# VKostoulas/Medical_Image_Generation

Measured on AMD Instinct MI355X. Metric: 3D DDPM U-Net train-step voxels/sec at 128^3 bf16, higher is better.
Workload: dtype bf16; 1 GPU; C4: DiffusionModelUNet num_channels=(32,64,128,256), attention at 16^3 (heads of 64), 128^3 x batch 1/GPU, eps-prediction, AdamW, clip 1.0; global_batch=1, parallelism=dp1, hipgraph=True

## Files before the change

include/medimgen_hip.h:

```cpp
#ifndef MEDIMGEN_HIP_H
#define MEDIMGEN_HIP_H

#include <hip/hip_runtime_api.h>
#include <stdint.h>

#ifdef __cplusplus
extern "C" {
#endif

#define MI_ERR_BAD_ARG 10001
#define MI_ERR_UNSUPPORTED 10002

int mi_abi_version(void);

int mi_ncdhw_f32_to_ndhwc_bf16(const float* src, void* dst, int N, int C, int64_t V, hipStream_t stream);
int mi_ndhwc_bf16_to_ncdhw_f32(const void* src, float* dst, int N, int C, int64_t V, hipStream_t stream);
int mi_cast_f32_to_bf16(const float* src, void* dst, int64_t n, hipStream_t stream);
int mi_cast_bf16_to_f32(const void* src, float* dst, int64_t n, int accumulate, hipStream_t stream);

int mi_add_bf16(const void* a, const void* b, void* out, int64_t n, hipStream_t stream);
int mi_copy_channels(const void* src, int Cs, int c0s, void* dst, int Cd, int c0d, int nC, int64_t nvox, hipStream_t stream);

int mi_upsample_nearest_fwd(const void* x, void* y, int N, int D, int H, int W, int C, int fd, int fh, int fw, hipStream_t stream);
int mi_upsample_nearest_bwd(const void* dy, void* dx, int N, int D, int H, int W, int C, int fd, int fh, int fw, hipStream_t stream);
int mi_space_to_depth(const void* in, int in_cstride, void* out, int N, int D, int H, int W, int C, int fd, int fh, int fw, hipStream_t stream);
int mi_depth_to_space(const void* in, void* out, int N, int D, int H, int W, int C, int fd, int fh, int fw, hipStream_t stream);

int64_t mi_gn_workspace_bytes(int N, int64_t V, int C);
int mi_gn_stats(const void* x, int x_cstride, int N, int64_t V, int C, int G, float eps, const float* gamma, const float* beta,
                float* scale_shift, float* mean_rstd, void* workspace, int64_t workspace_bytes, hipStream_t stream);
int mi_gn_stats_from_partial(const float* partial_a, int chunks_a, int Ca, const float* partial_b, int chunks_b, int Cb, int N, int64_t V,
                             int G, float eps, const float* gamma, const float* beta, float* scale_shift, float* mean_rstd,
                             hipStream_t stream);
int mi_gn_small_supported(int N, int64_t V, int C, int G);
int mi_gn_small_fwd(const void* x, int x_cstride, void* y, int y_cstride, int N, int64_t V, int C, int G, float eps, const float* gamma,
                    const float* beta, float* scale_shift, float* mean_rstd, int act, hipStream_t stream);
int mi_gn_apply(const void* x, int x_cstride, const float* scale_shift, void* y, int y_cstride, int N, int64_t V, int C, int silu,
                hipStream_t stream);
int mi_gn_bwd(const void* g, int g_cstride, const void* x, int x_cstride, int N, int64_t V, int C, int G, const float* gamma,
              const float* scale_shift, const float* mean_rstd, int silu, const void* add, int add_cstride, const void* add2, int add2_cstride,
              void* dx, int dx_cstride, float* dgamma, float* dbeta, float* coef, void* workspace, int64_t workspace_bytes, hipStream_t stream);

#define MI_GN_FUSED_REPLICAS 16
int mi_gn_bwd_fused(const void* g, int g_cstride, const void* x, int x_cstride, int N, int64_t V, int C, int G, const float* gamma,
                    const float* scale_shift, const float* mean_rstd, int silu, const void* add, int add_cstride, const void* add2,
                    int add2_cstride, void* dx, int dx_cstride, float* dgamma, float* dbeta, double* sums_zeroed, hipStream_t stream);

typedef struct mi_conv_plan mi_conv_plan;
int mi_conv_plan_create(mi_conv_plan** plan, int N, int Di, int Hi, int Wi, int Cin, int Cout, const int* kernel3, const int* stride3,
                        const int* padding3);
int mi_upconv_plan_create(mi_conv_plan** out, int N, int D, int H, int W, int Cin, int Cout);
int mi_conv_plan_destroy(mi_conv_plan* plan);
int mi_conv_plan_out_dims(const mi_conv_plan* plan, int* dims3);
int mi_conv_pack_weights(mi_conv_plan* plan, const float* weight, hipStream_t stream);
typedef struct mi_pack_batch mi_pack_batch;
int mi_conv_pack_batch_create(mi_pack_batch** out, mi_conv_plan* const* plans, const float* const* weights, int n);
int mi_conv_pack_batch_run(mi_pack_batch* batch, hipStream_t stream);
int mi_conv_pack_batch_destroy(mi_pack_batch* batch);

int mi_conv_fwd(mi_conv_plan* plan, const void* x, int x_cstride, const float* scale_shift, int silu, const float* addvec,
                int addvec_stride, const void* res, int res_cstride, void* y, int y_cstride, float* out_stats, hipStream_t stream);
int mi_conv_fwd_stats_chunks(const mi_conv_plan* plan);
int mi_conv_dgrad(mi_conv_plan* plan, const void* dy, int dy_cstride, void* dx, int dx_cstride, hipStream_t stream);
int mi_conv_wgrad(mi_conv_plan* plan, const void* x, int x_cstride, const float* scale_shift, int silu, const void* dy, int dy_cstride,
                  float* dweight, float* dy_colsum, int dy_colsum_stride, hipStream_t stream);
int mi_linear_wgrad_bf16(const void* x, int ldx, int in_features, const void* dy, int ldy, int out_features, int64_t rows, float* dw,
                         float* dbias, hipStream_t stream);

int mi_colsum_bf16(const void* x, float* out, int out_stride, int N, int64_t V, int C, int accumulate, hipStream_t stream);
int mi_add_f32_2d(const float* x, int ldx, float* y, int ldy, int rows, int cols, hipStream_t stream);
int mi_sum_rows_f32(const float* in, int ld, int rows, int cols, float* out, int accumulate, hipStream_t stream);
int mi_zero_f32_2d(float* x, int ld, int rows, int cols, hipStream_t stream);

int mi_gemm_nt_bf16(const void* A, int lda, int64_t sA1, int64_t sA2, const void* B, int ldb, int64_t sB1, int64_t sB2, void* C, int ldc,
                    int64_t sC1, int64_t sC2, const float* bias, const void* R, int ldr, int64_t sR1, int64_t sR2, int M, int N, int K,
                    int Z, int Z2, float alpha, int out_f32, int accumulate, hipStream_t stream);
int mi_transpose_bf16(const void* in, int ld_in, int64_t si1, int64_t si2, void* out, int ld_out, int64_t so1, int64_t so2, int R, int Cc,
                      int Z, int Z2, hipStream_t stream);
int mi_softmax_fwd(const float* scores, void* probs, int64_t rows, int cols, int ld_probs, hipStream_t stream);
int mi_softmax_bwd(const void* probs, const float* dprobs, void* dscores, int64_t rows, int cols, int ld_probs, float scale,
                   hipStream_t stream);

int mi_attn_supported(int C, int heads);
int64_t mi_attn_workspace_bytes(int C, int heads, int B, int S);
int mi_attn_fwd(const void* qkv, int ld, int C, int heads, int B, int S, float scale, const void* resid, void* y, float* lse, void* ws,
                int64_t ws_bytes, hipStream_t stream);
int mi_attn_bwd(const void* qkv, int ld, int C, int heads, int B, int S, float scale, const void* y, const void* resid, const void* dy,
                const float* lse, float* dsum, void* dqkv, void* ws, int64_t ws_bytes, hipStream_t stream);

int mi_timestep_embedding(const int64_t* timesteps, float* out, int B, int dim, float max_period, hipStream_t stream);
int mi_embedding_add(float* emb, const float* weight, const int64_t* labels, int B, int dim, hipStream_t stream);
int mi_embedding_bwd(const float* d_emb, const int64_t* labels, float* dweight, int B, int dim, hipStream_t stream);
int mi_silu_f32(const float* x, float* y, int64_t n, hipStream_t stream);
int mi_silu_bwd_f32(const float* x, const float* dy, float* dx, int64_t n, hipStream_t stream);

int mi_logvar_to_sigma_fwd(const void* logvar, void* sigma, int64_t n, hipStream_t stream);
int mi_logvar_to_sigma_bwd(const void* dsigma, const void* logvar, const void* sigma, void* dlogvar, int64_t n, hipStream_t stream);

int mi_layernorm_fwd(const void* x, int ldx, const float* gamma, const float* beta, void* y, int ldy, float* mean_rstd, int64_t M, int C,
                     float eps, hipStream_t stream);
int mi_layernorm_bwd(const void* dy, int lddy, const void* x, int ldx, const float* gamma, const float* mean_rstd, void* dx, int lddx,
                     float* dgamma, float* dbeta, int64_t M, int C, hipStream_t stream);
int mi_geglu_fwd(const void* h, void* y, int64_t M, int F, hipStream_t stream);
int mi_geglu_bwd(const void* h, const void* dy, void* dh, int64_t M, int F, hipStream_t stream);

int mi_avgpool_fwd(const void* x, void* y, int N, int D, int H, int W, int C, const int kernel[3], const int stride[3], hipStream_t stream);
int mi_avgpool_bwd(const void* dy, void* dx, int N, int D, int H, int W, int C, const int kernel[3], const int stride[3], hipStream_t stream);

int mi_crop_pad(const void* src, int src_is_f16, int C, int D, int H, int W, const int lo[3], float* out, int oD, int oH, int oW,
                float pad_value, int flip_mask, float scale, int clamp01, hipStream_t stream);

enum { MI_AUG_SCALE = 0, MI_AUG_CONTRAST = 1, MI_AUG_GAMMA = 2, MI_AUG_RESTORE_STATS = 3, MI_AUG_ADD_NOISE = 4, MI_AUG_CLAMP01 = 5 };
int64_t mi_aug_stats_workspace_bytes(void);
int mi_aug_plane_stats(const float* x, int64_t V, float* stats, float* workspace, hipStream_t stream);
int mi_aug_pointwise(float* x, int64_t V, int op, float p0, const float* stats_a, const float* stats_b, const float* aux, hipStream_t stream);
int mi_aug_blur_axis(const float* x, float* y, int D, int H, int W, int axis, const float* taps_host, int ntaps, hipStream_t stream);
int mi_aug_lowres(const float* x, float* y, int D, int H, int W, int lD, int lH, int lW, hipStream_t stream);
int mi_aug_affine_sample(const float* x, float* y, int D, int H, int W, int oD, int oH, int oW, const float* a_host, hipStream_t stream);

int mi_im2col3d(const void* x, int x_cstride, void* patches, int N, int D, int H, int W, int C, int k, int s, int p, hipStream_t stream);
int mi_col2im3d(const void* dpatches, void* dx, int dx_cstride, int N, int D, int H, int W, int C, int k, int s, int p, hipStream_t stream);
int mi_disc_pack_weights(const float* w, void* w2, void* w2t, int Cout, int Cout_padded, int Cin, int taps, hipStream_t stream);
int mi_disc_wgrad_unpack(const float* dw2, float* dw, int Cout, int Cin, int taps, hipStream_t stream);
int mi_leaky_relu_fwd(const void* x, void* y, int64_t n, float slope, hipStream_t stream);
int mi_leaky_relu_bwd(const void* x, const void* dy, void* dx, int64_t n, float slope, hipStream_t stream);
int mi_ls_gan_loss(const void* logits, int cs, int64_t nvox, float target, float act_slope, void* dlogits, float* loss, float weight,
                   hipStream_t stream);
int mi_bn_running_update(const float* mean_rstd, float* running_mean, float* running_var, int64_t* num_batches_tracked, int C, float eps,
                         float momentum, int64_t count, hipStream_t stream);

int mi_perc_gather(const void* x, int x_cstride, int C, int N, int D, int H, int W, int axis, const int* idx, int S, const float* shift,
                   const float* scale, void* out, hipStream_t stream);
int mi_perc_scatter_add(const void* dslices, int axis, const int* idx, int S, int N, int D, int H, int W, int C, const float* scale, void* dx,
                        int dx_cstride, hipStream_t stream);
int mi_pad_cin_f32(const float* w, float* out, int Cout, int Cin, int Cin_pad, int taps, hipStream_t stream);
int mi_relu_maxpool2_fwd(void* x, void* pooled, int N, int H, int W, int C, hipStream_t stream);
int mi_relu_maxpool2_bwd(const void* a, const void* dpooled, const void* dadd, void* dx, int N, int H, int W, int C, hipStream_t stream);
int mi_lpips_head(const void* f0, const void* f1, const float* w, int S, int64_t P, int C, float weight, float eps, float* loss, void* df0,
                  hipStream_t stream);

int mi_ssim_tiles(int D, int H, int W, int kD, int kH, int kW);
int mi_ssim_pairs(const float* x_base, const float* y_base, const int* pairs, int P, int C, int D, int H, int W, const float* taps, int kD,
                  int kH, int kW, float c1, float c2, double* partials, int part_stride, int part_off, hipStream_t stream);
int mi_ssim_pool2(const float* x, float* y, int64_t NC, int D, int H, int W, int pool_d, hipStream_t stream);
int mi_ssim_finalize(const double* partials, int P, int part_stride, int S, const int* host_tiles, const double* host_counts,
                     const double* host_weights, float* ms_out, float* ssim_out, hipStream_t stream);

int mi_qsample(const float* x0, const float* noise, const float* sqrt_alphas_cumprod, const float* sqrt_one_minus_alphas_cumprod,
               const int64_t* timesteps, const float* cond, int cond_channels, void* out, float* velocity, int N, int C, int64_t V,
               int num_train_timesteps, hipStream_t stream);
int mi_ddpm_step(float* x, const void* eps, const float* noise, const float* coef, const int64_t* t, void* x_cl, int x_cl_cs, int N,
                 int C, int64_t V, int clip, hipStream_t stream);
int mi_mse_fwd_bwd(const void* pred, const float* target, void* dpred, float* loss, int N, int C, int64_t V, float grad_scale,
                   hipStream_t stream);

int mi_l1_fwd_bwd(const void* pred, const float* target, void* dpred, float* loss, int N, int C, int64_t V, int accumulate, hipStream_t stream);
int mi_reparam_kl_fwd(const void* mu, const void* sigma, const float* eps, void* z, float* loss, int N, int C, int64_t V, float kl_weight,
                      hipStream_t stream);
int mi_reparam_kl_bwd(const void* mu, const void* sigma, const float* eps, const void* dz, void* dmu, void* dsigma, int N, int C, int64_t V,
                      float kl_weight, hipStream_t stream);

int mi_sumsq_f32(const float* x, int64_t n, float* out, int accumulate, hipStream_t stream);
int mi_clip_grad_by_norm(float* grad, int64_t n, const float* grad_sumsq, float max_norm, hipStream_t stream);
int mi_adam_step(float* param, const float* grad, float* exp_avg, float* exp_avg_sq, int64_t n, float lr, float beta1, float beta2,
                 float eps, float weight_decay, int decoupled_weight_decay, const float* grad_sumsq, float max_norm, float grad_scale,
                 float* step_counter, hipStream_t stream);
int mi_adam_step_dev(float* param, const float* grad, float* exp_avg, float* exp_avg_sq, int64_t n, const float* hparams,
                     int decoupled_weight_decay, const float* grad_sumsq, float grad_scale, float* step_counter, hipStream_t stream);
int mi_axpy_f32(float* y, const float* x, float alpha, int64_t n, hipStream_t stream);
int mi_scale_f32(float* x, float alpha, int64_t n, hipStream_t stream);

#define MI_METER_HEADER 4
#define MI_METER_PARTIALS 1024
int64_t mi_meter_bytes(void);
int mi_meter_reset(double* acc, hipStream_t stream);
int mi_mse_eval(const void* pred, const float* target, double* acc, int N, int C, int64_t V, hipStream_t stream);
int mi_l1_eval(const void* pred, const float* target, double* acc, int N, int C, int64_t V, hipStream_t stream);
int mi_kl_eval(const void* mu, const void* sigma, double* acc, int N, int C, int64_t V, hipStream_t stream);

#ifdef __cplusplus
}
#endif
#endif
```

medical_image_generation_amd/_lib.py:

```python
from __future__ import annotations

import ctypes as C
import os

import torch

_HERE = os.path.dirname(os.path.abspath(__file__))
LIB_PATH = os.environ.get("MI_LIB_PATH") or os.path.join(_HERE, "libmedimgen_hip.so")

_p, _i, _l, _f = C.c_void_p, C.c_int, C.c_int64, C.c_float

_SIGS = {
    "mi_abi_version": [],
    "mi_ncdhw_f32_to_ndhwc_bf16": [_p, _p, _i, _i, _l, _p],
    "mi_ndhwc_bf16_to_ncdhw_f32": [_p, _p, _i, _i, _l, _p],
    "mi_cast_f32_to_bf16": [_p, _p, _l, _p],
    "mi_cast_bf16_to_f32": [_p, _p, _l, _i, _p],
    "mi_add_bf16": [_p, _p, _p, _l, _p],
    "mi_copy_channels": [_p, _i, _i, _p, _i, _i, _i, _l, _p],
    "mi_upsample_nearest_fwd": [_p, _p, _i, _i, _i, _i, _i, _i, _i, _i, _p],
    "mi_upsample_nearest_bwd": [_p, _p, _i, _i, _i, _i, _i, _i, _i, _i, _p],
    "mi_space_to_depth": [_p, _i, _p, _i, _i, _i, _i, _i, _i, _i, _i, _p],
    "mi_depth_to_space": [_p, _p, _i, _i, _i, _i, _i, _i, _i, _i, _p],
    "mi_gn_workspace_bytes": [_i, _l, _i],
    "mi_gn_stats": [_p, _i, _i, _l, _i, _i, _f, _p, _p, _p, _p, _p, _l, _p],
    "mi_gn_stats_from_partial": [_p, _i, _i, _p, _i, _i, _i, _l, _i, _f, _p, _p, _p, _p, _p],
    "mi_gn_apply": [_p, _i, _p, _p, _i, _i, _l, _i, _i, _p],
    "mi_gn_bwd": [_p, _i, _p, _i, _i, _l, _i, _i, _p, _p, _p, _i, _p, _i, _p, _i, _p, _i, _p, _p, _p, _p, _l, _p],
    "mi_gn_bwd_fused": [_p, _i, _p, _i, _i, _l, _i, _i, _p, _p, _p, _i, _p, _i, _p, _i, _p, _i, _p, _p, _p, _p],
    "mi_conv_plan_create": [C.POINTER(_p), _i, _i, _i, _i, _i, _i, C.POINTER(_i), C.POINTER(_i), C.POINTER(_i)],
    "mi_upconv_plan_create": [C.POINTER(_p), _i, _i, _i, _i, _i, _i],
    "mi_conv_plan_destroy": [_p],
    "mi_conv_plan_out_dims": [_p, C.POINTER(_i)],
    "mi_conv_pack_weights": [_p, _p, _p],
    "mi_conv_pack_batch_create": [C.POINTER(_p), C.POINTER(_p), C.POINTER(_p), _i],
    "mi_conv_pack_batch_run": [_p, _p],
    "mi_conv_pack_batch_destroy": [_p],
    "mi_conv_fwd": [_p, _p, _i, _p, _i, _p, _i, _p, _i, _p, _i, _p, _p],
    "mi_conv_fwd_stats_chunks": [_p],
    "mi_conv_dgrad": [_p, _p, _i, _p, _i, _p],
    "mi_conv_wgrad": [_p, _p, _i, _p, _i, _p, _i, _p, _p, _i, _p],
    "mi_linear_wgrad_bf16": [_p, _i, _i, _p, _i, _i, _l, _p, _p, _p],
    "mi_colsum_bf16": [_p, _p, _i, _i, _l, _i, _i, _p],
    "mi_add_f32_2d": [_p, _i, _p, _i, _i, _i, _p],
    "mi_sum_rows_f32": [_p, _i, _i, _i, _p, _i, _p],
    "mi_zero_f32_2d": [_p, _i, _i, _i, _p],
    "mi_gemm_nt_bf16": [_p, _i, _l, _l, _p, _i, _l, _l, _p, _i, _l, _l, _p, _p, _i, _l, _l, _i, _i, _i, _i, _i, _f, _i, _i, _p],
    "mi_transpose_bf16": [_p, _i, _l, _l, _p, _i, _l, _l, _i, _i, _i, _i, _p],
    "mi_softmax_fwd": [_p, _p, _l, _i, _i, _p],
    "mi_softmax_bwd": [_p, _p, _p, _l, _i, _i, _f, _p],
    "mi_attn_supported": [_i, _i],
    "mi_attn_workspace_bytes": [_i, _i, _i, _i],
    "mi_attn_fwd": [_p, _i, _i, _i, _i, _i, _f, _p, _p, _p, _p, _l, _p],
    "mi_attn_bwd": [_p, _i, _i, _i, _i, _i, _f, _p, _p, _p, _p, _p, _p, _p, _l, _p],
    "mi_timestep_embedding": [_p, _p, _i, _i, _f, _p],
    "mi_silu_f32": [_p, _p, _l, _p],
    "mi_silu_bwd_f32": [_p, _p, _p, _l, _p],
    "mi_logvar_to_sigma_fwd": [_p, _p, _l, _p],
    "mi_logvar_to_sigma_bwd": [_p, _p, _p, _p, _l, _p],
    "mi_embedding_add": [_p, _p, _p, _i, _i, _p],
    "mi_embedding_bwd": [_p, _p, _p, _i, _i, _p],
    "mi_layernorm_fwd": [_p, _i, _p, _p, _p, _i, _p, _l, _i, _f, _p],
    "mi_layernorm_bwd": [_p, _i, _p, _i, _p, _p, _p, _i, _p, _p, _l, _i, _p],
    "mi_geglu_fwd": [_p, _p, _l, _i, _p],
    "mi_geglu_bwd": [_p, _p, _p, _l, _i, _p],
    "mi_avgpool_fwd": [_p, _p, _i, _i, _i, _i, _i, _p, _p, _p],
    "mi_avgpool_bwd": [_p, _p, _i, _i, _i, _i, _i, _p, _p, _p],
    "mi_crop_pad": [_p, _i, _i, _i, _i, _i, _p, _p, _i, _i, _i, _f, _i, _f, _i, _p],
    "mi_gn_small_supported": [_i, _l, _i, _i],
    "mi_gn_small_fwd": [_p, _i, _p, _i, _i, _l, _i, _i, _f, _p, _p, _p, _p, _i, _p],
    "mi_aug_stats_workspace_bytes": [],
    "mi_aug_plane_stats": [_p, _l, _p, _p, _p],
    "mi_aug_pointwise": [_p, _l, _i, _f, _p, _p, _p, _p],
    "mi_aug_blur_axis": [_p, _p, _i, _i, _i, _i, _p, _i, _p],
    "mi_aug_lowres": [_p, _p, _i, _i, _i, _i, _i, _i, _p],
    "mi_aug_affine_sample": [_p, _p, _i, _i, _i, _i, _i, _i, _p, _p],
    "mi_im2col3d": [_p, _i, _p, _i, _i, _i, _i, _i, _i, _i, _i, _p],
    "mi_col2im3d": [_p, _p, _i, _i, _i, _i, _i, _i, _i, _i, _i, _p],
    "mi_disc_pack_weights": [_p, _p, _p, _i, _i, _i, _i, _p],
    "mi_disc_wgrad_unpack": [_p, _p, _i, _i, _i, _p],
    "mi_perc_gather": [_p, _i, _i, _i, _i, _i, _i, _i, _p, _i, _p, _p, _p, _p],
    "mi_perc_scatter_add": [_p, _i, _p, _i, _i, _i, _i, _i, _i, _p, _p, _i, _p],
    "mi_pad_cin_f32": [_p, _p, _i, _i, _i, _i, _p],
    "mi_relu_maxpool2_fwd": [_p, _p, _i, _i, _i, _i, _p],
    "mi_relu_maxpool2_bwd": [_p, _p, _p, _p, _i, _i, _i, _i, _p],
    "mi_lpips_head": [_p, _p, _p, _i, _l, _i, _f, _f, _p, _p, _p],
    "mi_ssim_tiles": [_i, _i, _i, _i, _i, _i],
    "mi_ssim_pairs": [_p, _p, _p, _i, _i, _i, _i, _i, _p, _i, _i, _i, _f, _f, _p, _i, _i, _p],
    "mi_ssim_pool2": [_p, _p, _l, _i, _i, _i, _i, _p],
    "mi_ssim_finalize": [_p, _i, _i, _i, _p, _p, _p, _p, _p, _p],
    "mi_leaky_relu_fwd": [_p, _p, _l, _f, _p],
    "mi_leaky_relu_bwd": [_p, _p, _p, _l, _f, _p],
    "mi_ls_gan_loss": [_p, _i, _l, _f, _f, _p, _p, _f, _p],
    "mi_bn_running_update": [_p, _p, _p, _p, _i, _f, _f, _l, _p],
    "mi_qsample": [_p, _p, _p, _p, _p, _p, _i, _p, _p, _i, _i, _l, _i, _p],
    "mi_ddpm_step": [_p, _p, _p, _p, _p, _p, _i, _i, _i, _l, _i, _p],
    "mi_mse_fwd_bwd": [_p, _p, _p, _p, _i, _i, _l, _f, _p],
    "mi_l1_fwd_bwd": [_p, _p, _p, _p, _i, _i, _l, _i, _p],
    "mi_reparam_kl_fwd": [_p, _p, _p, _p, _p, _i, _i, _l, _f, _p],
    "mi_reparam_kl_bwd": [_p, _p, _p, _p, _p, _p, _i, _i, _l, _f, _p],
    "mi_sumsq_f32": [_p, _l, _p, _i, _p],
    "mi_clip_grad_by_norm": [_p, _l, _p, _f, _p],
    "mi_adam_step": [_p, _p, _p, _p, _l, _f, _f, _f, _f, _f, _i, _p, _f, _f, _p, _p],
    "mi_adam_step_dev": [_p, _p, _p, _p, _l, _p, _i, _p, _f, _p, _p],
    "mi_axpy_f32": [_p, _p, _f, _l, _p],
    "mi_scale_f32": [_p, _f, _l, _p],
    "mi_meter_bytes": [],
    "mi_meter_reset": [_p, _p],
    "mi_mse_eval": [_p, _p, _p, _i, _i, _l, _p],
    "mi_l1_eval": [_p, _p, _p, _i, _i, _l, _p],
    "mi_kl_eval": [_p, _p, _p, _i, _i, _l, _p],
}
_RET = {"mi_gn_workspace_bytes": _l, "mi_attn_workspace_bytes": _l, "mi_aug_stats_workspace_bytes": _l, "mi_meter_bytes": _l}
_NOCHECK = {"mi_abi_version", "mi_meter_bytes", "mi_ssim_tiles", "mi_gn_small_supported", "mi_gn_workspace_bytes", "mi_aug_stats_workspace_bytes", "mi_attn_supported", "mi_attn_workspace_bytes", "mi_conv_fwd_stats_chunks"}

_lib = None
ABI_VERSION = 12


def exported_symbols() -> list[str]:
    return sorted(_SIGS)


def load():
    global _lib
    if _lib is None:
        if not os.path.exists(LIB_PATH):
            raise RuntimeError(
                f"{LIB_PATH} is missing: build it with `python -c 'import __graft_entry__ as g; g.build()'` "
                "(there is no CPU / PyTorch fallback for the HIP path)")
        lib = C.CDLL(LIB_PATH)
        try:
            lib.mi_abi_version.restype = _i
            have = int(lib.mi_abi_version())
        except AttributeError:
            have = None
        if have != ABI_VERSION:
            raise RuntimeError(f"{LIB_PATH} is a stale library (C ABI {have}, this binding needs {ABI_VERSION}): rebuild it with "
                               "`python -c 'import __graft_entry__ as g; g.build()'`")
        for name, args in _SIGS.items():
            fn = getattr(lib, name)
            fn.argtypes = args
            fn.restype = _RET.get(name, _i)
        _lib = lib
    return _lib


def stream_ptr() -> int:
    return torch.cuda.current_stream().cuda_stream


class HipError(RuntimeError):
    pass


_ERRS = {10001: "MI_ERR_BAD_ARG (host-side shape/alignment check failed)", 10002: "MI_ERR_UNSUPPORTED"}


def ptr(t):
    if t is None:
        return None
    assert t.is_cuda, "medimgen HIP ops take device tensors only"
    return t.data_ptr()


_profile = None


class profile_calls:

    def __enter__(self):
        global _profile
        self.records = []
        _profile = self
        return self

    def __exit__(self, *exc):
        global _profile
        _profile = None
        return False

    def summary(self):
        torch.cuda.synchronize()
        out = {}
        for name, e0, e1 in self.records:
            out[name] = out.get(name, 0.0) + e0.elapsed_time(e1)
        return out


def call(name: str, *args):
    fn = getattr(load(), name)
    prof = _profile
    if prof is not None:
        st = torch.cuda.current_stream()
        e0, e1 = torch.cuda.Event(enable_timing=True), torch.cuda.Event(enable_timing=True)
        e0.record(st)
    rc = fn(*args, stream_ptr())
    if prof is not None:
        e1.record(st)
        prof.records.append((name, e0, e1))
    if rc != 0:
        raise HipError(f"{name} failed: {_ERRS.get(rc, f'hipError_t {rc}')}")


def call_raw(name: str, *args):
    fn = getattr(load(), name)
    rc = fn(*args)
    if name not in _NOCHECK and rc != 0:
        raise HipError(f"{name} failed: {_ERRS.get(rc, f'hipError_t {rc}')}")
    return rc
```

medical_image_generation_amd/blocks.py:

```python
from __future__ import annotations

import torch

from . import engine as E
from . import hipops as ops
from .unet import HipModule, ParamSpec, _axis3, _NetFn


class _Block(HipModule):
    def _check(self, x, channels, msg):
        if x.shape[1] != channels:
            raise ValueError(msg)
        if not x.is_cuda:
            raise RuntimeError("medical_image_generation_amd runs on MI355X only: move the module and inputs to 'cuda' "
                               "(there is no CPU fallback; the CPU restatement lives in oracle/ for tests)")

    def _edge(self, runner, x, emb=None):
        grad_enabled = torch.is_grad_enabled() and (x.requires_grad or (emb is not None and emb.requires_grad)
                                                    or any(p.requires_grad for p in self.parameters()))
        return _NetFn.apply(self, runner, 1, grad_enabled, x, emb, *self.parameters())


class ResnetBlock(_Block):

    def __init__(self, spatial_dims: int, in_channels: int, temb_channels: int, out_channels: int | None = None, up: bool = False,
                 down: bool = False, norm_num_groups: int = 32, norm_eps: float = 1e-6, kernel_size=2, stride=4, padding=1) -> None:
        super().__init__()
        sd = self.spatial_dims = spatial_dims
        self.channels, self.emb_channels = in_channels, temb_channels
        self.out_channels = out_channels or in_channels
        self.up, self.down = up, down
        self.groups, self.eps = norm_num_groups, norm_eps
        self._mode = "up" if up else ("down" if down else None)
        self._stride, self._kernel = _axis3(stride, sd, 1), _axis3(kernel_size, sd, 1)
        spec = ParamSpec(self, sd)
        spec.norm("norm1", in_channels)
        spec.conv("conv1.conv", in_channels, self.out_channels, 3)
        spec.linear("time_emb_proj", temb_channels, self.out_channels)
        spec.norm("norm2", self.out_channels)
        spec.conv("conv2.conv", self.out_channels, self.out_channels, 3, zero=True)
        if self.out_channels != in_channels:
            spec.conv("skip_connection.conv", in_channels, self.out_channels, 1)
        self._init_plumbing(spec, [])

    def forward(self, x: torch.Tensor, emb: torch.Tensor) -> torch.Tensor:
        self._check(x, self.channels, f"expected {self.channels} input channels, got {x.shape[1]}")

        def runner(c, xin, need_dx, emb_in):
            x_cl = ops.to_channels_last(xin.contiguous().float())
            e = emb_in.detach().contiguous().float()
            se = ops.silu_f32(e)
            temb, bwd = E.linear_f32(se, c.p("time_emb_proj.weight"), c.p("time_emb_proj.bias"), c.g("time_emb_proj.weight"),
                                     c.g("time_emb_proj.bias"))
            ops.add_f32_(temb, c.p("conv1.conv.bias"))
            d_temb = ops.zero_f32_2d_(torch.empty_like(temb)) if c.tape is not None else None
            state = {}
            if c.tape is not None:
                def bwd_emb():
                    ops.sum_rows_f32(d_temb, c.g("conv1.conv.bias"), accumulate=True)
                    state["d_emb"] = ops.silu_bwd_f32(e, bwd(d_temb))

                c.tape.record(bwd_emb)
            y = E.resnet(c, x_cl, "", self.spatial_dims, self.groups, self.eps, temb, d_temb, mode=self._mode, stride=self._stride,
                         kernel=self._kernel)
            return (y,), {"x_cl": x_cl, "d_emb": lambda: state.get("d_emb")}

        return self._edge(runner, x, emb)


class AttentionBlock(_Block):

    def __init__(self, spatial_dims: int, num_channels: int, num_head_channels: int | None = None, norm_num_groups: int = 32,
                 norm_eps: float = 1e-6, use_flash_attention: bool = False) -> None:
        super().__init__()
        if use_flash_attention:
            raise ValueError("use_flash_attention is True but xformers is not installed.")
        self.spatial_dims, self.num_channels = spatial_dims, num_channels
        self.num_heads = num_channels // num_head_channels if num_head_channels is not None else 1
        self.groups, self.eps = norm_num_groups, norm_eps
        spec = ParamSpec(self, spatial_dims)
        spec.attention("", num_channels)
        self._init_plumbing(spec, [[f"to_{t}.weight" for t in "qkv"], [f"to_{t}.bias" for t in "qkv"]])

    def forward(self, x: torch.Tensor) -> torch.Tensor:
        self._check(x, self.num_channels, f"expected {self.num_channels} input channels, got {x.shape[1]}")

        def runner(c, xin, need_dx):
            x_cl = ops.to_channels_last(xin.contiguous().float())
            return (E.attention(c, x_cl, "", self.groups, self.eps, self.num_heads),), {"x_cl": x_cl}

        return self._edge(runner, x)


class Downsample(_Block):

    def __init__(self, spatial_dims: int, num_channels: int, use_conv: bool, out_channels: int | None = None, stride=2, kernel_size=4,
                 padding=1) -> None:
        super().__init__()
        sd = self.spatial_dims = spatial_dims
        self.num_channels, self.out_channels, self.use_conv = num_channels, out_channels or num_channels, use_conv
        self._k, self._s, self._p = _axis3(kernel_size, sd, 1), _axis3(stride, sd, 1), _axis3(padding, sd, 0)
        spec = ParamSpec(self, sd)
        if use_conv:
            spec.conv("op.conv", num_channels, self.out_channels, kernel_size)
        elif self.num_channels != self.out_channels:
            raise ValueError("num_channels and out_channels must be equal when use_conv=False")
        self._init_plumbing(spec, [])

    def forward(self, x: torch.Tensor, emb: torch.Tensor | None = None) -> torch.Tensor:
        del emb
        self._check(x, self.num_channels, f"Input number of channels ({x.shape[1]}) is not equal to expected number of channels "
                                          f"({self.num_channels})")

        def runner(c, xin, need_dx):
            x_cl = ops.to_channels_last(xin.contiguous().float())
            if self.use_conv:
                y = E.conv(c, x_cl, "op.conv", self._k, self._s, self._p, need_dx=need_dx)
            else:
                y = E.avg_pool(c, x_cl, self._k, self._s)
            return (y,), {"x_cl": x_cl}

        return self._edge(runner, x)


class Upsample(_Block):

    def __init__(self, spatial_dims: int, num_channels: int, use_conv: bool, out_channels: int | None = None, stride=2, padding=1) -> None:
        super().__init__()
        sd = self.spatial_dims = spatial_dims
        self.num_channels, self.out_channels, self.use_conv, self.stride = num_channels, out_channels or num_channels, use_conv, stride
        self._s, self._p = tuple(int(v) for v in _axis3(stride, sd, 1)), _axis3(padding, sd, 0)
        spec = ParamSpec(self, sd)
        if use_conv:
            spec.conv("conv.conv", num_channels, self.out_channels, 3)
        self._init_plumbing(spec, [])

    def forward(self, x: torch.Tensor, emb: torch.Tensor | None = None) -> torch.Tensor:
        del emb
        self._check(x, self.num_channels, "Input channels should be equal to num_channels")
        sd = self.spatial_dims
        k3 = (1,) * (3 - sd) + (3,) * sd

        def runner(c, xin, need_dx):
            x_cl = ops.to_channels_last(xin.contiguous().float())
            if self.use_conv:
                y = E.upsample_conv(c, x_cl, "conv.conv", self._s, k3, self._p)
            else:
                y = E.upsample(c, x_cl, self._s)
            return (y,), {"x_cl": x_cl}

        return self._edge(runner, x)


class ResBlock(_Block):

    def __init__(self, spatial_dims: int, in_channels: int, norm_num_groups: int, norm_eps: float, out_channels: int) -> None:
        super().__init__()
        sd = self.spatial_dims = spatial_dims
        self.in_channels = in_channels
        self.out_channels = in_channels if out_channels is None else out_channels
        self.groups, self.eps = norm_num_groups, norm_eps
        spec = ParamSpec(self, sd)
        spec.norm("norm1", in_channels)
        spec.conv("conv1.conv", in_channels, self.out_channels, 3)
        spec.norm("norm2", self.out_channels)
        spec.conv("conv2.conv", self.out_channels, self.out_channels, 3)
        if self.in_channels != self.out_channels:
            spec.conv("nin_shortcut.conv", in_channels, self.out_channels, 1)
        self._init_plumbing(spec, [])

    def forward(self, x: torch.Tensor) -> torch.Tensor:
        self._check(x, self.in_channels, f"expected {self.in_channels} input channels, got {x.shape[1]}")
        sd = self.spatial_dims
        k3, s1, p1 = (1,) * (3 - sd) + (3,) * sd, (1, 1, 1), (0,) * (3 - sd) + (1,) * sd

        def runner(c, xin, need_dx):
            x_cl = ops.to_channels_last(xin.contiguous().float())
            n1 = E.gn(c, x_cl, "norm1", self.groups, self.eps)
            h = E.conv(c, x_cl, "conv1.conv", k3, s1, p1, norm=n1, silu=True)
            n2 = E.gn(c, h, "norm2", self.groups, self.eps)
            xs = x_cl
            if "nin_shortcut.conv.weight" in c.arena.offsets:
                xs = E.conv(c, x_cl, "nin_shortcut.conv", (1, 1, 1), s1, (0, 0, 0), bias_grad_like="conv2.conv")
            return (E.conv(c, h, "conv2.conv", k3, s1, p1, norm=n2, silu=True, res=xs),), {"x_cl": x_cl}

        return self._edge(runner, x)


class SpatialTransformer(_Block):

    def __init__(self, spatial_dims: int, in_channels: int, num_attention_heads: int, num_head_channels: int, num_layers: int = 1,
                 dropout: float = 0.0, norm_num_groups: int = 32, norm_eps: float = 1e-6, cross_attention_dim: int | None = None,
                 upcast_attention: bool = False, use_flash_attention: bool = False) -> None:
        super().__init__()
        if use_flash_attention:
            raise ValueError("use_flash_attention is True but xformers is not installed.")
        if dropout > 0.0:
            raise NotImplementedError("dropout > 0 is not on the HIP path (the reference's default is 0.0)")
        if num_attention_heads * num_head_channels != in_channels:
            raise NotImplementedError("the HIP path covers inner_dim == in_channels (how every block of the U-Net constructs it, UNet:976-990)")
        self.spatial_dims, self.in_channels = spatial_dims, in_channels
        self.heads, self.layers, self.groups, self.eps = num_attention_heads, num_layers, norm_num_groups, norm_eps
        self.cross_attention_dim = cross_attention_dim if cross_attention_dim is not None else in_channels
        spec = ParamSpec(self, spatial_dims)
        spec.transformer("", in_channels, self.cross_attention_dim, num_layers)
        self._init_plumbing(spec, [])

    def forward(self, x: torch.Tensor, context: torch.Tensor | None = None) -> torch.Tensor:
        self._check(x, self.in_channels, f"expected {self.in_channels} input channels, got {x.shape[1]}")
        ctx_tokens = None
        if context is not None:
            if context.dim() != 3 or context.shape[0] != x.shape[0] or context.shape[2] != self.cross_attention_dim:
                raise ValueError(f"context must be [batch, tokens, {self.cross_attention_dim}], got {tuple(context.shape)}")
            ctx_tokens = ops.cast_bf16(context.detach().to(x.device).contiguous().float().reshape(-1, context.shape[2]))

        def runner(c, xin, need_dx):
            x_cl = ops.to_channels_last(xin.contiguous().float())
            return (E.spatial_transformer(c, x_cl, "", ctx_tokens, self.groups, self.eps, self.heads, self.layers),), {"x_cl": x_cl}

        return self._edge(runner, x)
```

medical_image_generation_amd/csrc/api.hip:

```cpp
#include "common.h"
#include "medimgen_hip.h"
extern "C" int mi_abi_version(void) { return 12; }
```

medical_image_generation_amd/csrc/conv_c1.hip:

```cpp
#include <stdlib.h>

#include "common.h"
#include "conv_common.h"
#include "medimgen_hip.h"

namespace {

struct C1Args {
  int N, D, H, W, C;
  const bf16* s;
  int s_cs;
  const bf16* m;
  int m_cs;
  const float* w;
  const float* addvec;
  int av_stride;
  bf16* y;
  int y_cs;
  float* stats;
  int stats_chunks;
};

constexpr int kExpPitch = 64 * 2 + 16;
template <int FLIP>
__global__ void __launch_bounds__(256) k_c1_expand(C1Args a) {
  __shared__ __attribute__((aligned(16))) char stage[4][64 * kExpPitch];
  const int lane = threadIdx.x & 63, wave = threadIdx.x >> 6;
  const int64_t total = (int64_t)a.N * a.D * a.H * a.W;
  const int64_t v0 = blockIdx.x * 256ll + wave * 64;
  if (v0 >= total) return;
  const int64_t v = v0 + lane < total ? v0 + lane : total - 1;
  const int wx = (int)(v % a.W);
  int64_t t1 = v / a.W;
  const int hy = (int)(t1 % a.H);
  t1 /= a.H;
  const int dz = (int)(t1 % a.D), n = (int)(t1 / a.D);
  const bf16* sn = a.s + (int64_t)n * a.D * a.H * a.W * a.s_cs;
  float xs[27];
#pragma unroll
  for (int kd = 0; kd < 3; ++kd)
#pragma unroll
    for (int kh = 0; kh < 3; ++kh)
#pragma unroll
      for (int kw = 0; kw < 3; ++kw) {
        const int z = dz + kd - 1, yy = hy + kh - 1, x = wx + kw - 1;
        const int zc = min(max(z, 0), a.D - 1), yc = min(max(yy, 0), a.H - 1), xc = min(max(x, 0), a.W - 1);
        const float val = bf2f(sn[(((int64_t)zc * a.H + yc) * a.W + xc) * a.s_cs]);
        xs[(kd * 3 + kh) * 3 + kw] = (z == zc && yy == yc && x == xc) ? val : 0.f;
      }
  char* my = stage[wave];
  for (int c0 = 0; c0 < a.C; c0 += 8) {
    F8 acc;
#pragma unroll
    for (int j = 0; j < 8; ++j) acc.v[j] = a.addvec ? a.addvec[(int64_t)n * a.av_stride + c0 + j] : 0.f;
#pragma unroll
    for (int j = 0; j < 8; ++j) {
      const float* wr = a.w + (c0 + j) * 27;
#pragma unroll
      for (int t = 0; t < 27; ++t) acc.v[j] = fmaf(xs[t], wr[FLIP ? 26 - t : t], acc.v[j]);
    }
    *(u32x4*)(my + lane * kExpPitch + c0 * 2) = pack8(acc);
  }
  const int C8 = a.C / 8;
  for (int i = lane; i < 64 * C8; i += 64) {
    const int vox = i / C8, ch = i % C8;
    if (v0 + vox < total) *(u32x4*)(a.y + (v0 + vox) * a.y_cs + ch * 8) = *(const u32x4*)(my + vox * kExpPitch + ch * 16);
  }
}

constexpr int kTD = 4, kTH = 8, kTW = 8, kHD = kTD + 2, kHH = kTH + 2, kHW = kTW + 2, kHalo = kHD * kHH * kHW;
template <int NCB, int FLIP>
__global__ void __launch_bounds__(256) k_c1_expand_mfma(C1Args a, int ntiles) {
  constexpr int HS = 3 * kHH * kHW;
  __shared__ bf16 sh[4][2][HS + 4];
  const int lane = threadIdx.x & 63, wave = threadIdx.x >> 6, v = lane & 31, h = lane >> 5;
  const int tw = (a.W + kTW - 1) / kTW, th = (a.H + kTH - 1) / kTH, td = (a.D + kTD - 1) / kTD;
  const int crow = 16 * ((v >> 2) & 1) + (v & 3) + 4 * (v >> 3);
  bf16x8 wf[NCB][2];
#pragma unroll
  for (int cb = 0; cb < NCB; ++cb)
#pragma unroll
    for (int ks = 0; ks < 2; ++ks) {
      F8 f;
#pragma unroll
      for (int j = 0; j < 8; ++j) {
        const int tap = ks * 16 + 8 * h + j, c = cb * 32 + crow;
        f.v[j] = (tap < 27 && c < a.C) ? a.w[c * 27 + (FLIP ? 26 - tap : tap)] : 0.f;
      }
      wf[cb][ks] = __builtin_bit_cast(bf16x8, pack8(f));
    }
  int toff[2][8];
#pragma unroll
  for (int ks = 0; ks < 2; ++ks)
#pragma unroll
    for (int j = 0; j < 8; ++j) {
      const int tap = ks * 16 + 8 * h + j, t2 = tap < 27 ? tap : 13;
      toff[ks][j] = (t2 / 9) * (kHH * kHW) + ((t2 / 3) % 3) * kHW + t2 % 3;
    }
  bf16 sreg[5];
  auto issue = [&](int tile) {
    int r = tile;
    const int tx = r % tw; r /= tw;
    const int ty = r % th; r /= th;
    const int tz = r % td, n = r / td;
    const int z = tz * kTD + wave, y0 = ty * kTH, x0 = tx * kTW;
    const bf16* sn = a.s + (int64_t)n * a.D * a.H * a.W * a.s_cs;
#pragma unroll
    for (int i = 0; i < 5; ++i) {
      const int hi = i * 64 + lane;
      const int hx = hi % kHW, hy = (hi / kHW) % kHH, hz = hi / (kHW * kHH);
      const int zz = z + hz - 1, yy = y0 + hy - 1, xx = x0 + hx - 1;
      const bool in = hi < HS && (unsigned)zz < (unsigned)a.D && (unsigned)yy < (unsigned)a.H && (unsigned)xx < (unsigned)a.W;
      sreg[i] = in ? sn[(((int64_t)zz * a.H + yy) * a.W + xx) * a.s_cs] : f2bf(0.f);
    }
  };
  constexpr bool ST = NCB == 1 && FLIP == 0;
  __shared__ float sred[4][2][32];
  float sa[16], sq[16];
#pragma unroll
  for (int e = 0; e < 16; ++e) sa[e] = sq[e] = 0.f;
  int sn = -1;
  auto stats_flush = [&](int img) {
#pragma unroll
    for (int e = 0; e < 16; ++e) {
#pragma unroll
      for (int m = 1; m < 32; m <<= 1) {
        sa[e] += __shfl_xor(sa[e], m, 64);
        sq[e] += __shfl_xor(sq[e], m, 64);
      }
    }
    __syncthreads();
    if (v == 0) {
#pragma unroll
      for (int e = 0; e < 16; ++e) { sred[wave][0][16 * h + e] = sa[e]; sred[wave][1][16 * h + e] = sq[e]; }
    }
    __syncthreads();
    if (threadIdx.x < 32 && (int)threadIdx.x < a.C) {
      const int c = threadIdx.x;
      const float s0 = (sred[0][0][c] + sred[1][0][c]) + (sred[2][0][c] + sred[3][0][c]);
      const float s1 = (sred[0][1][c] + sred[1][1][c]) + (sred[2][1][c] + sred[3][1][c]);
      *(float2*)(a.stats + (((int64_t)img * a.C + c) * a.stats_chunks + blockIdx.x) * 2) = make_float2(s0, s1);
    }
#pragma unroll
    for (int e = 0; e < 16; ++e) sa[e] = sq[e] = 0.f;
  };
  if (ST && a.stats && threadIdx.x < 32 && (int)threadIdx.x < a.C)
    for (int img = 0; img < a.N; ++img) *(float2*)(a.stats + (((int64_t)img * a.C + threadIdx.x) * a.stats_chunks + blockIdx.x) * 2) = make_float2(0.f, 0.f);
  int tile = blockIdx.x, buf = 0;
  if (tile < ntiles) issue(tile);
  for (; tile < ntiles; tile += gridDim.x, buf ^= 1) {
    bf16* hb = sh[wave][buf];
#pragma unroll
    for (int i = 0; i < 5; ++i) {
      const int hi = i * 64 + lane;
      if (hi < HS) hb[hi] = sreg[i];
    }
    int r = tile;
    const int tx = r % tw; r /= tw;
    const int ty = r % th; r /= th;
    const int tz = r % td, n = r / td;
    const int z = tz * kTD + wave;
    if (ST && a.stats && n != sn) {
      if (sn >= 0) stats_flush(sn);
      sn = n;
    }
    if (tile + (int)gridDim.x < ntiles) issue(tile + gridDim.x);
#pragma unroll
    for (int blk = 0; blk < 2; ++blk) {
      const int row = 4 * blk + (v >> 3), col = v & 7;
      const int base = row * kHW + col;
      f32x16 acc[NCB];
#pragma unroll
      for (int cb = 0; cb < NCB; ++cb)
#pragma unroll
        for (int e = 0; e < 16; ++e) {
          const int c = cb * 32 + 16 * h + e;
          acc[cb][e] = (a.addvec && c < a.C) ? a.addvec[(int64_t)n * a.av_stride + c] : 0.f;
        }
#pragma unroll
      for (int ks = 0; ks < 2; ++ks) {
        bf16x8 bfr;
#pragma unroll
        for (int j = 0; j < 8; ++j) bfr[j] = (ks * 16 + 8 * h + j) < 27 ? hb[base + toff[ks][j]] : f2bf(0.f);
#pragma unroll
        for (int cb = 0; cb < NCB; ++cb) acc[cb] = __builtin_amdgcn_mfma_f32_32x32x16_bf16(wf[cb][ks], bfr, acc[cb], 0, 0, 0);
      }
      const int y = ty * kTH + row, x = tx * kTW + col;
      if (z < a.D && y < a.H && x < a.W) {
        bf16* out = a.y + ((((int64_t)n * a.D + z) * a.H + y) * a.W + x) * a.y_cs;
#pragma unroll
        for (int cb = 0; cb < NCB; ++cb) {
          const int c0 = cb * 32 + 16 * h;
          F8 lo, hi;
#pragma unroll
          for (int e = 0; e < 8; ++e) { lo.v[e] = acc[cb][e]; hi.v[e] = acc[cb][8 + e]; }
          const u32x4 plo = pack8(lo), phi = pack8(hi);
          if (c0 < a.C) *(u32x4*)(out + c0) = plo;
          if (c0 + 8 < a.C) *(u32x4*)(out + c0 + 8) = phi;
          if (ST && a.stats) {
            const F8 rl = unpack8(plo), rh = unpack8(phi);
#pragma unroll
            for (int e = 0; e < 8; ++e) {
              sa[e] += rl.v[e]; sq[e] = fmaf(rl.v[e], rl.v[e], sq[e]);
              sa[8 + e] += rh.v[e]; sq[8 + e] = fmaf(rh.v[e], rh.v[e], sq[8 + e]);
            }
          }
        }
      }
    }
  }
  if (ST && a.stats && sn >= 0) stats_flush(sn);
}

constexpr int kYP = 33;

template <int NK>
__global__ void __launch_bounds__(256) k_c1_reduce(C1Args a) {
  extern __shared__ float Y[];
  const int lane = threadIdx.x & 63, wave = threadIdx.x >> 6, r = lane & 31, h = lane >> 5;
  const int tw = (a.W + kTW - 1) / kTW, th = (a.H + kTH - 1) / kTH, td = (a.D + kTD - 1) / kTD;
  int tile = blockIdx.x;
  const int tx = tile % tw; tile /= tw;
  const int ty = tile % th; tile /= th;
  const int tz = tile % td, n = tile / td;
  const int z0 = tz * kTD - 1, y0 = ty * kTH - 1, x0 = tx * kTW - 1;
  bf16x8 wf[NK];
#pragma unroll
  for (int ks = 0; ks < NK; ++ks) {
    F8 f;
#pragma unroll
    for (int j = 0; j < 8; ++j) {
      const int c = ks * 16 + 8 * h + j;
      f.v[j] = (r < 27 && c < a.C) ? a.w[c * 27 + r] : 0.f;
    }
    wf[ks] = __builtin_bit_cast(bf16x8, pack8(f));
  }
  const bf16* xn = a.m + (int64_t)n * a.D * a.H * a.W * a.m_cs;
  constexpr int NB = ((kHalo + 31) / 32 + 3) / 4;
  u32x4 raw[NB][NK];
  bool ok[NB];
#pragma unroll
  for (int i = 0; i < NB; ++i) {
    const int hu = (wave + 4 * i) * 32 + r;
    const int hx = hu % kHW, hy = (hu / kHW) % kHH, hz = hu / (kHW * kHH);
    const int z = z0 + hz, yy = y0 + hy, x = x0 + hx;
    const int zc = min(max(z, 0), a.D - 1), yc = min(max(yy, 0), a.H - 1), xc = min(max(x, 0), a.W - 1);
    ok[i] = hu < kHalo && z == zc && yy == yc && x == xc;
    const bf16* px = xn + (((int64_t)zc * a.H + yc) * a.W + xc) * a.m_cs;
#pragma unroll
    for (int ks = 0; ks < NK; ++ks) {
      const int c = min(ks * 16 + 8 * h, a.C - 8);
      raw[i][ks] = *(const u32x4*)(px + c);
    }
  }
#pragma unroll
  for (int i = 0; i < NB; ++i) {
    const int blk = wave + 4 * i;
    if (blk >= (kHalo + 31) / 32) break;
    f32x16 acc;
#pragma unroll
    for (int e = 0; e < 16; ++e) acc[e] = 0.f;
#pragma unroll
    for (int ks = 0; ks < NK; ++ks) {
      u32x4 b = raw[i][ks];
      if (!(ok[i] && ks * 16 + 8 * h < a.C)) b = u32x4{0u, 0u, 0u, 0u};
      acc = __builtin_amdgcn_mfma_f32_32x32x16_bf16(wf[ks], __builtin_bit_cast(bf16x8, b), acc, 0, 0, 0);
    }
    const int hu = blk * 32 + r;
#pragma unroll
    for (int e = 0; e < 16; ++e) Y[hu * kYP + (e & 3) + 8 * (e >> 2) + 4 * h] = acc[e];
  }
  __syncthreads();
  const int ox = threadIdx.x & 7, oy = (threadIdx.x >> 3) & 7, oz = threadIdx.x >> 6;
  const int z = tz * kTD + oz, yy = ty * kTH + oy, x = tx * kTW + ox;
  if (z >= a.D || yy >= a.H || x >= a.W) return;
  float o = a.addvec ? a.addvec[(int64_t)n * a.av_stride] : 0.f;
#pragma unroll
  for (int kd = 0; kd < 3; ++kd)
#pragma unroll
    for (int kh = 0; kh < 3; ++kh)
#pragma unroll
      for (int kw = 0; kw < 3; ++kw) o += Y[(((oz + kd) * kHH + oy + kh) * kHW + ox + kw) * kYP + (kd * 3 + kh) * 3 + kw];
  a.y[((((int64_t)n * a.D + z) * a.H + yy) * a.W + x) * a.y_cs] = f2bf(o);
}

struct C1WgArgs {
  int N, D, H, W, C;
  const bf16* m; int m_cs;
  const bf16* s; int s_cs;
  float* part;
  int ntiles, flip;
};
template <int NCB>
__global__ void __launch_bounds__(256) k_c1_wgrad(C1WgArgs a) {
  constexpr int PITCH = NCB * 64, MT = 64 * PITCH, HS = 3 * kHH * kHW, HSB = (HS * 2 + 15) / 16 * 16, WV = 2 * MT + 2 * HSB;
  constexpr int PVMAX = NCB * 4;
  extern __shared__ __attribute__((aligned(16))) char c1w_lds[];
  const int lane = threadIdx.x & 63, wave = threadIdx.x >> 6, t = lane & 31, h = lane >> 5;
  char* my = c1w_lds + wave * WV;
  const int tw = (a.W + kTW - 1) / kTW, th = (a.H + kTH - 1) / kTH, td = (a.D + kTD - 1) / kTD;
  const int PV = a.C >> 3;
  const int tt = a.flip ? 26 - t : t;
  const int kd = tt / 9, kh = (tt / 3) % 3, kw = tt % 3;
  for (int i = lane; i < 2 * MT / 16; i += 64) ((u32x4*)my)[i] = u32x4{0u, 0u, 0u, 0u};
  f32x16 acc[NCB];
#pragma unroll
  for (int cb = 0; cb < NCB; ++cb)
#pragma unroll
    for (int e = 0; e < 16; ++e) acc[cb][e] = 0.f;
  float s_acc = 0.f;

  u32x4 mreg[PVMAX];
  bf16 sreg[5];
  auto issue = [&](int tile) {
    int r = tile;
    const int tx = r % tw; r /= tw;
    const int ty = r % th; r /= th;
    const int tz = r % td, n = r / td;
    const int z = tz * kTD + wave, y0 = ty * kTH, x0 = tx * kTW;
    const bf16* mn = a.m + (int64_t)n * a.D * a.H * a.W * a.m_cs;
    const bf16* sn = a.s + (int64_t)n * a.D * a.H * a.W * a.s_cs;
#pragma unroll
    for (int i = 0; i < PVMAX; ++i) {
      const int idx = i * 64 + lane, v = idx / PV, p = idx - v * PV;
      const int y = y0 + (v >> 3), x = x0 + (v & 7);
      const bool in = i < PV && v < 64 && z < a.D && y < a.H && x < a.W;
      mreg[i] = in ? *(const u32x4*)(mn + (((int64_t)z * a.H + y) * a.W + x) * a.m_cs + p * 8) : u32x4{0u, 0u, 0u, 0u};
    }
#pragma unroll
    for (int i = 0; i < 5; ++i) {
      const int hi = i * 64 + lane;
      const int hx = hi % kHW, hy = (hi / kHW) % kHH, hz = hi / (kHW * kHH);
      const int zz = z + hz - 1, yy = y0 + hy - 1, xx = x0 + hx - 1;
      const bool in = hi < HS && (unsigned)zz < (unsigned)a.D && (unsigned)yy < (unsigned)a.H && (unsigned)xx < (unsigned)a.W;
      sreg[i] = in ? sn[(((int64_t)zz * a.H + yy) * a.W + xx) * a.s_cs] : f2bf(0.f);
    }
  };
  int tile = blockIdx.x, buf = 0;
  if (tile < a.ntiles) issue(tile);
  for (; tile < a.ntiles; tile += gridDim.x, buf ^= 1) {
    char* mt = my + buf * MT;
    bf16* sh = (bf16*)(my + 2 * MT + buf * HSB);
#pragma unroll
    for (int i = 0; i < PVMAX; ++i) {
      const int idx = i * 64 + lane, v = idx / PV, p = idx - v * PV;
      if (i < PV && v < 64) *(u32x4*)(mt + v * PITCH + p * 16) = mreg[i];
    }
#pragma unroll
    for (int i = 0; i < 5; ++i) {
      const int hi = i * 64 + lane;
      if (hi < HS) {
        sh[hi] = sreg[i];
        const int hx = hi % kHW, hy = (hi / kHW) % kHH, hz = hi / (kHW * kHH);
        if (hz == 1 && hy >= 1 && hy <= kTH && hx >= 1 && hx <= kTW) s_acc += bf2f(sreg[i]);
      }
    }
    if (tile + (int)gridDim.x < a.ntiles) issue(tile + gridDim.x);
#pragma unroll
    for (int q = 0; q < 4; ++q) {
      const int v0 = (2 * q + h) * 8;
      bf16x8 bfr;
      const int hb = (kd * kHH + 2 * q + h + kh) * kHW + kw;
#pragma unroll
      for (int j = 0; j < 8; ++j) bfr[j] = t < 27 ? sh[hb + j] : (t == 27 ? f2bf(1.f) : f2bf(0.f));
#pragma unroll
      for (int cb = 0; cb < NCB; ++cb) {
        bf16x8 af;
#pragma unroll
        for (int j = 0; j < 8; ++j) af[j] = *(const bf16*)(mt + (v0 + j) * PITCH + (cb * 32 + t) * 2);
        acc[cb] = __builtin_amdgcn_mfma_f32_32x32x16_bf16(af, bfr, acc[cb], 0, 0, 0);
      }
    }
  }
  __syncthreads();
  float* red = (float*)c1w_lds;
#pragma unroll
  for (int cb = 0; cb < NCB; ++cb)
#pragma unroll
    for (int e = 0; e < 16; ++e) red[wave * NCB * 1024 + cb * 1024 + ((e & 3) + 8 * (e >> 2) + 4 * h) * 32 + t] = acc[cb][e];
  s_acc = wave_sum(s_acc);
  if (lane == 0) red[4 * NCB * 1024 + wave] = s_acc;
  __syncthreads();
  float* out = a.part + (int64_t)blockIdx.x * (NCB * 1024 + 32);
  for (int i = threadIdx.x; i < NCB * 1024; i += 256)
    out[i] = (red[i] + red[NCB * 1024 + i]) + (red[2 * NCB * 1024 + i] + red[3 * NCB * 1024 + i]);
  if (threadIdx.x == 0) out[NCB * 1024] = (red[4 * NCB * 1024] + red[4 * NCB * 1024 + 1]) + (red[4 * NCB * 1024 + 2] + red[4 * NCB * 1024 + 3]);
}
__global__ void __launch_bounds__(256) k_c1_wgrad_reduce(const float* __restrict__ part, int nslab, int slab, int C, float* __restrict__ dw,
                                                         float* __restrict__ colsum_m, float* __restrict__ colsum_s) {
  __shared__ float red[8][32];
  const int i = blockIdx.x * 32 + (threadIdx.x & 31), g = threadIdx.x >> 5;
  const bool live = i <= C * 32;
  const int idx = i < C * 32 ? i : slab - 32;
  float s0 = 0.f, s1 = 0.f, s2 = 0.f, s3 = 0.f;
  if (live) {
    int k = g;
    for (; k + 24 < nslab; k += 32) {
      s0 += part[(int64_t)k * slab + idx];
      s1 += part[(int64_t)(k + 8) * slab + idx];
      s2 += part[(int64_t)(k + 16) * slab + idx];
      s3 += part[(int64_t)(k + 24) * slab + idx];
    }
    for (; k < nslab; k += 8) s0 += part[(int64_t)k * slab + idx];
  }
  red[g][threadIdx.x & 31] = (s0 + s1) + (s2 + s3);
  __syncthreads();
  if (g != 0 || !live) return;
  float v = 0.f;
#pragma unroll
  for (int j = 0; j < 8; ++j) v += red[j][threadIdx.x];
  if (i == C * 32) { if (colsum_s) colsum_s[0] += v; return; }
  const int c = i >> 5, tp = i & 31;
  if (tp < 27) dw[c * 27 + tp] += v;
  else if (tp == 27 && colsum_m) colsum_m[c] += v;
}

bool c1_dims_ok(int N, int D, int H, int W, int C) {
  return N > 0 && D > 0 && H > 0 && W > 0 && C >= 8 && C <= 64 && (C & 7) == 0 && (int64_t)N * D * H * W < (1ll << 31);
}

}

static int c1_use_mfma() {
  static const int v = [] { const char* e = getenv("MI_C1_EXPAND_MFMA"); return e ? atoi(e) : 1; }();
  return v;
}
int mi_c1_expand_stats_chunks(int N, int D, int H, int W, int C) {
  static const int on = [] { const char* e = getenv("MI_C1_STATS"); return e ? atoi(e) : 1; }();
  if (!on || !c1_use_mfma() || !c1_dims_ok(N, D, H, W, C) || C > 32 || N > 16) return 0;
  const int64_t tiles = (int64_t)N * ((D + kTD - 1) / kTD) * ((H + kTH - 1) / kTH) * ((W + kTW - 1) / kTW);
  if (tiles >= (1ll << 31)) return 0;
  return (int)(tiles < 2048 ? tiles : 2048);
}
int mi_launch_c1_expand(const void* s, int s_cs, const float* w, const float* addvec, int av_stride, void* y, int y_cs, int N, int D, int H,
                        int W, int C, int flip, hipStream_t st, float* stats) {
  if (!c1_dims_ok(N, D, H, W, C) || (y_cs & 7)) return MI_ERR_UNSUPPORTED;
  C1Args a{};
  a.N = N; a.D = D; a.H = H; a.W = W; a.C = C;
  a.s = (const bf16*)s; a.s_cs = s_cs; a.w = w; a.addvec = addvec; a.av_stride = av_stride; a.y = (bf16*)y; a.y_cs = y_cs;
  a.stats = stats; a.stats_chunks = stats ? mi_c1_expand_stats_chunks(N, D, H, W, C) : 0;
  if (stats && (flip || a.stats_chunks == 0)) return MI_ERR_UNSUPPORTED;
  const int use_mfma = c1_use_mfma();
  const int64_t tiles = (int64_t)N * ((D + kTD - 1) / kTD) * ((H + kTH - 1) / kTH) * ((W + kTW - 1) / kTW);
  if (use_mfma && tiles < (1ll << 31)) {
    const int grid = (int)(tiles < 2048 ? tiles : 2048);
    const int ncb = (C + 31) / 32;
    if (ncb == 1) {
      if (flip) hipLaunchKernelGGL((k_c1_expand_mfma<1, 1>), dim3(grid), dim3(256), 0, st, a, (int)tiles);
      else hipLaunchKernelGGL((k_c1_expand_mfma<1, 0>), dim3(grid), dim3(256), 0, st, a, (int)tiles);
    } else {
      if (flip) hipLaunchKernelGGL((k_c1_expand_mfma<2, 1>), dim3(grid), dim3(256), 0, st, a, (int)tiles);
      else hipLaunchKernelGGL((k_c1_expand_mfma<2, 0>), dim3(grid), dim3(256), 0, st, a, (int)tiles);
    }
    MI_CHECK_LAUNCH();
    return 0;
  }
  const int64_t total = (int64_t)N * D * H * W;
  dim3 grid((unsigned)((total + 255) / 256));
  if (flip) hipLaunchKernelGGL(k_c1_expand<1>, grid, dim3(256), 0, st, a);
  else hipLaunchKernelGGL(k_c1_expand<0>, grid, dim3(256), 0, st, a);
  MI_CHECK_LAUNCH();
  return 0;
}

int mi_launch_c1_reduce(const void* x, int x_cs, const float* w, const float* addvec, int av_stride, void* y, int y_cs, int N, int D, int H,
                        int W, int C, hipStream_t st) {
  if (!c1_dims_ok(N, D, H, W, C) || (x_cs & 7)) return MI_ERR_UNSUPPORTED;
  C1Args a{};
  a.N = N; a.D = D; a.H = H; a.W = W; a.C = C;
  a.m = (const bf16*)x; a.m_cs = x_cs; a.w = w; a.addvec = addvec; a.av_stride = av_stride; a.y = (bf16*)y; a.y_cs = y_cs;
  const int64_t tiles = (int64_t)N * ((D + kTD - 1) / kTD) * ((H + kTH - 1) / kTH) * ((W + kTW - 1) / kTW);
  if (tiles >= (1ll << 31)) return MI_ERR_UNSUPPORTED;
  const size_t lds = sizeof(float) * (size_t)((kHalo + 31) / 32 * 32) * kYP;
  const int nk = (C + 15) / 16;
  auto k = nk == 1 ? k_c1_reduce<1> : nk == 2 ? k_c1_reduce<2> : nk == 3 ? k_c1_reduce<3> : k_c1_reduce<4>;
  static bool attr_done[4] = {false, false, false, false};
  if (!attr_done[nk - 1]) {
    hipError_t e = hipFuncSetAttribute((const void*)k, hipFuncAttributeMaxDynamicSharedMemorySize, (int)lds);
    if (e != hipSuccess) return (int)e;
    attr_done[nk - 1] = true;
  }
  hipLaunchKernelGGL(k, dim3((unsigned)tiles), dim3(256), lds, st, a);
  MI_CHECK_LAUNCH();
  return 0;
}

int mi_c1_wgrad_slabs() { return 512; }
int64_t mi_c1_wgrad_scratch_floats(int C) { return (int64_t)mi_c1_wgrad_slabs() * (((C + 31) / 32) * 1024 + 32); }
int mi_launch_c1_wgrad(const void* m, int m_cs, const void* s1, int s_cs, float* dw, float* colsum_m, float* colsum_s, float* part, int N, int D,
                       int H, int W, int C, int flip, hipStream_t st) {
  if (!c1_dims_ok(N, D, H, W, C) || !part) return MI_ERR_UNSUPPORTED;
  const int64_t tiles = (int64_t)N * ((D + kTD - 1) / kTD) * ((H + kTH - 1) / kTH) * ((W + kTW - 1) / kTW);
  if (tiles >= (1ll << 31)) return MI_ERR_UNSUPPORTED;
  C1WgArgs a{};
  a.N = N; a.D = D; a.H = H; a.W = W; a.C = C;
  a.m = (const bf16*)m; a.m_cs = m_cs; a.s = (const bf16*)s1; a.s_cs = s_cs; a.part = part; a.ntiles = (int)tiles; a.flip = flip;
  const int ncb = (C + 31) / 32;
  int grid = mi_c1_wgrad_slabs();
  if (grid > tiles) grid = (int)tiles;
  {
    const int pitch = ncb * 64, mt = 64 * pitch, hsb = (3 * kHH * kHW * 2 + 15) / 16 * 16;
    size_t lds = 4 * (size_t)(2 * mt + 2 * hsb);
    const size_t need_red = sizeof(float) * (size_t)(4 * ncb * 1024 + 4);
    if (lds < need_red) lds = need_red;
    static bool attr_done[2] = {false, false};
    auto kern = ncb == 1 ? k_c1_wgrad<1> : k_c1_wgrad<2>;
    if (!attr_done[ncb - 1]) {
      hipError_t e = hipFuncSetAttribute((const void*)kern, hipFuncAttributeMaxDynamicSharedMemorySize, 96 * 1024);
      if (e != hipSuccess) return (int)e;
      attr_done[ncb - 1] = true;
    }
    hipLaunchKernelGGL(kern, dim3(grid), dim3(256), lds, st, a);
  }
  const int slab = ncb * 1024 + 32;
  hipLaunchKernelGGL(k_c1_wgrad_reduce, dim3((C * 32 + 1 + 31) / 32), dim3(256), 0, st, part, grid, slab, C, dw, colsum_m, colsum_s);
  MI_CHECK_LAUNCH();
  return 0;
}
```

medical_image_generation_amd/csrc/gemm.hip:

```cpp
#include "common.h"
#include "medimgen_hip.h"

namespace {

constexpr int BK = 32, PITCH = 40;

struct GemmArgs {
  const bf16* A;
  const bf16* B;
  void* C;
  const float* bias;
  const bf16* R;
  int M, N, K, lda, ldb, ldc, ldr;
  int Z2;
  int64_t sA1, sA2, sB1, sB2, sC1, sC2, sR1, sR2;
  float alpha;
  int out_f32, accumulate;
};

template <int WT>
__global__ void __launch_bounds__(256) k_gemm_nt(GemmArgs p) {
  constexpr int BM = 64 * WT, BN = 64 * WT;
  __shared__ __attribute__((aligned(16))) bf16 lds[2][2][BM * PITCH];
  const int tid = threadIdx.x, lane = tid & 63, wave = tid >> 6;
  const int wm = wave >> 1, wn = wave & 1;
  const int r = lane & 31, h = lane >> 5;
  const int z = blockIdx.z, z1 = z / p.Z2, z2 = z % p.Z2;
  const bf16* A = p.A + z1 * p.sA1 + z2 * p.sA2;
  const bf16* B = p.B + z1 * p.sB1 + z2 * p.sB2;
  const int m0 = blockIdx.y * BM, n0 = blockIdx.x * BN;

  int prow[WT], pk[WT];
#pragma unroll
  for (int i = 0; i < WT; ++i) {
    int pc = tid + 256 * i;
    prow[i] = pc >> 2;
    pk[i] = (pc & 3) * 8;
  }
  u32x4 ra[WT], rb[WT];
  auto gload = [&](int k0) {
#pragma unroll
    for (int i = 0; i < WT; ++i) {
      u32x4 zero = {0u, 0u, 0u, 0u};
      int k = k0 + pk[i];
      int am = m0 + prow[i], bn = n0 + prow[i];
      ra[i] = (am < p.M && k < p.K) ? *(const u32x4*)(A + (int64_t)am * p.lda + k) : zero;
      rb[i] = (bn < p.N && k < p.K) ? *(const u32x4*)(B + (int64_t)bn * p.ldb + k) : zero;
    }
  };
  auto lstore = [&](int buf) {
#pragma unroll
    for (int i = 0; i < WT; ++i) {
      *(u32x4*)(&lds[buf][0][prow[i] * PITCH + pk[i]]) = ra[i];
      *(u32x4*)(&lds[buf][1][prow[i] * PITCH + pk[i]]) = rb[i];
    }
  };

  f32x16 acc[WT][WT];
#pragma unroll
  for (int a = 0; a < WT; ++a)
#pragma unroll
    for (int b = 0; b < WT; ++b)
#pragma unroll
      for (int e = 0; e < 16; ++e) acc[a][b][e] = 0.f;

  const int nk = (p.K + BK - 1) / BK;
  gload(0);
  lstore(0);
  __syncthreads();
  for (int kt = 0; kt < nk; ++kt) {
    const int buf = kt & 1;
    if (kt + 1 < nk) gload((kt + 1) * BK);
#pragma unroll
    for (int ks = 0; ks < 2; ++ks) {
      bf16x8 fa[WT], fb[WT];
#pragma unroll
      for (int i = 0; i < WT; ++i) {
        fa[i] = *(const bf16x8*)(&lds[buf][0][(wm * 32 * WT + i * 32 + r) * PITCH + ks * 16 + h * 8]);
        fb[i] = *(const bf16x8*)(&lds[buf][1][(wn * 32 * WT + i * 32 + r) * PITCH + ks * 16 + h * 8]);
      }
#pragma unroll
      for (int a = 0; a < WT; ++a)
#pragma unroll
        for (int b = 0; b < WT; ++b) acc[a][b] = __builtin_amdgcn_mfma_f32_32x32x16_bf16(fa[a], fb[b], acc[a][b], 0, 0, 0);
    }
    if (kt + 1 < nk) lstore(buf ^ 1);
    __syncthreads();
  }

  const int64_t coff = z1 * p.sC1 + z2 * p.sC2;
  const int64_t roff = z1 * p.sR1 + z2 * p.sR2;
#pragma unroll
  for (int a = 0; a < WT; ++a)
#pragma unroll
    for (int b = 0; b < WT; ++b) {
      const int n = n0 + wn * 32 * WT + b * 32 + r;
      if (n >= p.N) continue;
      const float bv = p.bias ? p.bias[n] : 0.f;
#pragma unroll
      for (int e = 0; e < 16; ++e) {
        const int m = m0 + wm * 32 * WT + a * 32 + (e & 3) + 8 * (e >> 2) + 4 * h;
        if (m >= p.M) continue;
        float v = acc[a][b][e] * p.alpha + bv;
        if (p.R) v += bf2f(p.R[roff + (int64_t)m * p.ldr + n]);
        const int64_t ci = coff + (int64_t)m * p.ldc + n;
        if (p.out_f32) {
          float* c = (float*)p.C;
          c[ci] = p.accumulate ? c[ci] + v : v;
        } else {
          ((bf16*)p.C)[ci] = f2bf(v);
        }
      }
    }
}

__global__ void __launch_bounds__(256) k_transpose(const bf16* __restrict__ in, bf16* __restrict__ out, int R, int Cc, int ld_in,
                                                   int ld_out, int Z2, int64_t si1, int64_t si2, int64_t so1, int64_t so2) {
  __shared__ bf16 t[64][66];
  const int z = blockIdx.z, z1 = z / Z2, z2 = z % Z2;
  in += z1 * si1 + z2 * si2;
  out += z1 * so1 + z2 * so2;
  const int r0 = blockIdx.y * 64, c0 = blockIdx.x * 64;
  for (int i = threadIdx.x; i < 64 * 64; i += 256) {
    int rr = i >> 6, cc = i & 63;
    t[rr][cc] = (r0 + rr < R && c0 + cc < Cc) ? in[(int64_t)(r0 + rr) * ld_in + c0 + cc] : f2bf(0.f);
  }
  __syncthreads();
  for (int i = threadIdx.x; i < 64 * 64; i += 256) {
    int cc = i >> 6, rr = i & 63;
    if (c0 + cc < Cc && r0 + rr < R) out[(int64_t)(c0 + cc) * ld_out + r0 + rr] = t[rr][cc];
    else if (c0 + cc < Cc && r0 + rr < min((R + 7) & ~7, ld_out)) out[(int64_t)(c0 + cc) * ld_out + r0 + rr] = f2bf(0.f);
  }
}

__global__ void __launch_bounds__(256) k_softmax_fwd(const float* __restrict__ s, bf16* __restrict__ pr, int cols, int ldp) {
  __shared__ float red[4];
  const float* row = s + (int64_t)blockIdx.x * cols;
  bf16* o = pr + (int64_t)blockIdx.x * ldp;
  float mx = -3.0e38f;
  for (int j = threadIdx.x; j < cols; j += 256) mx = fmaxf(mx, row[j]);
  mx = wave_max(mx);
  if ((threadIdx.x & 63) == 0) red[threadIdx.x >> 6] = mx;
  __syncthreads();
  mx = fmaxf(fmaxf(red[0], red[1]), fmaxf(red[2], red[3]));
  float sum = 0.f;
  for (int j = threadIdx.x; j < cols; j += 256) sum += __expf(row[j] - mx);
  sum = block_sum_256(sum, red);
  const float inv = 1.0f / sum;
  for (int j = threadIdx.x; j < cols; j += 256) o[j] = f2bf(__expf(row[j] - mx) * inv);
  for (int j = cols + threadIdx.x; j < ldp; j += 256) o[j] = f2bf(0.f);
}
__global__ void __launch_bounds__(256) k_softmax_bwd(const bf16* __restrict__ pr, const float* __restrict__ dp, bf16* __restrict__ ds,
                                                     int cols, int ldp, float scale) {
  __shared__ float red[4];
  const bf16* prow = pr + (int64_t)blockIdx.x * ldp;
  const float* drow = dp + (int64_t)blockIdx.x * cols;
  bf16* o = ds + (int64_t)blockIdx.x * ldp;
  float dot = 0.f;
  for (int j = threadIdx.x; j < cols; j += 256) dot += bf2f(prow[j]) * drow[j];
  dot = block_sum_256(dot, red);
  for (int j = threadIdx.x; j < cols; j += 256) o[j] = f2bf(bf2f(prow[j]) * (drow[j] - dot) * scale);
  for (int j = cols + threadIdx.x; j < ldp; j += 256) o[j] = f2bf(0.f);
}

}

extern "C" {

int mi_gemm_nt_bf16(const void* A, int lda, int64_t sA1, int64_t sA2, const void* B, int ldb, int64_t sB1, int64_t sB2, void* C, int ldc,
                    int64_t sC1, int64_t sC2, const float* bias, const void* R, int ldr, int64_t sR1, int64_t sR2, int M, int N, int K,
                    int Z, int Z2, float alpha, int out_f32, int accumulate, hipStream_t st) {
  if (M <= 0 || N <= 0 || K <= 0 || Z <= 0 || Z2 <= 0 || Z % Z2) return MI_ERR_BAD_ARG;
  if ((K & 7) || (lda & 7) || (ldb & 7) || ((uintptr_t)A & 15) || ((uintptr_t)B & 15)) return MI_ERR_BAD_ARG;
  if ((sA1 | sA2 | sB1 | sB2) & 7) return MI_ERR_BAD_ARG;
  if (accumulate && !out_f32) return MI_ERR_BAD_ARG;
  GemmArgs p;
  p.A = (const bf16*)A; p.B = (const bf16*)B; p.C = C; p.bias = bias; p.R = (const bf16*)R;
  p.M = M; p.N = N; p.K = K; p.lda = lda; p.ldb = ldb; p.ldc = ldc; p.ldr = ldr;
  p.Z2 = Z2; p.sA1 = sA1; p.sA2 = sA2; p.sB1 = sB1; p.sB2 = sB2; p.sC1 = sC1; p.sC2 = sC2; p.sR1 = sR1; p.sR2 = sR2;
  p.alpha = alpha; p.out_f32 = out_f32; p.accumulate = accumulate;
  if ((int64_t)ceil_div(N, 128) * ceil_div(M, 128) * Z < 256)
    hipLaunchKernelGGL(k_gemm_nt<1>, dim3(ceil_div(N, 64), ceil_div(M, 64), Z), dim3(256), 0, st, p);
  else
    hipLaunchKernelGGL(k_gemm_nt<2>, dim3(ceil_div(N, 128), ceil_div(M, 128), Z), dim3(256), 0, st, p);
  MI_CHECK_LAUNCH();
  return 0;
}

int mi_transpose_bf16(const void* in, int ld_in, int64_t si1, int64_t si2, void* out, int ld_out, int64_t so1, int64_t so2, int R, int Cc,
                      int Z, int Z2, hipStream_t st) {
  if (R <= 0 || Cc <= 0 || Z <= 0 || Z2 <= 0 || Z % Z2) return MI_ERR_BAD_ARG;
  hipLaunchKernelGGL(k_transpose, dim3(ceil_div(Cc, 64), ceil_div(R, 64), Z), dim3(256), 0, st, (const bf16*)in, (bf16*)out, R, Cc, ld_in,
                     ld_out, Z2, si1, si2, so1, so2);
  MI_CHECK_LAUNCH();
  return 0;
}

int mi_softmax_fwd(const float* scores, void* probs, int64_t rows, int cols, int ld_probs, hipStream_t st) {
  if (rows <= 0 || cols <= 0 || rows > 2147483647LL || ld_probs < cols) return MI_ERR_BAD_ARG;
  hipLaunchKernelGGL(k_softmax_fwd, dim3((int)rows), dim3(256), 0, st, scores, (bf16*)probs, cols, ld_probs);
  MI_CHECK_LAUNCH();
  return 0;
}
int mi_softmax_bwd(const void* probs, const float* dprobs, void* dscores, int64_t rows, int cols, int ld_probs, float scale,
                   hipStream_t st) {
  if (rows <= 0 || cols <= 0 || rows > 2147483647LL || ld_probs < cols) return MI_ERR_BAD_ARG;
  hipLaunchKernelGGL(k_softmax_bwd, dim3((int)rows), dim3(256), 0, st, (const bf16*)probs, dprobs, (bf16*)dscores, cols, ld_probs, scale);
  MI_CHECK_LAUNCH();
  return 0;
}

}
```

medical_image_generation_amd/engine.py:

```python
from __future__ import annotations

import math
import weakref

import torch

from . import _lib
from . import hipops as ops
from ._lib import call, ptr

BF16, F32 = torch.bfloat16, torch.float32

import os as _os
FLASH_ATTENTION = _os.environ.get("MI_FLASH_ATTENTION", "1") == "1"
FUSE_GN_STATS = ops.FUSE_GN_STATS


class ParamArena:

    def __init__(self, entries, device, late=()):
        self.offsets, self.shapes = {}, {}
        late = set(late)
        off = 0
        self.n_late = 0
        for trainable_pass in (True, False):
            for name, shape, trainable in entries:
                if trainable != trainable_pass:
                    continue
                n = math.prod(shape)
                self.offsets[name], self.shapes[name] = off, tuple(shape)
                off += n
                if not trainable_pass or n % 4:
                    off = (off + 3) // 4 * 4
                if trainable_pass and name in late:
                    assert self.n_late == self.offsets[name], f"late tensors must form a prefix of the arena ({name})"
                    self.n_late = off
            if trainable_pass:
                off = (off + 3) // 4 * 4
                self.n_trainable = off
        self.numel = max(off, 4)
        self.data = torch.zeros(self.numel, dtype=F32, device=device)
        self.grad = torch.zeros(self.numel, dtype=F32, device=device)

    def view(self, name, flat=None):
        flat = self.data if flat is None else flat
        o, s = self.offsets[name], self.shapes[name]
        return flat[o:o + math.prod(s)].view(s)

    def gview(self, name):
        return self.view(name, self.grad)

    def span(self, names, flat=None):
        flat = self.data if flat is None else flat
        o = self.offsets[names[0]]
        end = o
        for nme in names:
            assert self.offsets[nme] == end, f"{nme} is not adjacent in the arena"
            end += math.prod(self.shapes[nme])
        return flat[o:end]


def CUT():
    """Tape marker (a no-op when called): recorded by a model at the forward position behind which -- in backward order: before
    which -- every gradient of the arena's early segment is final.  trainer._ArenaTrainer splits the backward there."""


class Tape:
    def __init__(self):
        self.fns = []
        self.grads = {}
        self.keep = []

    def record(self, fn):
        self.fns.append(fn)

    def take(self, t):
        g = self.grads.pop(id(t), None)
        return ops.add(g[0], g[1]) if isinstance(g, tuple) else g

    def take2(self, t):
        g = self.grads.pop(id(t), None)
        return g if isinstance(g, tuple) else (g, None)

    def put(self, t, g):
        cur = self.grads.get(id(t))
        if cur is None:
            self.grads[id(t)] = g
        elif isinstance(cur, tuple):
            self.grads[id(t)] = ops.add(ops.add(cur[0], cur[1]), g)
        else:
            self.grads[id(t)] = (cur, g)
        self.keep.append(t)

    def move(self, t, other: "Tape"):
        g = self.grads.pop(id(t), None)
        if g is not None:
            other.grads[id(t)] = g
            other.keep.append(t)

    def backward(self, out, dout):
        self.put(out, dout)
        for fn in reversed(self.fns):
            fn()
        self.fns.clear()


class Ctx:

    def __init__(self, arena: ParamArena, plans: dict, grad_enabled=True, prepacked=()):
        self.arena, self.plans = arena, plans
        self.tape = Tape() if grad_enabled else None
        self.packed = set(prepacked)
        self.flops_fwd = 0
        self.flops_bwd = 0
        self.sums = {}
        self.cat_parts = {}

    def sums_of(self, x):
        ent = self.sums.get(id(x))
        return ent[0] if ent is not None and ent[1]() is x else None

    def parts_of(self, x):
        ent = self.cat_parts.get(id(x))
        return ent[:2] if ent is not None and ent[2]() is x else None

    def count(self, fwd_flops, dgrad=True, wgrad=True):
        self.flops_fwd += fwd_flops
        if self.tape is not None:
            self.flops_bwd += fwd_flops * (int(dgrad) + int(wgrad))

    def p(self, name):
        return self.arena.view(name)

    def g(self, name):
        return self.arena.gview(name)


class PackBatch:

    def __init__(self, arena: ParamArena, plans: dict):
        import ctypes as C
        self.keys = tuple(plans)
        n = len(self.keys)
        plan_arr = (C.c_void_p * n)(*[plans[k].handle for k in self.keys])
        w_arr = (C.c_void_p * n)(*[arena.view(k[0] + ".weight").data_ptr() for k in self.keys])
        h = C.c_void_p()
        _lib.call_raw("mi_conv_pack_batch_create", C.byref(h), plan_arr, w_arr, n)
        self.handle = h

    def run(self):
        call("mi_conv_pack_batch_run", self.handle)
        return self.keys

    def __del__(self):
        try:
            if getattr(self, "handle", None):
                _lib.call_raw("mi_conv_pack_batch_destroy", self.handle)
                self.handle = None
        except Exception:
            pass


def gn(ctx: Ctx, x, name, groups, eps):
    gamma, beta = ctx.p(name + ".weight"), ctx.p(name + ".bias")
    st = None
    if FUSE_GN_STATS:
        n, v = x.shape[0], x.shape[1] * x.shape[2] * x.shape[3]
        ent, parts = ctx.sums_of(x), ctx.parts_of(x)
        if ent is not None:
            st = ops.gn_stats_from_sums(ent, None, n, v, groups, eps, gamma, beta)
        elif parts is not None:
            ea, eb = ctx.sums_of(parts[0]), ctx.sums_of(parts[1])
            if ea is not None and eb is not None:
                st = ops.gn_stats_from_sums(ea, eb, n, v, groups, eps, gamma, beta)
    if st is None:
        st = ops.gn_stats(x, groups, eps, gamma, beta)
    st.name = name
    return st


UPCONV = _os.environ.get("MI_UPCONV", "1") == "1"


def upsample_conv(ctx: Ctx, x, name, factors, kernel, padding, out=None):
    n, d, h, w, cin = x.shape
    fused = UPCONV and tuple(factors) == (2, 2, 2) and tuple(kernel) == (3, 3, 3) and tuple(padding) == (1, 1, 1) and d > 1 and \
        cin % 8 == 0 and ctx.p(name + ".weight").shape[0] % 8 == 0 and x.is_contiguous()
    if not fused:
        return conv(ctx, upsample(ctx, x, factors), name, kernel, (1, 1, 1), padding, out=out)
    return conv(ctx, x, name, kernel, (1, 1, 1), padding, out=out, upconv=True)


def conv_transpose(ctx: Ctx, x, name, kernel, stride, padding):
    n, d, h, w, cin = x.shape
    wt = ctx.p(name + ".weight")
    cout = wt.shape[1]
    k, s_, p_ = tuple(kernel), tuple(stride), tuple(padding)
    if d <= 1 or k != (3, 3, 3) or p_ != (1, 1, 1) or s_ not in ((1, 1, 1), (2, 2, 2)) or cin % 8 or cout % 8:
        raise NotImplementedError(f"use_convtranspose: kernel {k} stride {s_} padding {p_} ({cin}->{cout}) is not on the HIP path "
                                  "(3-D, kernel 3, padding 1, stride 1 or 2 on all axes, channels in multiples of 8)")
    fine = tuple(v * s_[0] for v in (d, h, w))
    key = (name, n, d, h, w)
    plan = ctx.plans.get(key)
    if plan is None:
        plan = ctx.plans[key] = ops.ConvPlan(n, fine, cout, cin, k, s_, p_)
    if key not in ctx.packed:
        plan.pack(wt)
        ctx.packed.add(key)
    y0 = plan.dgrad(x)
    bias = ctx.p(name + ".bias")
    ss = torch.stack([torch.ones_like(bias), bias], dim=1).unsqueeze(0).expand(n, cout, 2).contiguous()
    y = ops.gn_apply(y0, ops.GNStats(ss, None, 1), False)
    del y0
    ctx.count(2 * y.numel() * cin * 27 // (s_[0] ** 3), dgrad=True)
    if ctx.tape is not None:
        tape = ctx.tape

        def bwd():
            dy = tape.take(y)
            if dy is None:
                return
            plan.wgrad(dy, x, ctx.g(name + ".weight"))
            ops.colsum(dy.contiguous(), out=ctx.g(name + ".bias"), accumulate=True, merge_batch=True)
            tape.put(x, plan.fwd(dy))

        tape.record(bwd)
    return y


def conv(ctx: Ctx, x, name, kernel, stride, padding, norm=None, silu=False, addvec=None, res=None, d_addvec=None,
         need_dx=True, bias_grad_like=None, out=None, upconv=False):
    n, d, h, w, cin = x.shape
    wt = ctx.p(name + ".weight")
    cout = wt.shape[0]
    key = (name, n, d, h, w)
    plan = ctx.plans.get(key)
    if plan is None:
        plan = ctx.plans[key] = ops.UpConvPlan(n, (d, h, w), cin, cout) if upconv else ops.ConvPlan(n, (d, h, w), cin, cout, kernel, stride, padding)
    if key not in ctx.packed:
        plan.pack(wt)
        ctx.packed.add(key)
    av = addvec if addvec is not None else ctx.p(name + ".bias")
    xin = ops.gn_apply(x, norm, silu) if norm is not None else x
    y, sums = plan.fwd(xin, addvec=av, res=res, out=out, want_sums=True)
    if sums is not None:
        ctx.sums[id(y)] = (sums, weakref.ref(y))
    ctx.count(2 * y.numel() * cin * math.prod(kernel), dgrad=need_dx)
    if ctx.tape is not None:
        tape = ctx.tape

        def bwd():
            dy = tape.take(y)
            if dy is None:
                return
            gw = ctx.g(name + ".weight")
            if bias_grad_like is not None:
                plan.wgrad(xin, dy, gw)
                ops.add_f32_(ctx.g(name + ".bias"), ctx.g(bias_grad_like + ".bias"))
            else:
                plan.wgrad(xin, dy, gw, colsum=d_addvec if d_addvec is not None else ctx.g(name + ".bias"))
            if res is not None:
                tape.put(res, dy)
            if need_dx:
                g = plan.dgrad(dy)
                if norm is not None:
                    other, other2 = tape.take2(x)
                    dx = ops.gn_bwd(g, x, norm, ctx.p(norm.name + ".weight"), silu, ctx.g(norm.name + ".weight"),
                                    ctx.g(norm.name + ".bias"), add=other, add2=other2)
                    tape.grads[id(x)] = dx
                    tape.keep.append(x)
                else:
                    tape.put(x, g)

        tape.record(bwd)
    return y


def upsample(ctx: Ctx, x, factors):
    y = ops.upsample_nearest(x, factors)
    if ctx.tape is not None:
        tape = ctx.tape

        def bwd():
            dy = tape.take(y)
            if dy is not None:
                tape.put(x, ops.upsample_nearest_bwd(ops.dense(dy), factors))

        tape.record(bwd)
    return y


def checkpoint(ctx: Ctx, fn, x):
    if ctx.tape is None:
        return fn(ctx, x)
    sub = Ctx(ctx.arena, ctx.plans, grad_enabled=False)
    sub.packed, sub.sums, sub.cat_parts = ctx.packed, ctx.sums, ctx.cat_parts
    y = fn(sub, x)
    ctx.flops_fwd += sub.flops_fwd
    ctx.flops_bwd += 2 * sub.flops_fwd
    tape = ctx.tape

    def bwd():
        dy = tape.take(y)
        if dy is None:
            return
        inner = Ctx(ctx.arena, ctx.plans, grad_enabled=True)
        inner.packed, inner.sums, inner.cat_parts = ctx.packed, ctx.sums, ctx.cat_parts
        y2 = fn(inner, x)
        it = inner.tape
        tape.move(x, it)
        it.backward(y2, dy)
        g = it.take(x)
        if g is not None:
            tape.grads[id(x)] = g
            tape.keep.append(x)
        it.grads.clear(), it.keep.clear()

    tape.record(bwd)
    return y


def avg_pool(ctx: Ctx, x, kernel, stride):
    y = ops.avg_pool(x, kernel, stride)
    if ctx.tape is not None:
        tape = ctx.tape
        dims = tuple(x.shape[1:4])

        def bwd():
            dy = tape.take(y)
            if dy is not None:
                tape.put(x, ops.avg_pool_bwd(ops.dense(dy), dims, kernel, stride))

        tape.record(bwd)
    return y


def gn_act(ctx: Ctx, x, st, silu):
    y = ops.gn_apply(x, st, silu)
    if ctx.tape is not None:
        tape = ctx.tape

        def bwd():
            g = tape.take(y)
            if g is None:
                return
            other, other2 = tape.take2(x)
            dx = ops.gn_bwd(g, x, st, ctx.p(st.name + ".weight"), silu, ctx.g(st.name + ".weight"), ctx.g(st.name + ".bias"),
                            add=other, add2=other2)
            tape.grads[id(x)] = dx
            tape.keep.append(x)

        tape.record(bwd)
    return y


def add(ctx: Ctx, a, b, b_needs_grad=True):
    y = ops.add(a, b)
    if ctx.tape is not None:
        tape = ctx.tape

        def bwd():
            dy = tape.take(y)
            if dy is not None:
                tape.put(a, dy)
                if b_needs_grad:
                    tape.put(b, dy)

        tape.record(bwd)
    return y


def resnet(ctx: Ctx, x, name, sd, groups, eps, addvec, d_addvec, mode=None, stride=None, kernel=None, out=None):
    k3, s1, p1 = (1,) * (3 - sd) + (3,) * sd, (1, 1, 1), (0,) * (3 - sd) + (1,) * sd
    name = name + "." if name else ""
    n1 = gn(ctx, x, name + "norm1", groups, eps)
    if mode is None:
        h = conv(ctx, x, name + "conv1.conv", k3, s1, p1, norm=n1, silu=True, addvec=addvec, d_addvec=d_addvec)
    else:
        h = gn_act(ctx, x, n1, True)
        if mode == "up":
            x, h = upsample(ctx, x, stride), upsample(ctx, h, stride)
        else:
            x, h = avg_pool(ctx, x, kernel, stride), avg_pool(ctx, h, kernel, stride)
        h = conv(ctx, h, name + "conv1.conv", k3, s1, p1, addvec=addvec, d_addvec=d_addvec)
    n2 = gn(ctx, h, name + "norm2", groups, eps)
    if name + "skip_connection.conv.weight" in ctx.arena.offsets:
        xs = conv(ctx, x, name + "skip_connection.conv", (1, 1, 1), s1, (0, 0, 0), bias_grad_like=name + "conv2.conv")
    else:
        xs = x
    return conv(ctx, h, name + "conv2.conv", k3, s1, p1, norm=n2, silu=True, res=xs, out=out)


def concat_buffer(a_shape, ca, cb, device):
    buf = torch.empty(tuple(a_shape[:-1]) + (ca + cb,), dtype=BF16, device=device)
    return buf, buf[..., :ca]


def concat(ctx: Ctx, a, b, buf=None):
    ca, cb = a.shape[-1], b.shape[-1]
    a_in = buf is not None and a.data_ptr() == buf.data_ptr() and ops._cs(a) == ca + cb
    b_in = buf is not None and b.data_ptr() == buf.data_ptr() + 2 * ca and ops._cs(b) == ca + cb
    if a_in or b_in:
        n, v = a.shape[0], a.shape[1] * a.shape[2] * a.shape[3]
        if not a_in:
            call("mi_copy_channels", ptr(a), ops._cs(a), 0, ptr(buf), ca + cb, 0, ca, n * v)
        if not b_in:
            call("mi_copy_channels", ptr(b), ops._cs(b), 0, ptr(buf), ca + cb, ca, cb, n * v)
        y = buf
    else:
        y = ops.concat_channels(a, b)
    ctx.cat_parts[id(y)] = (a, b, weakref.ref(y))
    if ctx.tape is not None:
        tape = ctx.tape

        def bwd():
            dy = tape.take(y)
            if dy is None:
                return
            for t, lo, n_c, in_place in ((a, 0, ca, a_in), (b, ca, cb, b_in)):
                if in_place and id(t) not in tape.grads:
                    tape.grads[id(t)] = dy[..., lo:lo + n_c]
                    tape.keep.append(t)
                    tape.keep.append(dy)
                else:
                    tape.put(t, ops.slice_channels(dy, lo, n_c))

        tape.record(bwd)
    return y


def token_wgrad(dy, x, out=None):
    return ops.gemm_nt(ops.transpose(dy, pad_to=8), ops.transpose(x, pad_to=8), out=out, out_f32=True, accumulate=out is not None)


def linear_dgrad(dy, wb, out_f32=False):
    return ops.gemm_nt(dy, ops.transpose(wb), out_f32=out_f32)


def _heads(t, b, heads):
    return t.view(b, -1, heads, t.shape[-1] // heads).permute(0, 2, 1, 3)


def _sdpa(q, k, v, scale, out, res=None):
    if q.shape[-1] % 8:
        raise ValueError("head width must be a multiple of 8 on the HIP path")
    scores = ops.gemm_nt(q, k, alpha=scale, out_f32=True)
    probs = ops.softmax_fwd(scores, pad8=True)
    del scores
    ops.gemm_nt(ops.padded(probs), ops.transpose(v, pad_to=8), out=out, res=res)

    def bwd(do, dq, dk, dv):
        dp = ops.gemm_nt(do, v, out_f32=True)
        ds = ops.softmax_bwd(probs, dp, scale)
        del dp
        ops.gemm_nt(ops.padded(ds), ops.transpose(k, pad_to=8), out=dq)
        qt = ops.transpose(q, pad_to=8)
        dst = ops.transpose(ds, pad_to=8)
        ops.gemm_nt(dst, qt, out=dk)
        del dst, ds
        pt = ops.transpose(probs, pad_to=8)
        ops.gemm_nt(pt, ops.transpose(do, pad_to=8), out=dv)

    return bwd


def _attention_flash(ctx, x, name, st, xn, wqkv, qkv, b, s, c, heads, scale):
    dev = x.device
    d_, h_, w_ = x.shape[1:4]
    y = torch.empty_like(x)
    lse = torch.empty((b * heads, s), dtype=F32, device=dev)
    nws = _lib.call_raw("mi_attn_workspace_bytes", c, heads, b, s)
    ws = torch.empty(max(nws, 16), dtype=torch.uint8, device=dev)
    call("mi_attn_fwd", ptr(qkv), 3 * c, c, heads, b, s, float(scale), ptr(x), ptr(y), ptr(lse), ptr(ws), nws)
    del ws
    ctx.count(2 * b * s * c * 3 * c)
    ctx.count(4 * b * s * s * c)
    if ctx.tape is not None:
        tape = ctx.tape

        def bwd():
            dy = tape.take(y)
            if dy is None:
                return
            dqkv = torch.empty((b * s, 3 * c), dtype=BF16, device=dev)
            dsum = torch.empty((b * heads, s), dtype=F32, device=dev)
            ws = torch.empty(max(nws, 16), dtype=torch.uint8, device=dev)
            call("mi_attn_bwd", ptr(qkv), 3 * c, c, heads, b, s, float(scale), ptr(y), ptr(x), ptr(dy), ptr(lse), ptr(dsum), ptr(dqkv),
                 ptr(ws), nws)
            _attention_param_and_input_grads(ctx, tape, x, name, st, xn, wqkv, dqkv, dy, b, s, c)

        tape.record(bwd)
    return y


def _attention_param_and_input_grads(ctx, tape, x, name, st, xn, wqkv, dqkv, dy, b, s, c):
    pre = name + "." if name else ""
    gw = ctx.arena.span([f"{pre}to_{t}.weight" for t in "qkv"], ctx.arena.grad)
    gb = ctx.arena.span([f"{pre}to_{t}.bias" for t in "qkv"], ctx.arena.grad)
    call("mi_linear_wgrad_bf16", ptr(xn), c, c, ptr(dqkv), 3 * c, 3 * c, b * s, ptr(gw), ptr(gb))
    dxn = linear_dgrad(dqkv, wqkv).view(x.shape)
    other = tape.take(x)
    dx = ops.gn_bwd(dxn, x, st, ctx.p(pre + "norm.weight"), False, ctx.g(pre + "norm.weight"), ctx.g(pre + "norm.bias"), add=dy, add2=other)
    tape.grads[id(x)] = dx
    tape.keep.append(x)


def attention(ctx: Ctx, x, name, groups, eps, heads):
    b, d_, h_, w_, c = x.shape
    s = d_ * h_ * w_
    scale = 1.0 / math.sqrt(c / heads)
    dev = x.device
    pre = name + "." if name else ""
    st = gn(ctx, x, pre + "norm", groups, eps)
    xn = ops.gn_apply(x, st, False)
    wqkv = ops.cast_bf16(ctx.arena.span([f"{pre}to_{t}.weight" for t in "qkv"]).view(3 * c, c))
    bqkv = ctx.arena.span([f"{pre}to_{t}.bias" for t in "qkv"])
    qkv = ops.gemm_nt(xn.view(b * s, c), wqkv, bias=bqkv)
    if FLASH_ATTENTION and _lib.call_raw("mi_attn_supported", c, heads):
        return _attention_flash(ctx, x, name, st, xn, wqkv, qkv, b, s, c, heads, scale)
    q, k, v = (_heads(qkv[:, i * c:(i + 1) * c], b, heads) for i in range(3))
    y = torch.empty_like(x)
    sdpa_bwd = _sdpa(q, k, v, scale, out=_heads(y, b, heads), res=_heads(x, b, heads))
    ctx.count(2 * b * s * c * 3 * c)
    ctx.count(4 * b * s * s * c)
    if ctx.tape is not None:
        tape = ctx.tape

        def bwd():
            dy = tape.take(y)
            if dy is None:
                return
            dqkv = torch.empty((b * s, 3 * c), dtype=BF16, device=dev)
            sdpa_bwd(_heads(dy, b, heads), *(_heads(dqkv[:, i * c:(i + 1) * c], b, heads) for i in range(3)))
            _attention_param_and_input_grads(ctx, tape, x, name, st, xn, wqkv, dqkv, dy, b, s, c)

        tape.record(bwd)
    return y


def linear_f32(x_f32, w, b, gw, gb):
    xb, wb = ops.cast_bf16(x_f32), ops.cast_bf16(w)
    y = ops.gemm_nt(xb, wb, bias=b, out_f32=True)

    def bwd(dy_f32, need_dx=True):
        dyb = ops.cast_bf16(dy_f32)
        ops.sum_rows_f32(dy_f32, gb, accumulate=True)
        token_wgrad(dyb, xb, out=gw)
        return linear_dgrad(dyb, wb, out_f32=True) if need_dx else None

    return y, bwd


def _reshape(ctx: Ctx, x, shape):
    y = x.view(shape)
    if ctx.tape is not None:
        tape = ctx.tape

        def bwd():
            g = tape.take(y)
            if g is not None:
                tape.put(x, ops.dense(g).view(x.shape))

        tape.record(bwd)
    return y


def layernorm(ctx: Ctx, x, name, eps=1e-5):
    m, c = x.shape
    gamma, beta = ctx.p(name + ".weight"), ctx.p(name + ".bias")
    y = torch.empty_like(x)
    mr = torch.empty((m, 2), dtype=F32, device=x.device)
    call("mi_layernorm_fwd", ptr(x), c, ptr(gamma), ptr(beta), ptr(y), c, ptr(mr), m, c, float(eps))
    if ctx.tape is not None:
        tape = ctx.tape

        def bwd():
            dy = tape.take(y)
            if dy is None:
                return
            dx = torch.empty_like(x)
            call("mi_layernorm_bwd", ptr(dy), c, ptr(x), c, ptr(gamma), ptr(mr), ptr(dx), c, ptr(ctx.g(name + ".weight")),
                 ptr(ctx.g(name + ".bias")), m, c)
            tape.put(x, dx)

        tape.record(bwd)
    return y


def linear(ctx: Ctx, x, name, bias=True, res=None, need_dx=True):
    m, k = x.shape
    w = ctx.p(name + ".weight")
    n = w.shape[0]
    if k % 8 or n % 8:
        raise ValueError(f"{name}: feature counts must be multiples of 8 on the HIP path (got {k} -> {n})")
    wb = ops.cast_bf16(w)
    y = ops.gemm_nt(x, wb, bias=ctx.p(name + ".bias") if bias else None, res=res)
    ctx.count(2 * m * n * k, dgrad=need_dx)
    if ctx.tape is not None:
        tape = ctx.tape

        def bwd():
            dy = tape.take(y)
            if dy is None:
                return
            call("mi_linear_wgrad_bf16", ptr(x), k, k, ptr(dy), n, n, m, ptr(ctx.g(name + ".weight")), ptr(ctx.g(name + ".bias")) if bias else None)
            if res is not None:
                tape.put(res, dy)
            if need_dx:
                tape.put(x, linear_dgrad(dy, wb))

        tape.record(bwd)
    return y


def geglu(ctx: Ctx, h):
    m, f2 = h.shape
    f = f2 // 2
    y = torch.empty((m, f), dtype=BF16, device=h.device)
    call("mi_geglu_fwd", ptr(h), ptr(y), m, f)
    if ctx.tape is not None:
        tape = ctx.tape

        def bwd():
            dy = tape.take(y)
            if dy is not None:
                dh = torch.empty_like(h)
                call("mi_geglu_bwd", ptr(h), ptr(dy), ptr(dh), m, f)
                tape.put(h, dh)

        tape.record(bwd)
    return y


def mha(ctx: Ctx, q, k, v, b, sq, skv, heads):
    c = q.shape[1]
    o = torch.empty((b * sq, c), dtype=BF16, device=q.device)
    sdpa_bwd = _sdpa(*(_heads(t, b, heads) for t in (q, k, v)), 1.0 / math.sqrt(c // heads), out=_heads(o, b, heads))
    ctx.count(4 * b * sq * skv * c)
    if ctx.tape is not None:
        tape = ctx.tape

        def bwd():
            do = tape.take(o)
            if do is None:
                return
            dq, dk, dv = torch.empty_like(q), torch.empty_like(k), torch.empty_like(v)
            sdpa_bwd(*(_heads(t, b, heads) for t in (do, dq, dk, dv)))
            tape.put(q, dq), tape.put(k, dk), tape.put(v, dv)

        tape.record(bwd)
    return o


def spatial_transformer(ctx: Ctx, x, name, context, groups, eps, heads, layers):
    b, d_, h_, w_, c = x.shape
    s = d_ * h_ * w_
    pre = name + "." if name else ""
    st = gn(ctx, x, pre + "norm", groups, eps)
    xn = gn_act(ctx, x, st, False)
    one, zero = (1, 1, 1), (0, 0, 0)
    t = _reshape(ctx, conv(ctx, xn, pre + "proj_in.conv", one, one, zero), (b * s, c))
    sc = context.shape[0] // b if context is not None else s
    for li in range(layers):
        blk = f"{pre}transformer_blocks.{li}"
        n1 = layernorm(ctx, t, blk + ".norm1")
        a1 = blk + ".attn1"
        o = mha(ctx, linear(ctx, n1, a1 + ".to_q", bias=False), linear(ctx, n1, a1 + ".to_k", bias=False),
                linear(ctx, n1, a1 + ".to_v", bias=False), b, s, s, heads)
        t = linear(ctx, o, a1 + ".to_out.0", res=t)
        n2 = layernorm(ctx, t, blk + ".norm2")
        a2 = blk + ".attn2"
        kv_src, kv_grad = (context, False) if context is not None else (n2, True)
        o = mha(ctx, linear(ctx, n2, a2 + ".to_q", bias=False), linear(ctx, kv_src, a2 + ".to_k", bias=False, need_dx=kv_grad),
                linear(ctx, kv_src, a2 + ".to_v", bias=False, need_dx=kv_grad), b, s, sc, heads)
        t = linear(ctx, o, a2 + ".to_out.0", res=t)
        n3 = layernorm(ctx, t, blk + ".norm3")
        t = linear(ctx, geglu(ctx, linear(ctx, n3, blk + ".ff.linear1")), blk + ".ff.linear2", res=t)
    return conv(ctx, _reshape(ctx, t, (b, d_, h_, w_, c)), pre + "proj_out.conv", one, one, zero, res=x)
```

medical_image_generation_amd/hipops.py:

```python
from __future__ import annotations

import ctypes as C
import os

import torch

from . import _lib
from ._lib import call, ptr

BF16, F32 = torch.bfloat16, torch.float32
import os as _os
FUSE_GN_STATS = _os.environ.get("MI_FUSE_GN_STATS", "1") == "1"


def _vox(t):
    n, d, h, w, c = t.shape
    return n, d * h * w, c


def _cs(t):
    assert t.dim() == 5
    if t.is_contiguous():
        return t.shape[-1]
    assert t.stride(-1) == 1
    cs = t.stride(3)
    assert t.stride(2) == t.shape[3] * cs and t.stride(1) == t.shape[2] * t.stride(2) and t.stride(0) == t.shape[1] * t.stride(1), \
        "activation must be dense in N, D, H, W"
    return cs


def to_channels_last(x_ncdhw: torch.Tensor) -> torch.Tensor:
    x = x_ncdhw.contiguous()
    if x.dim() == 4:
        x = x.unsqueeze(2)
    n, c, d, h, w = x.shape
    out = torch.empty((n, d, h, w, c), dtype=BF16, device=x.device)
    call("mi_ncdhw_f32_to_ndhwc_bf16", ptr(x), ptr(out), n, c, d * h * w)
    return out


def to_channels_first(x_cl: torch.Tensor, spatial_dims: int = 3) -> torch.Tensor:
    assert x_cl.is_contiguous()
    n, d, h, w, c = x_cl.shape
    out = torch.empty((n, c, d, h, w), dtype=F32, device=x_cl.device)
    call("mi_ndhwc_bf16_to_ncdhw_f32", ptr(x_cl), ptr(out), n, c, d * h * w)
    return out.squeeze(2) if spatial_dims == 2 else out


def add(a, b):
    a, b = dense(a), dense(b)
    assert a.shape == b.shape
    out = torch.empty_like(a)
    call("mi_add_bf16", ptr(a), ptr(b), ptr(out), a.numel())
    return out


def concat_channels(a, b):
    n, v, ca = _vox(a)
    cb = b.shape[-1]
    out = torch.empty(a.shape[:-1] + (ca + cb,), dtype=BF16, device=a.device)
    call("mi_copy_channels", ptr(a), _cs(a), 0, ptr(out), ca + cb, 0, ca, n * v)
    call("mi_copy_channels", ptr(b), _cs(b), 0, ptr(out), ca + cb, ca, cb, n * v)
    return out


def slice_channels(x, c0, nc):
    n, v, c = _vox(x)
    out = torch.empty(x.shape[:-1] + (nc,), dtype=BF16, device=x.device)
    call("mi_copy_channels", ptr(x), _cs(x), c0, ptr(out), nc, 0, nc, n * v)
    return out


def dense(t):
    return t if t.is_contiguous() else slice_channels(t, 0, t.shape[-1])


def upsample_nearest(x, f):
    x = dense(x)
    n, d, h, w, c = x.shape
    out = torch.empty((n, d * f[0], h * f[1], w * f[2], c), dtype=BF16, device=x.device)
    call("mi_upsample_nearest_fwd", ptr(x), ptr(out), n, d, h, w, c, f[0], f[1], f[2])
    return out


def upsample_nearest_bwd(dy, f):
    n, d, h, w, c = dy.shape
    out = torch.empty((n, d // f[0], h // f[1], w // f[2], c), dtype=BF16, device=dy.device)
    call("mi_upsample_nearest_bwd", ptr(dy), ptr(out), n, d // f[0], h // f[1], w // f[2], c, f[0], f[1], f[2])
    return out


def _pool_out(dims, kernel, stride):
    return tuple((d - k) // s + 1 for d, k, s in zip(dims, kernel, stride))


def avg_pool(x, kernel, stride):
    x = dense(x)
    n, d, h, w, c = x.shape
    od, oh, ow = _pool_out((d, h, w), kernel, stride)
    out = torch.empty((n, od, oh, ow, c), dtype=BF16, device=x.device)
    arr = lambda v: (C.c_int * 3)(*v)
    call("mi_avgpool_fwd", ptr(x), ptr(out), n, d, h, w, c, arr(kernel), arr(stride))
    return out


def avg_pool_bwd(dy, in_dims, kernel, stride):
    n, c = dy.shape[0], dy.shape[-1]
    assert dy.is_contiguous() and tuple(dy.shape[1:4]) == _pool_out(in_dims, kernel, stride)
    dx = torch.empty((n,) + tuple(in_dims) + (c,), dtype=BF16, device=dy.device)
    arr = lambda v: (C.c_int * 3)(*v)
    call("mi_avgpool_bwd", ptr(dy), ptr(dx), n, in_dims[0], in_dims[1], in_dims[2], c, arr(kernel), arr(stride))
    return dx


_ws_cache: dict = {}


def _workspace(nbytes, device):
    key = (device.index, "gn")
    ws = _ws_cache.get(key)
    if ws is None or ws.numel() < nbytes:
        ws = torch.empty(max(nbytes, 1 << 20), dtype=torch.uint8, device=device)
        _ws_cache[key] = ws
    return ws


class GNStats:
    __slots__ = ("_ss", "_mr", "groups", "name", "_pending")

    def __init__(self, scale_shift, mean_rstd, groups, pending=None):
        self._ss, self._mr, self.groups, self._pending = scale_shift, mean_rstd, groups, pending

    def _force(self):
        if self._pending is not None:
            x, eps, gamma, beta = self._pending
            self._pending = None
            st = gn_stats(x, self.groups, eps, gamma, beta, allow_small=False)
            self._ss, self._mr = st._ss, st._mr

    @property
    def scale_shift(self):
        self._force()
        return self._ss

    @property
    def mean_rstd(self):
        self._force()
        return self._mr


GN_SMALL = os.environ.get("MI_GN_SMALL", "0") == "1"


def gn_stats(x, groups, eps, gamma, beta, allow_small=True) -> GNStats:
    n, v, c = _vox(x)
    if allow_small and GN_SMALL and c % groups == 0 and _lib.call_raw("mi_gn_small_supported", n, v, c, groups):
        return GNStats(None, None, groups, pending=(x, float(eps), gamma, beta))
    ss = torch.empty((n, c, 2), dtype=F32, device=x.device)
    mr = torch.empty((n, groups, 2), dtype=F32, device=x.device)
    nb = _lib.call_raw("mi_gn_workspace_bytes", n, v, c)
    ws = _workspace(nb, x.device)
    call("mi_gn_stats", ptr(x), _cs(x), n, v, c, groups, float(eps), ptr(gamma), ptr(beta), ptr(ss), ptr(mr), ptr(ws), ws.numel())
    return GNStats(ss, mr, groups)


class ChannelSums:
    __slots__ = ("partial", "chunks", "channels")

    def __init__(self, partial, chunks, channels):
        self.partial, self.chunks, self.channels = partial, chunks, channels


def gn_stats_from_sums(a: ChannelSums, b: ChannelSums | None, n, v, groups, eps, gamma, beta) -> GNStats | None:
    c = a.channels + (b.channels if b is not None else 0)
    dev = a.partial.device
    ss = torch.empty((n, c, 2), dtype=F32, device=dev)
    mr = torch.empty((n, groups, 2), dtype=F32, device=dev)
    call("mi_gn_stats_from_partial", ptr(a.partial), a.chunks, a.channels, ptr(b.partial) if b is not None else None,
         b.chunks if b is not None else 0, b.channels if b is not None else 0, n, v, groups, float(eps), ptr(gamma), ptr(beta), ptr(ss), ptr(mr))
    return GNStats(ss, mr, groups)


def gn_apply(x, st: GNStats, silu: bool):
    n, v, c = _vox(x)
    y = torch.empty(x.shape, dtype=BF16, device=x.device)
    if st._pending is not None and st._pending[0] is x:
        _, eps, gamma, beta = st._pending
        st._pending = None
        st._ss = torch.empty((n, c, 2), dtype=F32, device=x.device)
        st._mr = torch.empty((n, st.groups, 2), dtype=F32, device=x.device)
        call("mi_gn_small_fwd", ptr(x), _cs(x), ptr(y), c, n, v, c, st.groups, eps, ptr(gamma), ptr(beta), ptr(st._ss), ptr(st._mr), int(silu))
        return y
    call("mi_gn_apply", ptr(x), _cs(x), ptr(st.scale_shift), ptr(y), c, n, v, c, int(silu))
    return y


GN_FUSED_REPLICAS = 16


def gn_bwd(g, x, st: GNStats, gamma, silu: bool, dgamma, dbeta, add=None, add2=None, sums=None):
    if add is None and add2 is not None:
        add, add2 = add2, None
    n, v, c = _vox(x)
    dx = torch.empty(x.shape, dtype=BF16, device=x.device)
    if sums is not None:
        assert sums.dtype == torch.float64 and sums.numel() >= GN_FUSED_REPLICAS * n * c * 2
        call("mi_gn_bwd_fused", ptr(g), _cs(g), ptr(x), _cs(x), n, v, c, st.groups, ptr(gamma), ptr(st.scale_shift), ptr(st.mean_rstd),
             int(silu), ptr(add), _cs(add) if add is not None else 0, ptr(add2), _cs(add2) if add2 is not None else 0, ptr(dx), c,
             ptr(dgamma), ptr(dbeta), ptr(sums))
        return dx
    coef = torch.empty((n, c, 3), dtype=F32, device=x.device)
    nb = _lib.call_raw("mi_gn_workspace_bytes", n, v, c)
    ws = _workspace(nb, x.device)
    call("mi_gn_bwd", ptr(g), _cs(g), ptr(x), _cs(x), n, v, c, st.groups, ptr(gamma), ptr(st.scale_shift), ptr(st.mean_rstd),
         int(silu), ptr(add), _cs(add) if add is not None else 0, ptr(add2), _cs(add2) if add2 is not None else 0, ptr(dx), c, ptr(dgamma),
         ptr(dbeta), ptr(coef), ptr(ws), ws.numel())
    return dx


class ConvPlan:

    def __init__(self, n, dims, cin, cout, kernel, stride, padding):
        self.n, self.dims, self.cin, self.cout = n, tuple(dims), cin, cout
        self.kernel, self.stride, self.padding = tuple(kernel), tuple(stride), tuple(padding)
        h = C.c_void_p()
        arr = lambda v: (C.c_int * 3)(*v)
        _lib.call_raw("mi_conv_plan_create", C.byref(h), n, dims[0], dims[1], dims[2], cin, cout, arr(kernel), arr(stride), arr(padding))
        self.handle = h
        od = (C.c_int * 3)()
        _lib.call_raw("mi_conv_plan_out_dims", self.handle, od)
        self.out_dims = tuple(od)
        self.stats_chunks = int(_lib.call_raw("mi_conv_fwd_stats_chunks", self.handle))

    def __del__(self):
        try:
            if getattr(self, "handle", None):
                _lib.call_raw("mi_conv_plan_destroy", self.handle)
                self.handle = None
        except Exception:
            pass

    def pack(self, weight_f32):
        assert weight_f32.dtype == F32 and weight_f32.is_contiguous()
        call("mi_conv_pack_weights", self.handle, ptr(weight_f32))

    def fwd(self, x, st: GNStats | None = None, silu=False, addvec=None, res=None, out=None, want_sums=False):
        n, d, h, w, c = x.shape
        assert (n, (d, h, w), c) == (self.n, self.dims, self.cin), f"plan/input mismatch {x.shape} vs {self.n, self.dims, self.cin}"
        if out is None:
            y = torch.empty((n,) + self.out_dims + (self.cout,), dtype=BF16, device=x.device)
        else:
            assert out.shape == (n,) + self.out_dims + (self.cout,) and out.dtype == BF16
            y = out
        av_stride = 0
        if addvec is not None and addvec.dim() == 2:
            assert addvec.shape == (n, self.cout) and addvec.stride(1) == 1
            av_stride = addvec.stride(0)
        sums = None
        if want_sums and FUSE_GN_STATS and st is None and self.stats_chunks > 0 and (_cs(x) % 8 == 0 or (self.cin == 1 and res is None)):
            sums = ChannelSums(torch.empty((n, self.cout, self.stats_chunks, 2), dtype=F32, device=x.device), self.stats_chunks, self.cout)
        call("mi_conv_fwd", self.handle, ptr(x), _cs(x), ptr(st.scale_shift) if st is not None else None, int(silu), ptr(addvec), av_stride,
             ptr(res), _cs(res) if res is not None else 0, ptr(y), _cs(y), ptr(sums.partial) if sums is not None else None)
        return (y, sums) if want_sums else y

    def dgrad(self, dy):
        assert dy.shape == (self.n,) + self.out_dims + (self.cout,)
        dx = torch.empty((self.n,) + self.dims + (self.cin,), dtype=BF16, device=dy.device)
        call("mi_conv_dgrad", self.handle, ptr(dy), _cs(dy), ptr(dx), self.cin)
        return dx

    def wgrad(self, x, dy, dweight_f32, st: GNStats | None = None, silu=False, colsum=None):
        assert dweight_f32.dtype == F32 and dweight_f32.is_contiguous()
        cs_stride = 0
        if colsum is not None:
            assert colsum.dtype == F32 and colsum.stride(-1) == 1
            if colsum.dim() == 2:
                assert colsum.shape == (self.n, self.cout)
                cs_stride = colsum.stride(0)
            else:
                assert colsum.shape == (self.cout,)
        call("mi_conv_wgrad", self.handle, ptr(x), _cs(x), ptr(st.scale_shift) if st is not None else None, int(silu), ptr(dy), _cs(dy),
             ptr(dweight_f32), ptr(colsum), cs_stride)


class UpConvPlan(ConvPlan):

    def __init__(self, n, dims, cin, cout):
        self.n, self.dims, self.cin, self.cout = n, tuple(dims), cin, cout
        self.kernel, self.stride, self.padding = (3, 3, 3), (1, 1, 1), (1, 1, 1)
        h = C.c_void_p()
        _lib.call_raw("mi_upconv_plan_create", C.byref(h), n, dims[0], dims[1], dims[2], cin, cout)
        self.handle = h
        self.out_dims = tuple(2 * d for d in dims)
        self.stats_chunks = 0


def colsum(x, out=None, accumulate=False, merge_batch=False):
    n, v, c = _vox(x)
    assert x.is_contiguous()
    if merge_batch:
        n, v = 1, n * v
    if out is None:
        out = torch.empty((n, c), dtype=F32, device=x.device)
    stride = out.stride(0) if out.dim() == 2 else c
    call("mi_colsum_bf16", ptr(x), ptr(out), stride, n, v, c, int(accumulate))
    return out


def add_f32_(y, x):
    y2 = y if y.dim() == 2 else y.unsqueeze(0)
    if x.dim() == 1:
        assert x.shape[0] == y2.shape[1] and x.stride(0) == 1
        ldx, xp = 0, x
    else:
        assert x.shape == y2.shape and x.stride(1) == 1
        ldx, xp = x.stride(0), x
    assert y2.stride(1) == 1
    call("mi_add_f32_2d", ptr(xp), ldx, ptr(y2), y2.stride(0), y2.shape[0], y2.shape[1])
    return y


def zero_f32_2d_(x):
    assert x.dim() == 2 and x.stride(1) == 1
    call("mi_zero_f32_2d", ptr(x), x.stride(0), x.shape[0], x.shape[1])
    return x


def sum_rows_f32(x, out, accumulate=True):
    assert x.dim() == 2 and x.stride(1) == 1 and out.is_contiguous()
    call("mi_sum_rows_f32", ptr(x), x.stride(0), x.shape[0], x.shape[1], ptr(out), int(accumulate))
    return out


def _batch(*views):
    shapes = [tuple(v.shape[:-2]) for v in views]
    rank = max(len(s) for s in shapes)
    if rank > 2:
        raise ValueError(f"at most two batch levels, got {max(shapes, key=len)}")
    return tuple(max(col) for col in zip(*[(1,) * (rank - len(s)) + s for s in shapes]))


def _strided(v, batch, what, vec16=False, broadcast=True):
    if v is None:
        return 0, 0, 0
    if v.stride(-1) != 1:
        raise ValueError(f"{what}: last-dim stride must be 1, got {v.stride(-1)}")
    own = tuple(v.shape[:-2])
    lead = len(batch) - len(own)
    if lead < 0 or any(o != n and (o != 1 or not broadcast) for o, n in zip((1,) * lead + own, batch)):
        raise ValueError(f"{what}: batch shape {own} does not {'broadcast to' if broadcast else 'equal'} {tuple(batch)}")
    s = [0] * lead + [st if o == n else 0 for st, o, n in zip(v.stride(), own, batch[lead:])] + [0] * (2 - len(batch))
    if vec16 and (v.stride(-2) % 8 or s[0] % 8 or s[1] % 8 or v.data_ptr() % 16):
        raise ValueError(f"{what}: rows must start 16-byte aligned (pitch {v.stride(-2)}, batch strides {s[0]}, {s[1]} bf16 elements)")
    return v.stride(-2), s[0], s[1]


def _z(batch):
    return (batch[0] * batch[1], batch[1]) if len(batch) == 2 else (batch[0] if batch else 1, 1)


def padded(v):
    return v.as_strided(tuple(v.shape[:-1]) + (v.stride(-2),), v.stride())


def gemm_nt(a, b, *, bias=None, res=None, alpha=1.0, out=None, out_f32=False, accumulate=False):
    (m, k), (n, kb) = a.shape[-2:], b.shape[-2:]
    if kb != k or k % 8:
        raise ValueError(f"gemm_nt reduces over a shared K that is a multiple of 8, got {k} and {kb}")
    batch = _batch(a, b)
    if out is None:
        out = torch.empty(batch + (m, n), dtype=F32 if out_f32 else BF16, device=a.device)
    for t, what in ((out, "out"), (res, "res")):
        if t is not None and tuple(t.shape[-2:]) != (m, n):
            raise ValueError(f"{what}: expected [.., {m}, {n}], got {tuple(t.shape)}")
    assert a.dtype == b.dtype == BF16 and (res is None or res.dtype == BF16) and (out.dtype == F32 or not accumulate)
    sa, sb = _strided(a, batch, "a", vec16=True), _strided(b, batch, "b", vec16=True)
    so, sr = _strided(out, batch, "out", broadcast=False), _strided(res, batch, "res")
    call("mi_gemm_nt_bf16", ptr(a), *sa, ptr(b), *sb, ptr(out), *so, ptr(bias), ptr(res), *sr, m, n, k, *_z(batch), float(alpha),
         int(out.dtype == F32), int(accumulate))
    return out


def transpose(x, pad_to=None, out=None):
    assert pad_to in (None, 8), "the kernel zero-fills up to the next multiple of 8 only"
    r, c = x.shape[-2:]
    p = (r + 7) // 8 * 8 if pad_to else r
    batch = _batch(x)
    if out is None:
        out = torch.empty(batch + (c, p), dtype=BF16, device=x.device)
    if tuple(out.shape[-2:]) != (c, p) or x.dtype != BF16 or out.dtype != BF16:
        raise ValueError(f"out: expected bf16 [.., {c}, {p}], got {out.dtype} {tuple(out.shape)}")
    sx, so = _strided(x, batch, "x"), _strided(out, batch, "out", broadcast=False)
    call("mi_transpose_bf16", ptr(x), *sx, ptr(out), *so, r, c, *_z(batch))
    return out


def softmax_fwd(scores_f32, pad8=False):
    s = scores_f32.contiguous()
    cols = s.shape[-1]
    ld = (cols + 7) // 8 * 8 if pad8 else cols
    out = torch.empty(s.shape[:-1] + (ld,), dtype=BF16, device=s.device)
    call("mi_softmax_fwd", ptr(s), ptr(out), s.numel() // cols, cols, ld)
    return out[..., :cols]


def softmax_bwd(probs, dprobs_f32, scale):
    cols, ld = probs.shape[-1], probs.stride(-2)
    assert probs.stride(-1) == 1 and dprobs_f32.is_contiguous()
    out = torch.empty(probs.shape[:-1] + (ld,), dtype=BF16, device=probs.device)
    call("mi_softmax_bwd", ptr(probs), ptr(dprobs_f32), ptr(out), probs.numel() // cols, cols, ld, float(scale))
    return out[..., :cols]


def timestep_embedding(t_i64, dim, max_period=10000.0):
    out = torch.empty((t_i64.shape[0], dim), dtype=F32, device=t_i64.device)
    call("mi_timestep_embedding", ptr(t_i64), ptr(out), t_i64.shape[0], dim, float(max_period))
    return out


def silu_f32(x):
    y = torch.empty_like(x)
    call("mi_silu_f32", ptr(x), ptr(y), x.numel())
    return y


def silu_bwd_f32(x, dy):
    dx = torch.empty_like(x)
    call("mi_silu_bwd_f32", ptr(x), ptr(dy), ptr(dx), x.numel())
    return dx


def cast_bf16(x_f32):
    assert x_f32.is_contiguous() and x_f32.dtype == F32
    out = torch.empty(x_f32.shape, dtype=BF16, device=x_f32.device)
    call("mi_cast_f32_to_bf16", ptr(x_f32), ptr(out), x_f32.numel())
    return out


def cast_f32(x_bf16, out=None, accumulate=False):
    if out is None:
        out = torch.empty(x_bf16.shape, dtype=F32, device=x_bf16.device)
    call("mi_cast_bf16_to_f32", ptr(x_bf16), ptr(out), x_bf16.numel(), int(accumulate))
    return out
```

medical_image_generation_amd/inferer.py:

```python
from __future__ import annotations

import torch

from . import engine as E
from . import hipops as ops
from ._lib import call, ptr

F32 = torch.float32


def betas(schedule, num_train_timesteps, beta_start, beta_end):
    if schedule == "scaled_linear_beta":
        return torch.linspace(beta_start ** 0.5, beta_end ** 0.5, num_train_timesteps, dtype=F32) ** 2
    if schedule == "linear_beta":
        return torch.linspace(beta_start, beta_end, num_train_timesteps, dtype=F32)
    raise ValueError(f"unknown schedule {schedule}")


class DDPMScheduler:

    def __init__(self, num_train_timesteps=1000, schedule="linear_beta", variance_type="fixed_small", clip_sample=True,
                 prediction_type="epsilon", beta_start=1e-4, beta_end=2e-2):
        if variance_type != "fixed_small":
            raise NotImplementedError("only variance_type='fixed_small' (the upstream default the reference uses)")
        if prediction_type not in ("epsilon", "v_prediction"):
            raise ValueError(f"unknown prediction_type {prediction_type}")
        self.betas = betas(schedule, num_train_timesteps, beta_start, beta_end)
        self.num_train_timesteps, self.prediction_type, self.clip_sample = num_train_timesteps, prediction_type, clip_sample
        self.alphas = 1.0 - self.betas
        self.alphas_cumprod = torch.cumprod(self.alphas, dim=0)
        acp, b = self.alphas_cumprod.double(), self.betas.double()
        prev = torch.cat([torch.ones(1, dtype=torch.float64), acp[:-1]])
        sigma = ((1 - prev) / (1 - acp) * b).clamp(min=1e-20).sqrt()
        sigma[0] = 0.0
        self._coef = torch.stack([1 / acp.sqrt(), (1 - acp).sqrt(), prev.sqrt() * b / (1 - acp), (1 - b).sqrt() * (1 - prev) / (1 - acp), sigma],
                                 dim=1).float().contiguous()
        self._coef_dev = None
        self.set_timesteps(num_train_timesteps)

    def set_timesteps(self, num_inference_steps, device=None):
        if num_inference_steps > self.num_train_timesteps:
            raise ValueError(f"`num_inference_steps`: {num_inference_steps} cannot be larger than `self.num_train_timesteps`: "
                             f"{self.num_train_timesteps}")
        self.num_inference_steps = num_inference_steps
        ratio = self.num_train_timesteps // num_inference_steps
        self.timesteps = (torch.arange(0, num_inference_steps) * ratio).round().flip(0).to(torch.int64)
        if device is not None:
            self.timesteps = self.timesteps.to(device)

    def coefficients(self, device):
        if self._coef_dev is None or self._coef_dev.device != torch.device(device):
            self._coef_dev = self._coef.to(device)
        return self._coef_dev

    def add_noise(self, original_samples, noise, timesteps):
        a = self.alphas_cumprod.to(original_samples.device)[timesteps]
        shape = (-1,) + (1,) * (original_samples.ndim - 1)
        return (a ** 0.5).reshape(shape) * original_samples + ((1 - a) ** 0.5).reshape(shape) * noise

    def step(self, model_output, timestep, sample, generator=None):
        t = int(timestep)
        k = self._coef[t].to(sample.device)
        if self.prediction_type == "v_prediction":
            x0 = sample / k[0] - k[1] * model_output
        else:
            x0 = (sample - k[1] * model_output) * k[0]
        if self.clip_sample:
            x0 = x0.clamp(-1, 1)
        prev = k[2] * x0 + k[3] * sample
        if t > 0:
            prev = prev + k[4] * torch.randn(sample.shape, generator=generator, device=sample.device, dtype=sample.dtype)
        return prev, x0


class _Loop:

    def __init__(self, model, scheduler, shape, device, cond_channels=0, context_shape=None):
        self.m, self.sch = model, scheduler
        n, c = shape[0], shape[1]
        sp = tuple(shape[2:])
        self.v = 1
        for s in sp:
            self.v *= s
        dims = (1,) * (3 - len(sp)) + sp
        self.n, self.c = n, c
        self.x = torch.empty(shape, dtype=F32, device=device)
        self.cc = int(cond_channels)
        self.x_cl = torch.empty((n,) + dims + (c + self.cc,), dtype=torch.bfloat16, device=device)
        self.ctx = None if context_shape is None else torch.empty((n * context_shape[0], context_shape[1]), dtype=torch.bfloat16, device=device)
        self.z = torch.empty(shape, dtype=F32, device=device)
        self.t = torch.zeros(1, dtype=torch.int64, device=device)
        self.tn = torch.zeros(n, dtype=torch.int64, device=device)
        self.coef = scheduler.coefficients(device)
        self.arena = model.arena(device)
        self.graph = None
        self.keys = ()
        self._pinned = None

    def _step(self):
        ctx = E.Ctx(self.arena, self.m._plans, grad_enabled=False, prepacked=self.keys)
        eps = self.m._run(ctx, self.x_cl, self.tn, need_dx=False, context=self.ctx)
        call("mi_ddpm_step", ptr(self.x), ptr(eps), ptr(self.z), ptr(self.coef), ptr(self.t), ptr(self.x_cl), self.c + self.cc, self.n, self.c,
             self.v, int(self.sch.clip_sample) | (2 if self.sch.prediction_type == "v_prediction" else 0))

    def _load(self, x):
        self.x.copy_(x)
        self.x_cl[..., :self.c].copy_(ops.to_channels_last(self.x))

    def run(self, input_noise, noises=None, generator=None, use_graph=True, on_step=None, conditioning=None):
        if self.m._arena is not self.arena:
            self.arena, self.graph, self.keys, self._pinned = self.m.arena(self.x.device), None, (), None
        if self.cc:
            self.x_cl[..., self.c:].copy_(ops.to_channels_last(conditioning))
        elif self.ctx is not None:
            self.ctx.copy_(ops.cast_bf16(conditioning.contiguous().reshape(-1, conditioning.shape[2])))
        self._load(input_noise)
        steps = [int(t) for t in self.sch.timesteps]
        keep = self.x.clone()
        if not self.m._plans or len(self.keys) != len(self.m._plans):
            self.keys = ()
            self.z.zero_()
            self._step()
        self.keys = self.m.pack_all()
        if use_graph and self.graph is None and len(steps) > 2:
            s = torch.cuda.Stream()
            s.wait_stream(torch.cuda.current_stream())
            with torch.cuda.stream(s):
                self.z.zero_()
                self._step()
            torch.cuda.current_stream().wait_stream(s)
            torch.cuda.synchronize()
            self.graph = torch.cuda.CUDAGraph()
            with torch.cuda.graph(self.graph, capture_error_mode="thread_local"):
                self._step()
            self._pinned = (dict(self.m._plans), dict(ops._ws_cache), self.arena)
        self._load(keep)
        for i, t in enumerate(steps):
            self.t.fill_(t)
            self.tn.fill_(t)
            if noises is not None:
                self.z.copy_(noises[i])
            elif t > 0:
                self.z.normal_(generator=generator)
            if self.graph is not None:
                self.graph.replay()
            else:
                self._step()
            if on_step is not None:
                on_step(i, t, self.x)
        return self.x.clone()


class DiffusionInferer:

    def __init__(self, scheduler):
        self.scheduler = scheduler
        self._loops = {}

    def _loop(self, model, scheduler, shape, device, cond_channels=0, context_shape=None):
        key = (id(model), id(scheduler), tuple(shape), cond_channels, context_shape)
        if key not in self._loops:
            self._loops[key] = _Loop(model, scheduler, tuple(shape), device, cond_channels, context_shape)
        return self._loops[key]

    @staticmethod
    def _check_mode(mode):
        if mode not in ("crossattn", "concat"):
            raise NotImplementedError(f"{mode} condition is not supported")

    def __call__(self, inputs, diffusion_model, noise, timesteps, condition=None, mode="crossattn"):
        self._check_mode(mode)
        noisy = self.scheduler.add_noise(original_samples=inputs, noise=noise, timesteps=timesteps)
        if mode == "concat" and condition is not None:
            noisy, condition = torch.cat([noisy, condition.to(noisy.dtype)], dim=1), None
        return diffusion_model(x=noisy, timesteps=timesteps, context=condition)

    @torch.no_grad()
    def sample(self, input_noise, diffusion_model, scheduler=None, save_intermediates=False, intermediate_steps=100, conditioning=None,
               mode="crossattn", verbose=True, noises=None, generator=None, use_graph=True):
        self._check_mode(mode)
        if not input_noise.is_cuda:
            raise RuntimeError("medical_image_generation_amd runs on MI355X only: move the inputs to 'cuda'")
        cc, ctx_shape = 0, None
        if conditioning is not None:
            conditioning = conditioning.to(device=input_noise.device, dtype=F32).contiguous()
            if mode == "concat":
                if conditioning.dim() != input_noise.dim() or conditioning.shape[0] != input_noise.shape[0] or \
                        conditioning.shape[2:] != input_noise.shape[2:]:
                    raise ValueError("mode='concat': conditioning must have the sample's batch and spatial shape")
                cc = conditioning.shape[1]
            else:
                if not getattr(diffusion_model, "with_conditioning", False):
                    raise ValueError("model should have with_conditioning = True if context is provided")
                if conditioning.dim() != 3 or conditioning.shape[0] != input_noise.shape[0] or \
                        conditioning.shape[2] != diffusion_model.cross_attention_dim:
                    raise ValueError(f"mode='crossattn': conditioning must be [batch, tokens, {diffusion_model.cross_attention_dim}]")
                ctx_shape = (conditioning.shape[1], conditioning.shape[2])
        elif getattr(diffusion_model, "with_conditioning", False):
            raise ValueError("the model was built with_conditioning=True: pass conditioning=[batch, tokens, cross_attention_dim]")
        if input_noise.shape[1] + cc != diffusion_model.in_channels:
            raise ValueError(f"Input number of channels ({input_noise.shape[1] + cc}) is not equal to expected number of channels "
                             f"({diffusion_model.in_channels})")
        scheduler = scheduler or self.scheduler
        inter = []

        def on_step(i, t, x):
            if save_intermediates and t % intermediate_steps == 0:
                inter.append(x.clone())

        loop = self._loop(diffusion_model, scheduler, input_noise.shape, input_noise.device, cc, ctx_shape)
        image = loop.run(input_noise.float(), noises=noises, generator=generator, use_graph=use_graph, on_step=on_step, conditioning=conditioning)
        return (image, inter) if save_intermediates else image


class LatentDiffusionInferer(DiffusionInferer):

    def __init__(self, scheduler, scale_factor=1.0):
        super().__init__(scheduler)
        self.scale_factor = scale_factor

    def __call__(self, inputs, autoencoder_model, diffusion_model, noise, timesteps, condition=None, mode="crossattn"):
        with torch.no_grad():
            latent = autoencoder_model.encode_stage_2_inputs(inputs) * self.scale_factor
        return super().__call__(inputs=latent, diffusion_model=diffusion_model, noise=noise, timesteps=timesteps, condition=condition,
                                mode=mode)

    @torch.no_grad()
    def sample(self, input_noise, autoencoder_model, diffusion_model, scheduler=None, save_intermediates=False, intermediate_steps=100,
               conditioning=None, mode="crossattn", verbose=True, noises=None, generator=None, use_graph=True):
        out = super().sample(input_noise, diffusion_model, scheduler, save_intermediates, intermediate_steps, conditioning, mode, verbose,
                             noises=noises, generator=generator, use_graph=use_graph)
        latent, inter = out if save_intermediates else (out, None)
        image = autoencoder_model.decode_stage_2_outputs(latent / self.scale_factor)
        if save_intermediates:
            return image, [autoencoder_model.decode_stage_2_outputs(z / self.scale_factor) for z in inter]
        return image
```

medical_image_generation_amd/unet.py:

```python
from __future__ import annotations

import math
from typing import Sequence

import torch
from torch import nn

from . import engine as E
from . import hipops as ops
from ._lib import call, ptr

F32 = torch.float32
import os as _os
SKIP_SLOTS = _os.environ.get("MI_SKIP_SLOTS", "1") == "1"


class _Tree(nn.Module):
    """Anonymous container: gives parameters the reference's dotted state_dict names."""


def _attach(root, dotted, tensor):
    mod = root
    parts = dotted.split(".")
    for part in parts[:-1]:
        if part not in mod._modules:
            mod.add_module(part, _Tree())
        mod = mod._modules[part]
    mod.register_parameter(parts[-1], nn.Parameter(tensor))


def _tuple_rep(v, n):
    if isinstance(v, (list, tuple)):
        if len(v) != n:
            raise ValueError(f"Sequence must have length {n}, got {len(v)}.")
        return tuple(v)
    return (v,) * n


def _axis3(v, sd, fill):
    t = _tuple_rep(v, sd)
    return (fill,) * (3 - sd) + tuple(int(a) for a in t)


class ParamSpec:

    def __init__(self, root, sd):
        self.root, self.sd = root, sd
        self.order = []

    def _add(self, name, t, trainable=True):
        _attach(self.root, name, t)
        self.order.append((name, tuple(t.shape), trainable))

    def conv(self, name, cin, cout, k, zero=False):
        k = _tuple_rep(k, self.sd)
        w, b = torch.empty(cout, cin, *k), torch.empty(cout)
        if zero:
            w.zero_(), b.zero_()
        else:
            nn.init.kaiming_uniform_(w, a=math.sqrt(5))
            bound = 1 / math.sqrt(cin * math.prod(k))
            nn.init.uniform_(b, -bound, bound)
        self._add(name + ".weight", w)
        self._add(name + ".bias", b)

    def linear(self, name, cin, cout, trainable=True, bias=True):
        w = torch.empty(cout, cin)
        nn.init.kaiming_uniform_(w, a=math.sqrt(5))
        bound = 1 / math.sqrt(cin)
        self._add(name + ".weight", w, trainable)
        if bias:
            self._add(name + ".bias", torch.empty(cout).uniform_(-bound, bound), trainable)

    def transformer(self, name, c, cdim, layers):
        name = name + "." if name else ""
        self.norm(name + "norm", c)
        self.conv(name + "proj_in.conv", c, c, 1)
        for k in range(layers):
            blk = f"{name}transformer_blocks.{k}"
            for attn, kv in (("attn1", c), ("attn2", cdim)):
                self.linear(f"{blk}.{attn}.to_q", c, c, bias=False)
                self.linear(f"{blk}.{attn}.to_k", kv, c, bias=False)
                self.linear(f"{blk}.{attn}.to_v", kv, c, bias=False)
                self.linear(f"{blk}.{attn}.to_out.0", c, c)
            self.linear(f"{blk}.ff.linear1", c, 8 * c)
            self.linear(f"{blk}.ff.linear2", 4 * c, c)
            for n in ("norm1", "norm2", "norm3"):
                self.norm(f"{blk}.{n}", c)
        self.conv(name + "proj_out.conv", c, c, 1, zero=True)

    def norm(self, name, c):
        self._add(name + ".weight", torch.ones(c))
        self._add(name + ".bias", torch.zeros(c))

    def attention(self, name, c):
        pre = name + "." if name else ""
        self.norm(pre + "norm", c)
        for n in ("to_q", "to_k", "to_v"):
            self.linear(pre + n, c, c)
        self.linear(pre + "proj_attn", c, c, trainable=False)


def arena_order(entries, groups, late=()):
    grouped = {n for g in groups for n in g}
    by_name = {e[0]: e for e in entries}
    out = []
    for g in groups:
        out.extend(by_name[n] for n in g)
    out.extend(e for e in entries if e[0] not in grouped)
    late = set(late)
    for g in groups:
        assert len({n in late for n in g}) <= 1, f"group straddles the late / early split: {g[0]} ..."
    return [e for e in out if e[0] in late and e[2]] + [e for e in out if not (e[0] in late and e[2])]


class HipModule(nn.Module):

    def _init_plumbing(self, spec: ParamSpec, groups, late=()):
        self._late = tuple(n for n in late)
        self._entries = arena_order(spec.order, groups, self._late)
        self._arena = None
        self._plans = {}
        self._packb = None

    def arena(self, device) -> E.ParamArena:
        device = torch.device(device)
        if device.type == "cuda" and device.index is None:
            device = torch.device("cuda", torch.cuda.current_device())
        params = dict(self.named_parameters())
        a = self._arena
        first = self._entries[0][0]
        if a is None or a.data.device != device or params[first].data_ptr() != a.view(first).data_ptr():
            a = E.ParamArena(self._entries, device, late=self._late)
            for name, _, _ in self._entries:
                v = a.view(name)
                v.copy_(params[name].data)
                params[name].data = v
            self._arena = a
            self._plans = {}
            self._packb = None
        return a

    def pack_all(self):
        if not self._plans or self._arena is None:
            return ()
        pb = getattr(self, "_packb", None)
        if pb is None or len(pb.keys) != len(self._plans):
            if torch.cuda.is_current_stream_capturing():
                return () if pb is None else pb.run()
            pb = self._packb = E.PackBatch(self._arena, self._plans)
        return pb.run()

    def _apply(self, fn, *args, **kwargs):
        self._arena = None
        self._packb = None
        return super()._apply(fn, *args, **kwargs)


class _NetFn(torch.autograd.Function):

    @staticmethod
    def forward(ctx, module, runner, nouts, grad_enabled, x, emb, *params):
        dev = x.device
        ctx.set_materialize_grads(False)
        arena = module.arena(dev)
        c = E.Ctx(arena, module._plans, grad_enabled=grad_enabled, prepacked=module.pack_all())
        need_dx = bool(grad_enabled and ctx.needs_input_grad[4])
        outs_cl, extra = runner(c, x, need_dx) if emb is None else runner(c, x, need_dx, emb)
        ctx.c, ctx.module, ctx.outs_cl, ctx.need_dx, ctx.extra = c, module, outs_cl, need_dx, extra
        ctx.need_demb = bool(emb is not None and grad_enabled and ctx.needs_input_grad[5])
        ctx.sd = module.spatial_dims
        ctx.names = [n for n, _ in module.named_parameters()]
        outs = tuple(ops.to_channels_first(o, ctx.sd) for o in outs_cl)
        return outs if nouts > 1 else outs[0]

    @staticmethod
    def backward(ctx, *douts):
        c = ctx.c
        arena = c.arena
        arena.grad.zero_()
        tape = c.tape
        for o, do in zip(ctx.outs_cl, douts):
            if do is not None:
                tape.put(o, ops.to_channels_last(do.contiguous().float()))
        for fn in reversed(tape.fns):
            fn()
        tape.fns.clear()
        dx = None
        if ctx.need_dx:
            g = tape.take(ctx.extra["x_cl"])
            dx = ops.to_channels_first(ops.dense(g), ctx.sd) if g is not None else None
        demb = ctx.extra["d_emb"]() if ctx.need_demb else None
        trainable = {n for n, _, t in ctx.module._entries if t}
        grads = tuple(arena.gview(n).clone() if n in trainable else None for n in ctx.names)
        tape.grads.clear(), tape.keep.clear()
        return (None, None, None, None, dx, demb) + grads


class DiffusionModelUNet(HipModule):
    def __init__(
        self,
        spatial_dims: int,
        in_channels: int,
        out_channels: int,
        num_res_blocks: Sequence[int] | int = (2, 2, 2, 2),
        num_channels: Sequence[int] = (32, 64, 64, 64),
        attention_levels: Sequence[bool] = (False, False, True, True),
        norm_num_groups: int = 32,
        norm_eps: float = 1e-6,
        resblock_updown: bool = False,
        num_head_channels: int | Sequence[int] = 8,
        with_conditioning: bool = False,
        transformer_num_layers: int = 1,
        cross_attention_dim: int | None = None,
        num_class_embeds: int | None = None,
        upcast_attention: bool = False,
        use_flash_attention: bool = False,
        dropout_cattn: float = 0.0,
        strides=((2, 2, 2), (2, 2, 2), (2, 2, 2)),
        kernel_sizes=((4, 4, 4), (4, 4, 4), (4, 4, 4)),
        paddings=(1, 1, 1),
    ) -> None:
        super().__init__()
        if with_conditioning is True and cross_attention_dim is None:
            raise ValueError("DiffusionModelUNet expects dimension of the cross-attention conditioning (cross_attention_dim) "
                             "when using with_conditioning.")
        if cross_attention_dim is not None and with_conditioning is False:
            raise ValueError("DiffusionModelUNet expects with_conditioning=True when specifying the cross_attention_dim.")
        if dropout_cattn > 1.0 or dropout_cattn < 0.0:
            raise ValueError("Dropout cannot be negative or >1.0!")
        if any((c % norm_num_groups) != 0 for c in num_channels):
            raise ValueError("DiffusionModelUNet expects all num_channels being multiple of norm_num_groups")
        if len(num_channels) != len(attention_levels):
            raise ValueError("DiffusionModelUNet expects num_channels being same size of attention_levels")
        if isinstance(num_head_channels, int):
            num_head_channels = _tuple_rep(num_head_channels, len(attention_levels))
        if len(num_head_channels) != len(attention_levels):
            raise ValueError("num_head_channels should have the same length as attention_levels.")
        if isinstance(num_res_blocks, int):
            num_res_blocks = _tuple_rep(num_res_blocks, len(num_channels))
        if len(num_res_blocks) != len(num_channels):
            raise ValueError("`num_res_blocks` should be a single integer or a tuple of integers with the same length as "
                             "`num_channels`.")
        if use_flash_attention:
            raise ValueError("use_flash_attention is True but xformers is not installed.")
        if with_conditioning and dropout_cattn > 0.0:
            raise NotImplementedError("dropout_cattn > 0 is not on the HIP path (the reference's default is 0.0)")
        if with_conditioning and (cross_attention_dim % 8 or any(a and n % 8 for a, n in zip(attention_levels, num_head_channels))):
            raise ValueError("cross_attention_dim and num_head_channels must be multiples of 8 on the HIP path")
        if spatial_dims not in (2, 3):
            raise ValueError("spatial_dims must be 2 or 3")

        sd = self.spatial_dims = spatial_dims
        self.in_channels, self.out_channels = in_channels, out_channels
        self.block_out_channels = ch = tuple(num_channels)
        self.num_res_blocks = nrb = tuple(num_res_blocks)
        self.attention_levels = att = tuple(attention_levels)
        self.num_head_channels = nhc = tuple(num_head_channels)
        self.with_conditioning = bool(with_conditioning)
        self.cross_attention_dim, self.transformer_num_layers = cross_attention_dim, transformer_num_layers
        self.num_class_embeds = num_class_embeds
        self.resblock_updown = bool(resblock_updown)
        self.use_checkpointing = False
        self.groups, self.eps = norm_num_groups, norm_eps
        L = len(ch)
        self._k = [_axis3(kernel_sizes[i], sd, 1) for i in range(L)]
        self._s = [_axis3(strides[i], sd, 1) for i in range(L)]
        self._p = [_axis3(paddings[i], sd, 0) for i in range(L)]
        temb = self.temb_dim = ch[0] * 4

        spec = ParamSpec(self, sd)
        self._resnets: list[tuple[str, int, int]] = []
        self._attns: list[str] = []

        def resnet(name, cin, cout):
            spec.norm(name + ".norm1", cin)
            spec.conv(name + ".conv1.conv", cin, cout, 3)
            spec.linear(name + ".time_emb_proj", temb, cout)
            spec.norm(name + ".norm2", cout)
            spec.conv(name + ".conv2.conv", cout, cout, 3, zero=True)
            if cin != cout:
                spec.conv(name + ".skip_connection.conv", cin, cout, 1)
            self._resnets.append((name, cin, cout))

        def attn(name, c):
            if with_conditioning:
                spec.transformer(name, c, cross_attention_dim, transformer_num_layers)
            else:
                spec.attention(name, c)
                self._attns.append(name)

        spec.conv("conv_in.conv", in_channels, ch[0], kernel_sizes[0])
        spec.linear("time_embed.0", ch[0], temb)
        spec.linear("time_embed.2", temb, temb)
        out_c = ch[0]
        for i in range(L):
            in_c, out_c = out_c, ch[i]
            for j in range(nrb[i]):
                resnet(f"down_blocks.{i}.resnets.{j}", in_c if j == 0 else out_c, out_c)
                if att[i]:
                    attn(f"down_blocks.{i}.attentions.{j}", out_c)
            if i != L - 1:
                if resblock_updown:
                    resnet(f"down_blocks.{i}.downsampler", out_c, out_c)
                else:
                    spec.conv(f"down_blocks.{i}.downsampler.op.conv", out_c, out_c, kernel_sizes[i + 1])
        resnet("middle_block.resnet_1", ch[-1], ch[-1])
        attn("middle_block.attention", ch[-1])
        resnet("middle_block.resnet_2", ch[-1], ch[-1])
        rch, rnrb, ratt = list(reversed(ch)), list(reversed(nrb)), list(reversed(att))
        out_c = rch[0]
        for i in range(L):
            prev, out_c = out_c, rch[i]
            in_c = rch[min(i + 1, L - 1)]
            n = rnrb[i] + 1
            for j in range(n):
                skip_c = in_c if j == n - 1 else out_c
                resnet(f"up_blocks.{i}.resnets.{j}", (prev if j == 0 else out_c) + skip_c, out_c)
                if ratt[i]:
                    attn(f"up_blocks.{i}.attentions.{j}", out_c)
            if i != L - 1:
                if resblock_updown:
                    resnet(f"up_blocks.{i}.upsampler", out_c, out_c)
                else:
                    spec.conv(f"up_blocks.{i}.upsampler.conv.conv", out_c, out_c, 3)
        spec.norm("out.0", ch[0])
        spec.conv("out.2.conv", ch[0], out_channels, 3, zero=True)
        if num_class_embeds is not None:
            spec._add("class_embedding.weight", torch.randn(num_class_embeds, temb))

        groups = [[r[0] + ".time_emb_proj.weight" for r in self._resnets], [r[0] + ".time_emb_proj.bias" for r in self._resnets],
                  [r[0] + ".conv1.conv.bias" for r in self._resnets]]
        for a in self._attns:
            groups.append([f"{a}.to_{t}.weight" for t in "qkv"])
            groups.append([f"{a}.to_{t}.bias" for t in "qkv"])
        self._cut_level = max(0, L // 2 - 1)
        late_pre = tuple(f"down_blocks.{i}." for i in range(self._cut_level + 1)) + ("conv_in.", "time_embed.", "class_embedding.")
        late = [n for n, _, _ in spec.order if n.startswith(late_pre) or ".time_emb_proj." in n or n.endswith(".conv1.conv.bias")]
        self._init_plumbing(spec, groups, late)
        rch_, rnrb_ = list(reversed(ch)), list(reversed(nrb))
        pops = []
        for i in range(L):
            for j in range(rnrb_[i] + 1):
                pops.append((rch_[i - 1] if i > 0 else rch_[0]) if j == 0 else rch_[i])
        self._skip_ca = list(reversed(pops))
        self._temb_off = {}
        off = 0
        for name, _, cout in self._resnets:
            self._temb_off[name] = off
            off += cout
        self._temb_total = off

    def _resnet(self, c, x, name, temb_all, d_temb_all, out=None, mode=None, stride=None, kernel=None):
        cout = c.p(name + ".conv1.conv.weight").shape[0]
        off = self._temb_off[name]

        def run(cc, xx):
            return E.resnet(cc, xx, name, self.spatial_dims, self.groups, self.eps, temb_all[:, off:off + cout],
                            d_temb_all[:, off:off + cout] if d_temb_all is not None else None, mode=mode, stride=stride, kernel=kernel,
                            out=out if cc is c or cc.tape is None else None)

        return E.checkpoint(c, run, x) if self.use_checkpointing else run(c, x)

    def _attention(self, c, x, name, heads):
        if self.with_conditioning:
            run = lambda cc, xx: E.spatial_transformer(cc, xx, name, self._context, self.groups, self.eps, heads, self.transformer_num_layers)
        else:
            run = lambda cc, xx: E.attention(cc, xx, name, self.groups, self.eps, heads)
        return E.checkpoint(c, run, x) if self.use_checkpointing else run(c, x)

    def _heads(self, ch, nhc):
        return ch // nhc if nhc is not None else 1

    def _run(self, c: E.Ctx, x_cl, timesteps, need_dx, class_labels=None, down_res=None, mid_res=None, context=None):
        ch, L, sd = self.block_out_channels, len(self.block_out_channels), self.spatial_dims
        self._context = context
        a = c.arena
        dev = x_cl.device
        grad = c.tape is not None
        t0 = ops.timestep_embedding(timesteps, ch[0])
        e1, bwd1 = E.linear_f32(t0, c.p("time_embed.0.weight"), c.p("time_embed.0.bias"), c.g("time_embed.0.weight"), c.g("time_embed.0.bias"))
        s1v = ops.silu_f32(e1)
        emb, bwd2 = E.linear_f32(s1v, c.p("time_embed.2.weight"), c.p("time_embed.2.bias"), c.g("time_embed.2.weight"), c.g("time_embed.2.bias"))
        if self.num_class_embeds is not None:
            call("mi_embedding_add", ptr(emb), ptr(c.p("class_embedding.weight")), ptr(class_labels), emb.shape[0], emb.shape[1])
        se = ops.silu_f32(emb)
        wn = [r[0] + ".time_emb_proj.weight" for r in self._resnets]
        bn = [r[0] + ".time_emb_proj.bias" for r in self._resnets]
        T = self._temb_total
        temb_all, bwd3 = E.linear_f32(se, a.span(wn).view(T, self.temb_dim), a.span(bn), a.span(wn, a.grad).view(T, self.temb_dim),
                                      a.span(bn, a.grad))
        ops.add_f32_(temb_all, a.span([r[0] + ".conv1.conv.bias" for r in self._resnets]))
        d_temb_all = ops.zero_f32_2d_(torch.empty_like(temb_all)) if grad else None
        if grad:
            def bwd_emb():
                ops.sum_rows_f32(d_temb_all, a.span([r[0] + ".conv1.conv.bias" for r in self._resnets], a.grad), accumulate=True)
                d_se = bwd3(d_temb_all)
                d_emb = ops.silu_bwd_f32(emb, d_se)
                if self.num_class_embeds is not None:
                    call("mi_embedding_bwd", ptr(d_emb), ptr(class_labels), ptr(c.g("class_embedding.weight")), d_emb.shape[0], d_emb.shape[1])
                d_s1 = bwd2(d_emb)
                bwd1(ops.silu_bwd_f32(e1, d_s1), need_dx=False)

            c.tape.record(bwd_emb)

        k3 = (1,) * (3 - sd) + (3,) * sd
        slots = down_res is None and SKIP_SLOTS
        skips = []

        def slot(dims, cb):
            if not slots:
                return None, None
            ca = self._skip_ca[len(skips)]
            buf = torch.empty((x_cl.shape[0],) + tuple(dims) + (ca + cb,), dtype=torch.bfloat16, device=dev)
            return buf, buf[..., ca:]

        def conv_dims(dims, k, s, p):
            return tuple((d + 2 * pp - kk) // ss + 1 for d, kk, ss, pp in zip(dims, k, s, p))

        buf, view = slot(conv_dims(x_cl.shape[1:4], self._k[0], self._s[0], self._p[0]), ch[0])
        h = E.conv(c, x_cl, "conv_in.conv", self._k[0], self._s[0], self._p[0], need_dx=need_dx, out=view)
        skips.append((h, buf))
        for i in range(L):
            for j in range(self.num_res_blocks[i]):
                att = self.attention_levels[i]
                buf, view = (None, None) if att else slot(h.shape[1:4], ch[i])
                h = self._resnet(c, h, f"down_blocks.{i}.resnets.{j}", temb_all, d_temb_all, out=view)
                if att:
                    h = self._attention(c, h, f"down_blocks.{i}.attentions.{j}", self._heads(ch[i], self.num_head_channels[i]))
                skips.append((h, buf))
            if i != L - 1:
                if self.resblock_updown:
                    h = self._resnet(c, h, f"down_blocks.{i}.downsampler", temb_all, d_temb_all, mode="down", stride=self._s[i + 1],
                                     kernel=self._k[i + 1])
                    skips.append((h, None))
                else:
                    buf, view = slot(conv_dims(h.shape[1:4], self._k[i + 1], self._s[i + 1], self._p[i + 1]), ch[i])
                    h = E.conv(c, h, f"down_blocks.{i}.downsampler.op.conv", self._k[i + 1], self._s[i + 1], self._p[i + 1], out=view)
                    skips.append((h, buf))
            if i == self._cut_level and grad:
                c.tape.record(E.CUT)
        if down_res is not None:
            if len(down_res) != len(skips):
                raise ValueError(f"down_block_additional_residuals must hold {len(skips)} tensors, got {len(down_res)}")
            skips = [(E.add(c, sk, r, b_needs_grad=False), None) for (sk, _), r in zip(skips, down_res)]
        h = self._resnet(c, h, "middle_block.resnet_1", temb_all, d_temb_all)
        h = self._attention(c, h, "middle_block.attention", self._heads(ch[-1], self.num_head_channels[-1]))

        def cat_buffer(ca):
            sk, sbuf = skips[-1]
            if sbuf is not None and sbuf.shape[-1] == ca + sk.shape[-1]:
                return sbuf, sbuf[..., :ca]
            return E.concat_buffer(sk.shape, ca, sk.shape[-1], dev)

        pending, view = cat_buffer(ch[-1])
        h = self._resnet(c, h, "middle_block.resnet_2", temb_all, d_temb_all, out=None if mid_res is not None else view)
        if mid_res is not None:
            h = E.add(c, h, mid_res, b_needs_grad=False)
        rch, rnrb = list(reversed(ch)), list(reversed(self.num_res_blocks))
        ratt, rnhc = list(reversed(self.attention_levels)), list(reversed(self.num_head_channels))
        rs, rp = list(reversed(self._s)), list(reversed(self._p))
        for i in range(L):
            n_res = rnrb[i] + 1
            for j in range(n_res):
                sk, sbuf = skips.pop()
                if pending is None or (sbuf is not None and pending is not sbuf):
                    pending = sbuf if sbuf is not None and sbuf.shape[-1] == h.shape[-1] + sk.shape[-1] else pending
                h = E.concat(c, h, sk, buf=pending)
                pending, view = (None, None)
                if j < n_res - 1 and not ratt[i]:
                    pending, view = cat_buffer(rch[i])
                h = self._resnet(c, h, f"up_blocks.{i}.resnets.{j}", temb_all, d_temb_all, out=view)
                if ratt[i]:
                    h = self._attention(c, h, f"up_blocks.{i}.attentions.{j}", self._heads(rch[i], rnhc[i]))
            if i != L - 1 and self.resblock_updown:
                pending, view = cat_buffer(rch[i])
                h = self._resnet(c, h, f"up_blocks.{i}.upsampler", temb_all, d_temb_all, out=view, mode="up", stride=rs[i])
            elif i != L - 1:
                pending, view = cat_buffer(rch[i])
                h = E.upsample_conv(c, h, f"up_blocks.{i}.upsampler.conv.conv", rs[i], k3, rp[i], out=view)
        no = E.gn(c, h, "out.0", self.groups, self.eps)
        p1 = (0,) * (3 - sd) + (1,) * sd
        return E.conv(c, h, "out.2.conv", k3, (1, 1, 1), p1, norm=no, silu=True)

    def forward(self, x, timesteps, context=None, class_labels=None, down_block_additional_residuals=None,
                mid_block_additional_residual=None):
        if context is not None and not self.with_conditioning:
            raise ValueError("model should have with_conditioning = True if context is provided")
        if timesteps.ndim != 1:
            raise ValueError("Timesteps should be a 1d-array")
        if x.shape[1] != self.in_channels:
            raise ValueError(f"Input number of channels ({x.shape[1]}) is not equal to expected number of channels ({self.in_channels})")
        if not x.is_cuda:
            raise RuntimeError("medical_image_generation_amd runs on MI355X only: move the module and inputs to 'cuda' "
                               "(there is no CPU fallback; the CPU restatement lives in oracle/ for tests)")
        timesteps = timesteps.to(device=x.device, dtype=torch.int64)
        if self.num_class_embeds is not None:
            if class_labels is None:
                raise ValueError("class_labels should be provided when num_class_embeds > 0")
            class_labels = class_labels.to(device=x.device, dtype=torch.int64).contiguous()
            if class_labels.shape != timesteps.shape or int(class_labels.min()) < 0 or int(class_labels.max()) >= self.num_class_embeds:
                raise IndexError("class_labels must hold one index in [0, num_class_embeds) per sample")

        to_cl = lambda r: ops.to_channels_last(r.detach().to(x.device).contiguous().float())
        down_res = [to_cl(r) for r in down_block_additional_residuals] if down_block_additional_residuals is not None else None
        mid_res = to_cl(mid_block_additional_residual) if mid_block_additional_residual is not None else None

        ctx_tokens = None
        if context is not None:
            if context.dim() != 3 or context.shape[0] != x.shape[0] or context.shape[2] != self.cross_attention_dim:
                raise ValueError(f"context must be [batch, tokens, {self.cross_attention_dim}], got {tuple(context.shape)}")
            ctx_tokens = ops.cast_bf16(context.detach().to(x.device).contiguous().float().reshape(-1, context.shape[2]))

        def runner(c, xin, need_dx):
            x_cl = ops.to_channels_last(xin.contiguous().float())
            y = self._run(c, x_cl, timesteps, need_dx, class_labels, down_res, mid_res, ctx_tokens)
            return (y,), {"x_cl": x_cl}

        grad_enabled = torch.is_grad_enabled() and (x.requires_grad or any(p.requires_grad for p in self.parameters()))
        return _NetFn.apply(self, runner, 1, grad_enabled, x, None, *self.parameters())
```

Measured before the change: 97.90 million voxels/s.

## Fuse time-embedding linears, cache bf16 weight forms, and stream c1 conv halos

The fp32 time-embedding linears now run through a GEMM that reads fp32 activations directly, applies SiLU and a second bias in the epilogue, and uses a dedicated row-vector wgrad kernel when the batch is one. This removes separate cast, SiLU, add and sum-rows launches. Linear weights get cached bf16 and transposed forms, produced by a batched pack kernel, so the per-step weight casts and transposes go away. Separately, the single-channel-output conv reduce kernel now walks a column of depth tiles using a ring buffer in LDS, which reuses halo slices across tiles but gives the grid fewer blocks.

```diff
diff --git a/include/medimgen_hip.h b/include/medimgen_hip.h
--- a/include/medimgen_hip.h
+++ b/include/medimgen_hip.h
@@ -75,6 +75,12 @@
 int mi_gemm_nt_bf16(const void* A, int lda, int64_t sA1, int64_t sA2, const void* B, int ldb, int64_t sB1, int64_t sB2, void* C, int ldc,
                     int64_t sC1, int64_t sC2, const float* bias, const void* R, int ldr, int64_t sR1, int64_t sR2, int M, int N, int K,
                     int Z, int Z2, float alpha, int out_f32, int accumulate, hipStream_t stream);
+int mi_gemm_nt_f32a(const float* A, int lda, int silu, const void* B, int ldb, void* C, int ldc, const float* bias, const float* bias2,
+                    int M, int N, int K, int out_f32, hipStream_t stream);
+int mi_rowlinear_wgrad_f32(const float* dy, int lddy, const float* x, int ldx, int M, int N, int K, int silu, float* gw, int ldgw,
+                           float* gb, float* gb2, hipStream_t stream);
+int mi_linear_pack_run(const void* tiles, int ntiles, hipStream_t stream);
+int mi_linear_pack_tile_bytes(void);
 int mi_transpose_bf16(const void* in, int ld_in, int64_t si1, int64_t si2, void* out, int ld_out, int64_t so1, int64_t so2, int R, int Cc,
                       int Z, int Z2, hipStream_t stream);
 int mi_softmax_fwd(const float* scores, void* probs, int64_t rows, int cols, int ld_probs, hipStream_t stream);
diff --git a/medical_image_generation_amd/_lib.py b/medical_image_generation_amd/_lib.py
--- a/medical_image_generation_amd/_lib.py
+++ b/medical_image_generation_amd/_lib.py
@@ -46,6 +46,10 @@
     "mi_sum_rows_f32": [_p, _i, _i, _i, _p, _i, _p],
     "mi_zero_f32_2d": [_p, _i, _i, _i, _p],
     "mi_gemm_nt_bf16": [_p, _i, _l, _l, _p, _i, _l, _l, _p, _i, _l, _l, _p, _p, _i, _l, _l, _i, _i, _i, _i, _i, _f, _i, _i, _p],
+    "mi_gemm_nt_f32a": [_p, _i, _i, _p, _i, _p, _i, _p, _p, _i, _i, _i, _i, _p],
+    "mi_rowlinear_wgrad_f32": [_p, _i, _p, _i, _i, _i, _i, _i, _p, _i, _p, _p, _p],
+    "mi_linear_pack_run": [_p, _i, _p],
+    "mi_linear_pack_tile_bytes": [],
     "mi_transpose_bf16": [_p, _i, _l, _l, _p, _i, _l, _l, _i, _i, _i, _i, _p],
     "mi_softmax_fwd": [_p, _p, _l, _i, _i, _p],
     "mi_softmax_bwd": [_p, _p, _p, _l, _i, _i, _f, _p],
@@ -112,10 +116,10 @@
     "mi_kl_eval": [_p, _p, _p, _i, _i, _l, _p],
 }
 _RET = {"mi_gn_workspace_bytes": _l, "mi_attn_workspace_bytes": _l, "mi_aug_stats_workspace_bytes": _l, "mi_meter_bytes": _l}
-_NOCHECK = {"mi_abi_version", "mi_meter_bytes", "mi_ssim_tiles", "mi_gn_small_supported", "mi_gn_workspace_bytes", "mi_aug_stats_workspace_bytes", "mi_attn_supported", "mi_attn_workspace_bytes", "mi_conv_fwd_stats_chunks"}
+_NOCHECK = {"mi_abi_version", "mi_linear_pack_tile_bytes", "mi_meter_bytes", "mi_ssim_tiles", "mi_gn_small_supported", "mi_gn_workspace_bytes", "mi_aug_stats_workspace_bytes", "mi_attn_supported", "mi_attn_workspace_bytes", "mi_conv_fwd_stats_chunks"}
 
 _lib = None
-ABI_VERSION = 12
+ABI_VERSION = 13
 
 
 def exported_symbols() -> list[str]:
diff --git a/medical_image_generation_amd/blocks.py b/medical_image_generation_amd/blocks.py
--- a/medical_image_generation_amd/blocks.py
+++ b/medical_image_generation_amd/blocks.py
@@ -49,15 +49,12 @@
         def runner(c, xin, need_dx, emb_in):
             x_cl = ops.to_channels_last(xin.contiguous().float())
             e = emb_in.detach().contiguous().float()
-            se = ops.silu_f32(e)
-            temb, bwd = E.linear_f32(se, c.p("time_emb_proj.weight"), c.p("time_emb_proj.bias"), c.g("time_emb_proj.weight"),
-                                     c.g("time_emb_proj.bias"))
-            ops.add_f32_(temb, c.p("conv1.conv.bias"))
+            temb, bwd = E.linear_f32(c, e, c.p("time_emb_proj.weight"), c.p("time_emb_proj.bias"), c.g("time_emb_proj.weight"),
+                                     c.g("time_emb_proj.bias"), silu=True, bias2=c.p("conv1.conv.bias"), gb2=c.g("conv1.conv.bias"))
             d_temb = ops.zero_f32_2d_(torch.empty_like(temb)) if c.tape is not None else None
             state = {}
             if c.tape is not None:
                 def bwd_emb():
-                    ops.sum_rows_f32(d_temb, c.g("conv1.conv.bias"), accumulate=True)
                     state["d_emb"] = ops.silu_bwd_f32(e, bwd(d_temb))
 
                 c.tape.record(bwd_emb)
diff --git a/medical_image_generation_amd/csrc/api.hip b/medical_image_generation_amd/csrc/api.hip
--- a/medical_image_generation_amd/csrc/api.hip
+++ b/medical_image_generation_amd/csrc/api.hip
@@ -1,3 +1,3 @@
 #include "common.h"
 #include "medimgen_hip.h"
-extern "C" int mi_abi_version(void) { return 12; }
+extern "C" int mi_abi_version(void) { return 13; }
diff --git a/medical_image_generation_amd/csrc/conv_c1.hip b/medical_image_generation_amd/csrc/conv_c1.hip
--- a/medical_image_generation_amd/csrc/conv_c1.hip
+++ b/medical_image_generation_amd/csrc/conv_c1.hip
@@ -213,17 +213,22 @@
 }
 
 constexpr int kYP = 33;
+constexpr int kSl = kHH * kHW;
+constexpr int kRing = kTD + 2;
+static_assert(kHalo == kRing * kSl, "halo = kTD + 2 slices");
 
 template <int NK>
-__global__ void __launch_bounds__(256) k_c1_reduce(C1Args a) {
+__global__ void __launch_bounds__(256) k_c1_reduce(C1Args a, int seg_tiles) {
   extern __shared__ float Y[];
   const int lane = threadIdx.x & 63, wave = threadIdx.x >> 6, r = lane & 31, h = lane >> 5;
   const int tw = (a.W + kTW - 1) / kTW, th = (a.H + kTH - 1) / kTH, td = (a.D + kTD - 1) / kTD;
-  int tile = blockIdx.x;
-  const int tx = tile % tw; tile /= tw;
-  const int ty = tile % th; tile /= th;
-  const int tz = tile % td, n = tile / td;
-  const int z0 = tz * kTD - 1, y0 = ty * kTH - 1, x0 = tx * kTW - 1;
+  const int nseg = (td + seg_tiles - 1) / seg_tiles;
+  int col = blockIdx.x;
+  const int sg = col % nseg; col /= nseg;
+  const int tx = col % tw; col /= tw;
+  const int ty = col % th, n = col / th;
+  const int tz0 = sg * seg_tiles, tz1 = min(td, tz0 + seg_tiles);
+  const int y0 = ty * kTH - 1, x0 = tx * kTW - 1;
   bf16x8 wf[NK];
 #pragma unroll
   for (int ks = 0; ks < NK; ++ks) {
@@ -236,52 +241,75 @@
     wf[ks] = __builtin_bit_cast(bf16x8, pack8(f));
   }
   const bf16* xn = a.m + (int64_t)n * a.D * a.H * a.W * a.m_cs;
-  constexpr int NB = ((kHalo + 31) / 32 + 3) / 4;
+  constexpr int NB = ((kTD * kSl + 31) / 32 + 3) / 4;
   u32x4 raw[NB][NK];
   bool ok[NB];
-#pragma unroll
-  for (int i = 0; i < NB; ++i) {
-    const int hu = (wave + 4 * i) * 32 + r;
-    const int hx = hu % kHW, hy = (hu / kHW) % kHH, hz = hu / (kHW * kHH);
-    const int z = z0 + hz, yy = y0 + hy, x = x0 + hx;
-    const int zc = min(max(z, 0), a.D - 1), yc = min(max(yy, 0), a.H - 1), xc = min(max(x, 0), a.W - 1);
-    ok[i] = hu < kHalo && z == zc && yy == yc && x == xc;
-    const bf16* px = xn + (((int64_t)zc * a.H + yc) * a.W + xc) * a.m_cs;
-#pragma unroll
-    for (int ks = 0; ks < NK; ++ks) {
-      const int c = min(ks * 16 + 8 * h, a.C - 8);
-      raw[i][ks] = *(const u32x4*)(px + c);
-    }
-  }
-#pragma unroll
-  for (int i = 0; i < NB; ++i) {
-    const int blk = wave + 4 * i;
-    if (blk >= (kHalo + 31) / 32) break;
-    f32x16 acc;
-#pragma unroll
-    for (int e = 0; e < 16; ++e) acc[e] = 0.f;
-#pragma unroll
-    for (int ks = 0; ks < NK; ++ks) {
-      u32x4 b = raw[i][ks];
-      if (!(ok[i] && ks * 16 + 8 * h < a.C)) b = u32x4{0u, 0u, 0u, 0u};
-      acc = __builtin_amdgcn_mfma_f32_32x32x16_bf16(wf[ks], __builtin_bit_cast(bf16x8, b), acc, 0, 0, 0);
-    }
-    const int hu = blk * 32 + r;
-#pragma unroll
-    for (int e = 0; e < 16; ++e) Y[hu * kYP + (e & 3) + 8 * (e >> 2) + 4 * h] = acc[e];
-  }
-  __syncthreads();
+  auto load = [&](int zf, int nsl) {
+#pragma unroll
+    for (int i = 0; i < NB; ++i) {
+      const int hu = (wave + 4 * i) * 32 + r;
+      const int hz = hu / kSl, rem = hu - hz * kSl;
+      const int hy = rem / kHW, hx = rem - hy * kHW;
+      const int z = zf + hz, yy = y0 + hy, x = x0 + hx;
+      const int zc = min(max(z, 0), a.D - 1), yc = min(max(yy, 0), a.H - 1), xc = min(max(x, 0), a.W - 1);
+      ok[i] = hu < nsl * kSl && z == zc && yy == yc && x == xc;
+      if ((wave + 4 * i) * 32 >= nsl * kSl) continue;
+      const bf16* px = xn + (((int64_t)zc * a.H + yc) * a.W + xc) * a.m_cs;
+#pragma unroll
+      for (int ks = 0; ks < NK; ++ks) {
+        const int c = min(ks * 16 + 8 * h, a.C - 8);
+        raw[i][ks] = *(const u32x4*)(px + c);
+      }
+    }
+  };
+  auto product = [&](int zf, int nsl) {
+#pragma unroll
+    for (int i = 0; i < NB; ++i) {
+      const int blk = wave + 4 * i;
+      if (blk * 32 >= nsl * kSl) break;
+      f32x16 acc;
+#pragma unroll
+      for (int e = 0; e < 16; ++e) acc[e] = 0.f;
+#pragma unroll
+      for (int ks = 0; ks < NK; ++ks) {
+        u32x4 b = raw[i][ks];
+        if (!(ok[i] && ks * 16 + 8 * h < a.C)) b = u32x4{0u, 0u, 0u, 0u};
+        acc = __builtin_amdgcn_mfma_f32_32x32x16_bf16(wf[ks], __builtin_bit_cast(bf16x8, b), acc, 0, 0, 0);
+      }
+      const int hu = blk * 32 + r;
+      if (hu < nsl * kSl) {
+        const int hz = hu / kSl;
+        float* row = Y + ((zf + hz + kRing) % kRing * kSl + hu - hz * kSl) * kYP;
+#pragma unroll
+        for (int e = 0; e < 16; ++e) row[(e & 3) + 8 * (e >> 2) + 4 * h] = acc[e];
+      }
+    }
+  };
   const int ox = threadIdx.x & 7, oy = (threadIdx.x >> 3) & 7, oz = threadIdx.x >> 6;
-  const int z = tz * kTD + oz, yy = ty * kTH + oy, x = tx * kTW + ox;
-  if (z >= a.D || yy >= a.H || x >= a.W) return;
-  float o = a.addvec ? a.addvec[(int64_t)n * a.av_stride] : 0.f;
-#pragma unroll
-  for (int kd = 0; kd < 3; ++kd)
-#pragma unroll
-    for (int kh = 0; kh < 3; ++kh)
-#pragma unroll
-      for (int kw = 0; kw < 3; ++kw) o += Y[(((oz + kd) * kHH + oy + kh) * kHW + ox + kw) * kYP + (kd * 3 + kh) * 3 + kw];
-  a.y[((((int64_t)n * a.D + z) * a.H + yy) * a.W + x) * a.y_cs] = f2bf(o);
+  const int yy = ty * kTH + oy, x = tx * kTW + ox;
+  const float av = a.addvec ? a.addvec[(int64_t)n * a.av_stride] : 0.f;
+  load(tz0 * kTD - 1, 2);
+  product(tz0 * kTD - 1, 2);
+  load(tz0 * kTD + 1, kTD);
+  for (int tz = tz0; tz < tz1; ++tz) {
+    product(tz * kTD + 1, kTD);
+    if (tz + 1 < tz1) load((tz + 1) * kTD + 1, kTD);
+    __syncthreads();
+    const int z = tz * kTD + oz;
+    if (z < a.D && yy < a.H && x < a.W) {
+      float o = av;
+#pragma unroll
+      for (int kd = 0; kd < 3; ++kd) {
+        const float* sl = Y + (z + kd - 1 + kRing) % kRing * (kSl * kYP);
+#pragma unroll
+        for (int kh = 0; kh < 3; ++kh)
+#pragma unroll
+          for (int kw = 0; kw < 3; ++kw) o += sl[((oy + kh) * kHW + ox + kw) * kYP + (kd * 3 + kh) * 3 + kw];
+      }
+      a.y[((((int64_t)n * a.D + z) * a.H + yy) * a.W + x) * a.y_cs] = f2bf(o);
+    }
+    __syncthreads();
+  }
 }
 
 struct C1WgArgs {
@@ -469,9 +497,15 @@
   C1Args a{};
   a.N = N; a.D = D; a.H = H; a.W = W; a.C = C;
   a.m = (const bf16*)x; a.m_cs = x_cs; a.w = w; a.addvec = addvec; a.av_stride = av_stride; a.y = (bf16*)y; a.y_cs = y_cs;
-  const int64_t tiles = (int64_t)N * ((D + kTD - 1) / kTD) * ((H + kTH - 1) / kTH) * ((W + kTW - 1) / kTW);
+  const int td = (D + kTD - 1) / kTD;
+  const int64_t cols = (int64_t)N * ((H + kTH - 1) / kTH) * ((W + kTW - 1) / kTW);
+  int nseg = (int)((512 + cols - 1) / cols);
+  nseg = nseg < 1 ? 1 : nseg;
+  if (nseg > td / 4) nseg = td / 4 > 0 ? td / 4 : 1;
+  const int seg_tiles = (td + nseg - 1) / nseg;
+  const int64_t tiles = cols * ((td + seg_tiles - 1) / seg_tiles);
   if (tiles >= (1ll << 31)) return MI_ERR_UNSUPPORTED;
-  const size_t lds = sizeof(float) * (size_t)((kHalo + 31) / 32 * 32) * kYP;
+  const size_t lds = sizeof(float) * (size_t)kRing * kSl * kYP;
   const int nk = (C + 15) / 16;
   auto k = nk == 1 ? k_c1_reduce<1> : nk == 2 ? k_c1_reduce<2> : nk == 3 ? k_c1_reduce<3> : k_c1_reduce<4>;
   static bool attr_done[4] = {false, false, false, false};
@@ -480,7 +514,7 @@
     if (e != hipSuccess) return (int)e;
     attr_done[nk - 1] = true;
   }
-  hipLaunchKernelGGL(k, dim3((unsigned)tiles), dim3(256), lds, st, a);
+  hipLaunchKernelGGL(k, dim3((unsigned)tiles), dim3(256), lds, st, a, seg_tiles);
   MI_CHECK_LAUNCH();
   return 0;
 }
diff --git a/medical_image_generation_amd/csrc/gemm.hip b/medical_image_generation_amd/csrc/gemm.hip
--- a/medical_image_generation_amd/csrc/gemm.hip
+++ b/medical_image_generation_amd/csrc/gemm.hip
@@ -10,6 +10,7 @@
   const bf16* B;
   void* C;
   const float* bias;
+  const float* bias2;
   const bf16* R;
   int M, N, K, lda, ldb, ldc, ldr;
   int Z2;
@@ -18,7 +19,7 @@
   int out_f32, accumulate;
 };
 
-template <int WT>
+template <int WT, int AMODE>
 __global__ void __launch_bounds__(256) k_gemm_nt(GemmArgs p) {
   constexpr int BM = 64 * WT, BN = 64 * WT;
   __shared__ __attribute__((aligned(16))) bf16 lds[2][2][BM * PITCH];
@@ -26,7 +27,8 @@
   const int wm = wave >> 1, wn = wave & 1;
   const int r = lane & 31, h = lane >> 5;
   const int z = blockIdx.z, z1 = z / p.Z2, z2 = z % p.Z2;
-  const bf16* A = p.A + z1 * p.sA1 + z2 * p.sA2;
+  const bf16* A = AMODE ? p.A : p.A + z1 * p.sA1 + z2 * p.sA2;
+  const float* Af = (const float*)p.A + z1 * p.sA1 + z2 * p.sA2;
   const bf16* B = p.B + z1 * p.sB1 + z2 * p.sB2;
   const int m0 = blockIdx.y * BM, n0 = blockIdx.x * BN;
 
@@ -44,7 +46,18 @@
       u32x4 zero = {0u, 0u, 0u, 0u};
       int k = k0 + pk[i];
       int am = m0 + prow[i], bn = n0 + prow[i];
-      ra[i] = (am < p.M && k < p.K) ? *(const u32x4*)(A + (int64_t)am * p.lda + k) : zero;
+      if constexpr (AMODE == 0) {
+        ra[i] = (am < p.M && k < p.K) ? *(const u32x4*)(A + (int64_t)am * p.lda + k) : zero;
+      } else {
+        ra[i] = zero;
+        if (am < p.M && k < p.K) {
+          const float* s = Af + (int64_t)am * p.lda + k;
+          F8 f;
+#pragma unroll
+          for (int j = 0; j < 8; ++j) f.v[j] = AMODE == 2 ? silu_f(s[j]) : s[j];
+          ra[i] = pack8(f);
+        }
+      }
       rb[i] = (bn < p.N && k < p.K) ? *(const u32x4*)(B + (int64_t)bn * p.ldb + k) : zero;
     }
   };
@@ -102,6 +115,9 @@
         const int m = m0 + wm * 32 * WT + a * 32 + (e & 3) + 8 * (e >> 2) + 4 * h;
         if (m >= p.M) continue;
         float v = acc[a][b][e] * p.alpha + bv;
+        if constexpr (AMODE != 0) {
+          if (p.bias2) v += p.bias2[n];
+        }
         if (p.R) v += bf2f(p.R[roff + (int64_t)m * p.ldr + n]);
         const int64_t ci = coff + (int64_t)m * p.ldc + n;
         if (p.out_f32) {
@@ -130,6 +146,60 @@
     int cc = i >> 6, rr = i & 63;
     if (c0 + cc < Cc && r0 + rr < R) out[(int64_t)(c0 + cc) * ld_out + r0 + rr] = t[rr][cc];
     else if (c0 + cc < Cc && r0 + rr < min((R + 7) & ~7, ld_out)) out[(int64_t)(c0 + cc) * ld_out + r0 + rr] = f2bf(0.f);
+  }
+}
+
+struct LinPackTile {
+  const float* src;
+  bf16* dst;
+  bf16* dstT;
+  int N, K, lds, ldt, r0, c0;
+};
+__global__ void __launch_bounds__(256) k_linear_pack(const LinPackTile* __restrict__ tiles) {
+  __shared__ bf16 t[64][72];
+  const LinPackTile j = tiles[blockIdx.x];
+  for (int i = threadIdx.x; i < 64 * 64; i += 256) {
+    const int rr = i >> 6, cc = i & 63;
+    t[rr][cc] = (j.r0 + rr < j.N && j.c0 + cc < j.K) ? f2bf(j.src[(int64_t)(j.r0 + rr) * j.lds + j.c0 + cc]) : f2bf(0.f);
+  }
+  __syncthreads();
+  for (int i = threadIdx.x; i < 64 * 8; i += 256) {
+    const int rr = i >> 3, c8 = (i & 7) * 8;
+    if (j.r0 + rr < j.N && j.c0 + c8 < j.K)
+      *(u32x4*)(j.dst + (int64_t)(j.r0 + rr) * j.K + j.c0 + c8) = *(const u32x4*)&t[rr][c8];
+    const int kk = i >> 3, n8 = (i & 7) * 8;
+    if (j.c0 + kk < j.K && j.r0 + n8 < j.ldt) {
+      bf16x8 v;
+#pragma unroll
+      for (int e = 0; e < 8; ++e) v[e] = t[n8 + e][kk];
+      *(bf16x8*)(j.dstT + (int64_t)(j.c0 + kk) * j.ldt + j.r0 + n8) = v;
+    }
+  }
+}
+
+__global__ void __launch_bounds__(256) k_rowlinear_wgrad(const float* __restrict__ dy, int lddy, const float* __restrict__ x, int ldx,
+                                                         int M, int N, int K, int silu, float* __restrict__ gw, int ldgw,
+                                                         float* __restrict__ gb, float* __restrict__ gb2) {
+  const int64_t i = blockIdx.x * (int64_t)blockDim.x + threadIdx.x;
+  if (i >= (int64_t)N * K) return;
+  const int n = (int)(i / K), k = (int)(i - (int64_t)n * K);
+  float acc = 0.f;
+  for (int m = 0; m < M; ++m) {
+    const float xv = x[(int64_t)m * ldx + k];
+    acc += bf2f(f2bf(dy[(int64_t)m * lddy + n])) * bf2f(f2bf(silu ? silu_f(xv) : xv));
+  }
+  gw[(int64_t)n * ldgw + k] += acc;
+  if (k == 0) {
+    if (gb) {
+      float s = gb[n];
+      for (int m = 0; m < M; ++m) s += dy[(int64_t)m * lddy + n];
+      gb[n] = s;
+    }
+    if (gb2) {
+      float s = gb2[n];
+      for (int m = 0; m < M; ++m) s += dy[(int64_t)m * lddy + n];
+      gb2[n] = s;
+    }
   }
 }
 
@@ -178,11 +248,46 @@
   p.A = (const bf16*)A; p.B = (const bf16*)B; p.C = C; p.bias = bias; p.R = (const bf16*)R;
   p.M = M; p.N = N; p.K = K; p.lda = lda; p.ldb = ldb; p.ldc = ldc; p.ldr = ldr;
   p.Z2 = Z2; p.sA1 = sA1; p.sA2 = sA2; p.sB1 = sB1; p.sB2 = sB2; p.sC1 = sC1; p.sC2 = sC2; p.sR1 = sR1; p.sR2 = sR2;
-  p.alpha = alpha; p.out_f32 = out_f32; p.accumulate = accumulate;
+  p.alpha = alpha; p.out_f32 = out_f32; p.accumulate = accumulate; p.bias2 = nullptr;
   if ((int64_t)ceil_div(N, 128) * ceil_div(M, 128) * Z < 256)
-    hipLaunchKernelGGL(k_gemm_nt<1>, dim3(ceil_div(N, 64), ceil_div(M, 64), Z), dim3(256), 0, st, p);
+    hipLaunchKernelGGL((k_gemm_nt<1, 0>), dim3(ceil_div(N, 64), ceil_div(M, 64), Z), dim3(256), 0, st, p);
   else
-    hipLaunchKernelGGL(k_gemm_nt<2>, dim3(ceil_div(N, 128), ceil_div(M, 128), Z), dim3(256), 0, st, p);
+    hipLaunchKernelGGL((k_gemm_nt<2, 0>), dim3(ceil_div(N, 128), ceil_div(M, 128), Z), dim3(256), 0, st, p);
+  MI_CHECK_LAUNCH();
+  return 0;
+}
+
+int mi_gemm_nt_f32a(const float* A, int lda, int silu, const void* B, int ldb, void* C, int ldc, const float* bias, const float* bias2,
+                    int M, int N, int K, int out_f32, hipStream_t st) {
+  if (M <= 0 || N <= 0 || K <= 0 || lda < K || ldb < K || ldc < N) return MI_ERR_BAD_ARG;
+  if ((K & 7) || (ldb & 7) || ((uintptr_t)B & 15) || ((uintptr_t)A & 3)) return MI_ERR_BAD_ARG;
+  GemmArgs p = {};
+  p.A = (const bf16*)A; p.B = (const bf16*)B; p.C = C; p.bias = bias; p.bias2 = bias2; p.R = nullptr;
+  p.M = M; p.N = N; p.K = K; p.lda = lda; p.ldb = ldb; p.ldc = ldc; p.ldr = 0;
+  p.Z2 = 1;
+  p.alpha = 1.0f; p.out_f32 = out_f32; p.accumulate = 0;
+  const dim3 grid(ceil_div(N, 64), ceil_div(M, 64), 1);
+  if (silu)
+    hipLaunchKernelGGL((k_gemm_nt<1, 2>), grid, dim3(256), 0, st, p);
+  else
+    hipLaunchKernelGGL((k_gemm_nt<1, 1>), grid, dim3(256), 0, st, p);
+  MI_CHECK_LAUNCH();
+  return 0;
+}
+
+int mi_linear_pack_run(const void* tiles, int ntiles, hipStream_t st) {
+  if (!tiles || ntiles <= 0) return MI_ERR_BAD_ARG;
+  hipLaunchKernelGGL(k_linear_pack, dim3(ntiles), dim3(256), 0, st, (const LinPackTile*)tiles);
+  MI_CHECK_LAUNCH();
+  return 0;
+}
+int mi_linear_pack_tile_bytes(void) { return (int)sizeof(LinPackTile); }
+
+int mi_rowlinear_wgrad_f32(const float* dy, int lddy, const float* x, int ldx, int M, int N, int K, int silu, float* gw, int ldgw,
+                           float* gb, float* gb2, hipStream_t st) {
+  if (M <= 0 || M > 8 || N <= 0 || K <= 0 || lddy < N || ldx < K || ldgw < K || !gw) return MI_ERR_BAD_ARG;
+  hipLaunchKernelGGL(k_rowlinear_wgrad, dim3(ceil_div((int64_t)N * K, 256)), dim3(256), 0, st, dy, lddy, x, ldx, M, N, K, silu, gw, ldgw,
+                     gb, gb2);
   MI_CHECK_LAUNCH();
   return 0;
 }
diff --git a/medical_image_generation_amd/engine.py b/medical_image_generation_amd/engine.py
--- a/medical_image_generation_amd/engine.py
+++ b/medical_image_generation_amd/engine.py
@@ -41,6 +41,7 @@
         self.numel = max(off, 4)
         self.data = torch.zeros(self.numel, dtype=F32, device=device)
         self.grad = torch.zeros(self.numel, dtype=F32, device=device)
+        self.linear_forms = {}
 
     def view(self, name, flat=None):
         flat = self.data if flat is None else flat
@@ -140,16 +141,23 @@
 
     def __init__(self, arena: ParamArena, plans: dict):
         import ctypes as C
-        self.keys = tuple(plans)
-        n = len(self.keys)
-        plan_arr = (C.c_void_p * n)(*[plans[k].handle for k in self.keys])
-        w_arr = (C.c_void_p * n)(*[arena.view(k[0] + ".weight").data_ptr() for k in self.keys])
+        conv_keys = tuple(plans)
+        n = len(conv_keys)
+        plan_arr = (C.c_void_p * n)(*[plans[k].handle for k in conv_keys])
+        w_arr = (C.c_void_p * n)(*[arena.view(k[0] + ".weight").data_ptr() for k in conv_keys])
         h = C.c_void_p()
-        _lib.call_raw("mi_conv_pack_batch_create", C.byref(h), plan_arr, w_arr, n)
+        if n:
+            _lib.call_raw("mi_conv_pack_batch_create", C.byref(h), plan_arr, w_arr, n)
         self.handle = h
+        self.forms = dict(arena.linear_forms)
+        self.lin_table = ops.linear_pack_table(list(self.forms.values())) if self.forms else None
+        self.keys = conv_keys + tuple(self.forms)
 
     def run(self):
-        call("mi_conv_pack_batch_run", self.handle)
+        if self.handle:
+            call("mi_conv_pack_batch_run", self.handle)
+        if self.lin_table is not None:
+            ops.linear_pack_run(self.lin_table)
         return self.keys
 
     def __del__(self):
@@ -433,8 +441,19 @@
     return ops.gemm_nt(ops.transpose(dy, pad_to=8), ops.transpose(x, pad_to=8), out=out, out_f32=True, accumulate=out is not None)
 
 
-def linear_dgrad(dy, wb, out_f32=False):
-    return ops.gemm_nt(dy, ops.transpose(wb), out_f32=out_f32)
+def linear_forms(ctx: "Ctx", w):
+    key = ("linear", w.data_ptr(), w.shape[0], w.shape[1], w.stride(0))
+    forms = ctx.arena.linear_forms
+    f = forms.get(key)
+    if f is None and w.shape[1] % 8 == 0 and not torch.cuda.is_current_stream_capturing():
+        f = forms[key] = ops.LinearForms(w)
+    if f is not None and key in ctx.packed:
+        return f.wb, f.wt
+    return ops.cast_bf16(w), None
+
+
+def linear_dgrad(dy, wb, out_f32=False, wt=None):
+    return ops.gemm_nt(dy, wt if wt is not None else ops.transpose(wb), out_f32=out_f32)
 
 
 def _heads(t, b, heads):
@@ -464,7 +483,7 @@
     return bwd
 
 
-def _attention_flash(ctx, x, name, st, xn, wqkv, qkv, b, s, c, heads, scale):
+def _attention_flash(ctx, x, name, st, xn, wqkv, wqkv_t, qkv, b, s, c, heads, scale):
     dev = x.device
     d_, h_, w_ = x.shape[1:4]
     y = torch.empty_like(x)
@@ -487,18 +506,18 @@
             ws = torch.empty(max(nws, 16), dtype=torch.uint8, device=dev)
             call("mi_attn_bwd", ptr(qkv), 3 * c, c, heads, b, s, float(scale), ptr(y), ptr(x), ptr(dy), ptr(lse), ptr(dsum), ptr(dqkv),
                  ptr(ws), nws)
-            _attention_param_and_input_grads(ctx, tape, x, name, st, xn, wqkv, dqkv, dy, b, s, c)
-
-        tape.record(bwd)
-    return y
-
-
-def _attention_param_and_input_grads(ctx, tape, x, name, st, xn, wqkv, dqkv, dy, b, s, c):
+            _attention_param_and_input_grads(ctx, tape, x, name, st, xn, wqkv, wqkv_t, dqkv, dy, b, s, c)
+
+        tape.record(bwd)
+    return y
+
+
+def _attention_param_and_input_grads(ctx, tape, x, name, st, xn, wqkv, wqkv_t, dqkv, dy, b, s, c):
     pre = name + "." if name else ""
     gw = ctx.arena.span([f"{pre}to_{t}.weight" for t in "qkv"], ctx.arena.grad)
     gb = ctx.arena.span([f"{pre}to_{t}.bias" for t in "qkv"], ctx.arena.grad)
     call("mi_linear_wgrad_bf16", ptr(xn), c, c, ptr(dqkv), 3 * c, 3 * c, b * s, ptr(gw), ptr(gb))
-    dxn = linear_dgrad(dqkv, wqkv).view(x.shape)
+    dxn = linear_dgrad(dqkv, wqkv, wt=wqkv_t).view(x.shape)
     other = tape.take(x)
     dx = ops.gn_bwd(dxn, x, st, ctx.p(pre + "norm.weight"), False, ctx.g(pre + "norm.weight"), ctx.g(pre + "norm.bias"), add=dy, add2=other)
     tape.grads[id(x)] = dx
@@ -513,11 +532,11 @@
     pre = name + "." if name else ""
     st = gn(ctx, x, pre + "norm", groups, eps)
     xn = ops.gn_apply(x, st, False)
-    wqkv = ops.cast_bf16(ctx.arena.span([f"{pre}to_{t}.weight" for t in "qkv"]).view(3 * c, c))
+    wqkv, wqkv_t = linear_forms(ctx, ctx.arena.span([f"{pre}to_{t}.weight" for t in "qkv"]).view(3 * c, c))
     bqkv = ctx.arena.span([f"{pre}to_{t}.bias" for t in "qkv"])
     qkv = ops.gemm_nt(xn.view(b * s, c), wqkv, bias=bqkv)
     if FLASH_ATTENTION and _lib.call_raw("mi_attn_supported", c, heads):
-        return _attention_flash(ctx, x, name, st, xn, wqkv, qkv, b, s, c, heads, scale)
+        return _attention_flash(ctx, x, name, st, xn, wqkv, wqkv_t, qkv, b, s, c, heads, scale)
     q, k, v = (_heads(qkv[:, i * c:(i + 1) * c], b, heads) for i in range(3))
     y = torch.empty_like(x)
     sdpa_bwd = _sdpa(q, k, v, scale, out=_heads(y, b, heads), res=_heads(x, b, heads))
@@ -532,21 +551,28 @@
                 return
             dqkv = torch.empty((b * s, 3 * c), dtype=BF16, device=dev)
             sdpa_bwd(_heads(dy, b, heads), *(_heads(dqkv[:, i * c:(i + 1) * c], b, heads) for i in range(3)))
-            _attention_param_and_input_grads(ctx, tape, x, name, st, xn, wqkv, dqkv, dy, b, s, c)
-
-        tape.record(bwd)
-    return y
-
-
-def linear_f32(x_f32, w, b, gw, gb):
-    xb, wb = ops.cast_bf16(x_f32), ops.cast_bf16(w)
-    y = ops.gemm_nt(xb, wb, bias=b, out_f32=True)
+            _attention_param_and_input_grads(ctx, tape, x, name, st, xn, wqkv, wqkv_t, dqkv, dy, b, s, c)
+
+        tape.record(bwd)
+    return y
+
+
+def linear_f32(ctx: Ctx, x_f32, w, b, gw, gb, silu=False, bias2=None, gb2=None):
+    wb, wt = linear_forms(ctx, w)
+    y = ops.gemm_nt_f32a(x_f32, wb, silu=silu, bias=b, bias2=bias2)
+    m = x_f32.shape[0]
 
     def bwd(dy_f32, need_dx=True):
-        dyb = ops.cast_bf16(dy_f32)
-        ops.sum_rows_f32(dy_f32, gb, accumulate=True)
-        token_wgrad(dyb, xb, out=gw)
-        return linear_dgrad(dyb, wb, out_f32=True) if need_dx else None
+        if m == 1:
+            ops.rowlinear_wgrad(dy_f32, x_f32, gw, gb, gb2, silu=silu)
+        else:
+            ops.sum_rows_f32(dy_f32, gb, accumulate=True)
+            if gb2 is not None:
+                ops.sum_rows_f32(dy_f32, gb2, accumulate=True)
+            token_wgrad(ops.cast_bf16(dy_f32), ops.cast_bf16(ops.silu_f32(x_f32) if silu else x_f32), out=gw)
+        if not need_dx:
+            return None
+        return ops.gemm_nt_f32a(dy_f32, wt if wt is not None else ops.transpose(wb))
 
     return y, bwd
 
@@ -593,7 +619,7 @@
     n = w.shape[0]
     if k % 8 or n % 8:
         raise ValueError(f"{name}: feature counts must be multiples of 8 on the HIP path (got {k} -> {n})")
-    wb = ops.cast_bf16(w)
+    wb, wt = linear_forms(ctx, w)
     y = ops.gemm_nt(x, wb, bias=ctx.p(name + ".bias") if bias else None, res=res)
     ctx.count(2 * m * n * k, dgrad=need_dx)
     if ctx.tape is not None:
@@ -607,7 +633,7 @@
             if res is not None:
                 tape.put(res, dy)
             if need_dx:
-                tape.put(x, linear_dgrad(dy, wb))
+                tape.put(x, linear_dgrad(dy, wb, wt=wt))
 
         tape.record(bwd)
     return y
diff --git a/medical_image_generation_amd/hipops.py b/medical_image_generation_amd/hipops.py
--- a/medical_image_generation_amd/hipops.py
+++ b/medical_image_generation_amd/hipops.py
@@ -381,6 +381,54 @@
     return out
 
 
+def gemm_nt_f32a(a_f32, b, *, silu=False, bias=None, bias2=None, out_f32=True):
+    (m, k), (n, kb) = a_f32.shape, b.shape
+    if kb != k or k % 8:
+        raise ValueError(f"gemm_nt_f32a reduces over a shared K that is a multiple of 8, got {k} and {kb}")
+    assert a_f32.dtype == F32 and b.dtype == BF16 and a_f32.stride(1) == 1
+    (ldb, _, _) = _strided(b, (), "b", vec16=True)
+    out = torch.empty((m, n), dtype=F32 if out_f32 else BF16, device=a_f32.device)
+    call("mi_gemm_nt_f32a", ptr(a_f32), a_f32.stride(0), int(silu), ptr(b), ldb, ptr(out), n, ptr(bias), ptr(bias2), m, n, k, int(out_f32))
+    return out
+
+
+def rowlinear_wgrad(dy_f32, x_f32, gw, gb, gb2=None, silu=False):
+    (m, n), (mx, k) = dy_f32.shape, x_f32.shape
+    assert mx == m and m <= 8 and tuple(gw.shape) == (n, k) and gw.stride(1) == 1 and dy_f32.stride(1) == 1 and x_f32.stride(1) == 1
+    assert gb is None or (gb.numel() == n and gb.is_contiguous())
+    assert gb2 is None or (gb2.numel() == n and gb2.is_contiguous())
+    call("mi_rowlinear_wgrad_f32", ptr(dy_f32), dy_f32.stride(0), ptr(x_f32), x_f32.stride(0), m, n, k, int(silu), ptr(gw), gw.stride(0),
+         ptr(gb), ptr(gb2))
+
+
+class LinearForms:
+
+    def __init__(self, w):
+        n, k = w.shape
+        if k % 8 or w.stride(1) != 1 or w.dtype != F32:
+            raise ValueError(f"Linear weight forms need fp32 [N, K] rows with K a multiple of 8, got {w.dtype} {tuple(w.shape)}")
+        self.w = w
+        self.wb = torch.empty((n, k), dtype=BF16, device=w.device)
+        self._wt = torch.empty((k, (n + 7) // 8 * 8), dtype=BF16, device=w.device)
+        self.wt = self._wt[:, :n]
+
+    def tiles(self):
+        n, k = self.w.shape
+        lo = lambda a, b: a | (b << 32)
+        return [[self.w.data_ptr(), self.wb.data_ptr(), self._wt.data_ptr(), lo(n, k), lo(self.w.stride(0), self._wt.stride(0)), lo(r0, c0)]
+                for r0 in range(0, n, 64) for c0 in range(0, k, 64)]
+
+
+def linear_pack_table(forms):
+    assert _lib.call_raw("mi_linear_pack_tile_bytes") == 48
+    rows = [t for f in forms for t in f.tiles()]
+    return torch.tensor(rows, dtype=torch.int64).to(forms[0].w.device)
+
+
+def linear_pack_run(table):
+    call("mi_linear_pack_run", ptr(table), table.shape[0])
+
+
 def transpose(x, pad_to=None, out=None):
     assert pad_to in (None, 8), "the kernel zero-fills up to the next multiple of 8 only"
     r, c = x.shape[-2:]
diff --git a/medical_image_generation_amd/inferer.py b/medical_image_generation_amd/inferer.py
--- a/medical_image_generation_amd/inferer.py
+++ b/medical_image_generation_amd/inferer.py
@@ -117,7 +117,7 @@
         self._load(input_noise)
         steps = [int(t) for t in self.sch.timesteps]
         keep = self.x.clone()
-        if not self.m._plans or len(self.keys) != len(self.m._plans):
+        if not self.m._plans or len(self.keys) != len(self.m._plans) + len(self.arena.linear_forms):
             self.keys = ()
             self.z.zero_()
             self._step()
diff --git a/medical_image_generation_amd/unet.py b/medical_image_generation_amd/unet.py
--- a/medical_image_generation_amd/unet.py
+++ b/medical_image_generation_amd/unet.py
@@ -145,7 +145,7 @@
         if not self._plans or self._arena is None:
             return ()
         pb = getattr(self, "_packb", None)
-        if pb is None or len(pb.keys) != len(self._plans):
+        if pb is None or len(pb.keys) != len(self._plans) + len(self._arena.linear_forms):
             if torch.cuda.is_current_stream_capturing():
                 return () if pb is None else pb.run()
             pb = self._packb = E.PackBatch(self._arena, self._plans)
@@ -379,22 +379,20 @@
         dev = x_cl.device
         grad = c.tape is not None
         t0 = ops.timestep_embedding(timesteps, ch[0])
-        e1, bwd1 = E.linear_f32(t0, c.p("time_embed.0.weight"), c.p("time_embed.0.bias"), c.g("time_embed.0.weight"), c.g("time_embed.0.bias"))
-        s1v = ops.silu_f32(e1)
-        emb, bwd2 = E.linear_f32(s1v, c.p("time_embed.2.weight"), c.p("time_embed.2.bias"), c.g("time_embed.2.weight"), c.g("time_embed.2.bias"))
+        e1, bwd1 = E.linear_f32(c, t0, c.p("time_embed.0.weight"), c.p("time_embed.0.bias"), c.g("time_embed.0.weight"), c.g("time_embed.0.bias"))
+        emb, bwd2 = E.linear_f32(c, e1, c.p("time_embed.2.weight"), c.p("time_embed.2.bias"), c.g("time_embed.2.weight"), c.g("time_embed.2.bias"),
+                                 silu=True)
         if self.num_class_embeds is not None:
             call("mi_embedding_add", ptr(emb), ptr(c.p("class_embedding.weight")), ptr(class_labels), emb.shape[0], emb.shape[1])
-        se = ops.silu_f32(emb)
         wn = [r[0] + ".time_emb_proj.weight" for r in self._resnets]
         bn = [r[0] + ".time_emb_proj.bias" for r in self._resnets]
         T = self._temb_total
-        temb_all, bwd3 = E.linear_f32(se, a.span(wn).view(T, self.temb_dim), a.span(bn), a.span(wn, a.grad).view(T, self.temb_dim),
-                                      a.span(bn, a.grad))
-        ops.add_f32_(temb_all, a.span([r[0] + ".conv1.conv.bias" for r in self._resnets]))
+        cb = [r[0] + ".conv1.conv.bias" for r in self._resnets]
+        temb_all, bwd3 = E.linear_f32(c, emb, a.span(wn).view(T, self.temb_dim), a.span(bn), a.span(wn, a.grad).view(T, self.temb_dim),
+                                      a.span(bn, a.grad), silu=True, bias2=a.span(cb), gb2=a.span(cb, a.grad))
         d_temb_all = ops.zero_f32_2d_(torch.empty_like(temb_all)) if grad else None
         if grad:
             def bwd_emb():
-                ops.sum_rows_f32(d_temb_all, a.span([r[0] + ".conv1.conv.bias" for r in self._resnets], a.grad), accumulate=True)
                 d_se = bwd3(d_temb_all)
                 d_emb = ops.silu_bwd_f32(emb, d_se)
                 if self.num_class_embeds is not None:
```

New measurement: 98.75 million voxels/s (median of 6 runs). Within noise of the previous version (+0.9%).
